# jopohl/urh

Hardware: NVIDIA H100
Metric: MSamples/s IQ demod+digitize (complex64) (higher is better)
Workload: dtype f32

## Files before the change

### urh_b200/csrc/center.cu

```cuda
#include "dense.cuh"
#include "scan.cuh"

#include <math.h>
#include <stdlib.h>

int urh_window_var_bitwise(urh_ctx* ctx, const float* d_x, int64_t n, const int64_t* d_prefix, int64_t t0, int64_t t1, int64_t r0,
                           int64_t r1, float* h_out2);

struct CenStats {
    double sum, sumsq;
    float mn, mx;
    long long cnt;
};

__global__ void __launch_bounds__(URH_WARPS_PER_BLOCK * 32)
k_tile_stats_f32(const float* __restrict__ x, int64_t n, int64_t ntiles, UrhTileStats* __restrict__ ts) {
    const int lane = threadIdx.x & 31;
    const int64_t tile = (int64_t)blockIdx.x * URH_WARPS_PER_BLOCK + (threadIdx.x >> 5);
    if (tile >= ntiles) return;
    const int64_t base = tile * URH_TILE;
    UrhStatAcc acc;
    acc.init();
    acc.all_noise = false;
    if (base + URH_TILE <= n && (((uintptr_t)x) & 15) == 0) {
        const float4* p = (const float4*)(x + base) + lane;
        constexpr int ITERS = URH_TILE / 128;
        float4 cur[4], nxt[4];
#pragma unroll
        for (int j = 0; j < 4; j++) cur[j] = __ldg(p + j * 32);
        for (int it = 0; it < ITERS; it += 4) {
            if (it + 4 < ITERS) {
#pragma unroll
                for (int j = 0; j < 4; j++) nxt[j] = __ldg(p + (it + 4 + j) * 32);
            }
#pragma unroll
            for (int j = 0; j < 4; j++) {
                acc.add(cur[j].x); acc.add(cur[j].y); acc.add(cur[j].z); acc.add(cur[j].w);
            }
#pragma unroll
            for (int j = 0; j < 4; j++) cur[j] = nxt[j];
        }
    } else {
        for (int j = lane; j < URH_TILE; j += 32)
            if (base + j < n) acc.add(x[base + j]);
    }
    acc.store(ts + tile, lane);
}

__global__ void k_tile_counts(const UrhTileStats* __restrict__ ts, int64_t ntiles, int64_t* __restrict__ prefix) {
    const int64_t t = (int64_t)blockIdx.x * blockDim.x + threadIdx.x;
    if (t < ntiles) prefix[t] = ts[t].cnt;
}

__global__ void k_find_window_tiles(const int64_t* __restrict__ prefix, int64_t ntiles, int64_t r0, int64_t r1, int64_t* __restrict__ win) {
    const int64_t t = (int64_t)blockIdx.x * blockDim.x + threadIdx.x;
    if (t >= ntiles) return;
    const int64_t a = prefix[t], b = prefix[t + 1];
    if (b <= a) return;
    const bool covered = a >= r0 && b <= r1;
    const bool has_r0 = a <= r0 && r0 < b, has_r1 = a <= r1 - 1 && r1 - 1 < b;
    if (has_r0) { win[0] = t; win[2] = covered ? -1 : t; }
    if (has_r1) { win[1] = t; win[3] = (covered || has_r0) ? -1 : t; }
}

#define CEN_PER (URH_TILE / 256)
__device__ __forceinline__ int64_t cen_tile_ranks(const float* __restrict__ x, int64_t n, int64_t t, int64_t tile_rank0, float (&v)[CEN_PER],
                                                  int* s_pre) {
    const int64_t base = t * URH_TILE + (int64_t)threadIdx.x * CEN_PER;
    int mine = 0;
#pragma unroll
    for (int j = 0; j < CEN_PER; j++) {
        v[j] = (base + j < n) ? x[base + j] : -5.0f;
        mine += (v[j] > -4.0f) ? 1 : 0;
    }
    s_pre[threadIdx.x] = mine;
    __syncthreads();
    for (int off = 1; off < 256; off <<= 1) {
        int add = 0;
        if (threadIdx.x >= off) add = s_pre[threadIdx.x - off];
        __syncthreads();
        s_pre[threadIdx.x] += add;
        __syncthreads();
    }
    return tile_rank0 + s_pre[threadIdx.x] - mine;
}

__device__ __forceinline__ void cen_block_fold(double sum, double sq, float mn, float mx, long long cnt, CenStats* out) {
    __shared__ double s_sum[256], s_sq[256];
    __shared__ float s_mn[256], s_mx[256];
    __shared__ long long s_cnt[256];
    __syncthreads();
    s_sum[threadIdx.x] = sum; s_sq[threadIdx.x] = sq; s_mn[threadIdx.x] = mn; s_mx[threadIdx.x] = mx; s_cnt[threadIdx.x] = cnt;
    __syncthreads();
    for (int off = 128; off > 0; off >>= 1) {
        if (threadIdx.x < off) {
            s_sum[threadIdx.x] += s_sum[threadIdx.x + off];
            s_sq[threadIdx.x] += s_sq[threadIdx.x + off];
            s_mn[threadIdx.x] = fminf(s_mn[threadIdx.x], s_mn[threadIdx.x + off]);
            s_mx[threadIdx.x] = fmaxf(s_mx[threadIdx.x], s_mx[threadIdx.x + off]);
            s_cnt[threadIdx.x] += s_cnt[threadIdx.x + off];
        }
        __syncthreads();
    }
    if (threadIdx.x == 0) {
        CenStats r;
        r.sum = s_sum[0]; r.sumsq = s_sq[0]; r.mn = s_mn[0]; r.mx = s_mx[0]; r.cnt = s_cnt[0];
        *out = r;
    }
}

__global__ void __launch_bounds__(256) k_cut_tile_stats(const float* __restrict__ x, int64_t n, const int64_t* __restrict__ prefix,
                                                       const int64_t* __restrict__ win, int64_t r0, int64_t r1, CenStats* __restrict__ out) {
    __shared__ int s_pre[256];
    const int64_t t = win[2 + blockIdx.x];
    double sum = 0.0, sq = 0.0;
    float mn = INFINITY, mx = -INFINITY;
    long long cnt = 0;
    if (t >= 0) {
        float v[CEN_PER];
        int64_t rank = cen_tile_ranks(x, n, t, prefix[t], v, s_pre);
#pragma unroll
        for (int j = 0; j < CEN_PER; j++) {
            if (v[j] > -4.0f) {
                if (rank >= r0 && rank < r1) {
                    sum += (double)v[j];
                    sq += (double)v[j] * (double)v[j];
                    mn = fminf(mn, v[j]);
                    mx = fmaxf(mx, v[j]);
                    cnt++;
                }
                rank++;
            }
        }
    }
    cen_block_fold(sum, sq, mn, mx, cnt, out + blockIdx.x);
}

__global__ void __launch_bounds__(256) k_interior_tile_stats(const UrhTileStats* __restrict__ ts, const int64_t* __restrict__ prefix,
                                                            int64_t ntiles, int64_t r0, int64_t r1, CenStats* __restrict__ partial) {
    double sum = 0.0, sq = 0.0;
    float mn = INFINITY, mx = -INFINITY;
    long long cnt = 0;
    for (int64_t t = (int64_t)blockIdx.x * 256 + threadIdx.x; t < ntiles; t += (int64_t)gridDim.x * 256) {
        const int64_t a = prefix[t], b = prefix[t + 1];
        if (b > a && a >= r0 && b <= r1) {
            const UrhTileStats v = ts[t];
            sum += v.sum; sq += v.sumsq; mn = fminf(mn, v.mn); mx = fmaxf(mx, v.mx); cnt += v.cnt;
        }
    }
    cen_block_fold(sum, sq, mn, mx, cnt, partial + blockIdx.x);
}

__global__ void __launch_bounds__(256) k_center_fold(const CenStats* __restrict__ partial, int64_t count, CenStats* __restrict__ out) {
    double sum = 0.0, sq = 0.0;
    float mn = INFINITY, mx = -INFINITY;
    long long cnt = 0;
    for (int64_t t = threadIdx.x; t < count; t += 256) {
        const CenStats p = partial[t];
        sum += p.sum; sq += p.sumsq; mn = fminf(mn, p.mn); mx = fmaxf(mx, p.mx); cnt += p.cnt;
    }
    cen_block_fold(sum, sq, mn, mx, cnt, out);
}

int urh_center_tiles_begin(urh_ctx* ctx, const float* d_x, const UrhTileStats* ts, int64_t n, int64_t* h_total) {
    const int64_t ntiles = urh_div_up(n, URH_TILE);
    int64_t *prefix, *d_total;
    URH_CHECK(urh_arena(ctx, (size_t)ntiles + 1, &prefix));
    URH_CHECK(urh_arena(ctx, 4, &d_total));
    URH_LAUNCH(ctx, k_tile_counts, (unsigned)urh_div_up(ntiles, 256), 256, 0, ts, ntiles, prefix);
    URH_CHECK((urhscan::device_scan<int64_t, urhscan::AddI64>(ctx, prefix, ntiles, urhscan::AddI64(), (int64_t)0, true, d_total)));
    URH_CUDA(ctx, cudaMemcpyAsync(prefix + ntiles, d_total, sizeof(int64_t), cudaMemcpyDeviceToDevice, ctx->stream));
    URH_CHECK(urh_read_i64(ctx, d_total, 1, h_total));
    ctx->center_prefix = prefix;
    ctx->center_ts = ts;
    ctx->center_n = n;
    ctx->center_x = d_x;
    return URH_OK;
}

static int tiles_from_array(urh_ctx* ctx, const float* d_x, int64_t n, int64_t* h_total) {
    urh_arena_reset(ctx);
    ctx->center_prefix = nullptr;
    const int64_t ntiles = urh_div_up(n, URH_TILE);
    UrhTileStats* ts;
    URH_CHECK(urh_arena(ctx, (size_t)ntiles, &ts));
    URH_LAUNCH(ctx, k_tile_stats_f32, (unsigned)urh_div_up(ntiles, URH_WARPS_PER_BLOCK), URH_WARPS_PER_BLOCK * 32, 0, d_x, n, ntiles, ts);
    return urh_center_tiles_begin(ctx, d_x, ts, n, h_total);
}

static bool tiles_match(const urh_ctx* ctx, const float* d_x, int64_t n) {
    return ctx->center_prefix && ctx->center_n == n && ctx->center_x == (const void*)d_x;
}

extern "C" int urh_center_window_stats(urh_ctx* ctx, const float* d_qad, int64_t n, int64_t r0, int64_t r1, double* h_out5) {
    h_out5[0] = 0.0; h_out5[1] = INFINITY; h_out5[2] = -INFINITY; h_out5[3] = 0.0; h_out5[4] = 0.0;
    if (!tiles_match(ctx, d_qad, n)) URH_FAIL(ctx, URH_ERR_INVALID, "urh_afp_demod_tiles (same qad, same n) must precede urh_center_window_stats");
    if (r1 <= r0) return URH_OK;
    const int64_t ntiles = urh_div_up(n, URH_TILE);
    const int64_t* prefix = (const int64_t*)ctx->center_prefix;
    const UrhTileStats* ts = (const UrhTileStats*)ctx->center_ts;
    int64_t* d_win;
    CenStats* partial;
    CenStats* folded;
    const int nb = ctx->sm_count * 2;
    URH_CHECK(urh_arena(ctx, 4, &d_win));
    URH_CHECK(urh_arena(ctx, (size_t)nb + 4, &partial));
    URH_CHECK(urh_arena(ctx, 2, &folded));
    URH_CUDA(ctx, cudaMemsetAsync(d_win, 0xff, 4 * sizeof(int64_t), ctx->stream));
    URH_LAUNCH(ctx, k_find_window_tiles, (unsigned)urh_div_up(ntiles, 256), 256, 0, prefix, ntiles, r0, r1, d_win);
    URH_LAUNCH(ctx, k_interior_tile_stats, nb, 256, 0, ts, prefix, ntiles, r0, r1, partial);
    URH_LAUNCH(ctx, k_cut_tile_stats, 2, 256, 0, d_qad, n, prefix, d_win, r0, r1, partial + nb);
    URH_LAUNCH(ctx, k_center_fold, 1, 256, 0, partial, (int64_t)nb + 2, folded);
    CenStats st;
    URH_CUDA(ctx, cudaMemcpyAsync(ctx->h_mail, folded, sizeof(CenStats), cudaMemcpyDeviceToHost, ctx->stream));
    URH_CUDA(ctx, cudaStreamSynchronize(ctx->stream));
    memcpy(&st, ctx->h_mail, sizeof(st));
    h_out5[0] = (double)st.cnt; h_out5[1] = (double)st.mn; h_out5[2] = (double)st.mx; h_out5[3] = st.sum; h_out5[4] = st.sumsq;
    return URH_OK;
}

extern "C" int urh_center_window_var(urh_ctx* ctx, const float* d_qad, int64_t n, int64_t r0, int64_t r1, double* h_out2) {
    h_out2[0] = h_out2[1] = 0.0;
    if (!tiles_match(ctx, d_qad, n)) URH_FAIL(ctx, URH_ERR_INVALID, "the tile table of this array must precede urh_center_window_var");
    if (r1 <= r0) return URH_OK;
    float mv[2];
    URH_CHECK(urh_window_var_bitwise(ctx, d_qad, n, (const int64_t*)ctx->center_prefix, 0, urh_div_up(n, URH_TILE) - 1, r0, r1, mv));
    h_out2[0] = (double)mv[0];
    h_out2[1] = (double)mv[1];
    return URH_OK;
}

extern "C" int urh_center_stats(urh_ctx* ctx, const float* d_x, int64_t n, int64_t max_size, double* h_out) {
    for (int i = 0; i < 7; i++) h_out[i] = 0.0;
    if (n <= 0) return URH_OK;
    int64_t total = 0;
    URH_CHECK(tiles_from_array(ctx, d_x, n, &total));
    int64_t r0 = (int64_t)(0.05 * (double)total), r1 = (int64_t)(0.95 * (double)total);
    if (max_size >= 0 && r1 - r0 > max_size) r1 = r0 + max_size;
    h_out[0] = (double)total; h_out[1] = (double)r0; h_out[2] = (double)r1;
    if (r1 <= r0) return URH_OK;
    double w[5];
    URH_CHECK(urh_center_window_stats(ctx, d_x, n, r0, r1, w));
    if (w[0] <= 0.0) return URH_OK;
    h_out[3] = w[1]; h_out[4] = w[2];
    float mv[2];
    URH_CHECK(urh_window_var_bitwise(ctx, d_x, n, (const int64_t*)ctx->center_prefix, 0, urh_div_up(n, URH_TILE) - 1, r0, r1, mv));
    h_out[5] = (double)mv[0];
    h_out[6] = (double)mv[1];
    return URH_OK;
}

__global__ void k_hist_edges(double hmin, double hstep, int64_t nbins, float* __restrict__ fe) {
    const int64_t k = (int64_t)blockIdx.x * blockDim.x + threadIdx.x;
    if (k <= nbins) fe[k] = __double2float_ru(__dadd_rn(hmin, __dmul_rn((double)k, hstep)));
    if (k == nbins) {
        fe[nbins + 1] = __double2float_rd(__dadd_rn(hmin, __dmul_rn((double)nbins, hstep)));
        fe[nbins + 2] = fmaxf(__double2float_ru(hmin), nextafterf(-4.0f, 0.0f));
    }
}

struct HistBins {
    const float* fe;
    float f_min, f_hi, scale, off;
    int nbins;
    __device__ __forceinline__ void load(const float* fe_, float scale_, int nbins_) {
        fe = fe_; nbins = nbins_; scale = scale_;
        f_hi = fe[nbins + 1];
        f_min = fe[nbins + 2];
        off = -fe[0] * scale;
    }
    template <bool FAST>
    __device__ __forceinline__ int bin_of(float f) const {
        const bool valid = f >= f_min && f <= f_hi;
        if (FAST) {
            const float t = fmaf(f, scale, off);
            int r = __float_as_int(t + 12582912.0f) - 0x4B400000;
            r = max(0, min(r, nbins));
            int k = r - ((f < fe[r]) ? 1 : 0);
            k = min(k, nbins - 1);
            return valid ? k : -1;
        }
        if (!valid) return -1;
        int k = (int)((f - fe[0]) * scale);
        k = max(0, min(k, nbins - 1));
        while (k > 0 && f < fe[k]) k--;
        while (k < nbins - 1 && f >= fe[k + 1]) k++;
        return k;
    }
};

struct HistCache {
    float lo0, hi0, lo1, hi1, lo2, hi2, lo3, hi3;
    int h0, h1, h2, h3;
    unsigned c0, c1, c2, c3;
    __device__ __forceinline__ void init() {
        lo0 = lo1 = lo2 = lo3 = INFINITY;
        hi0 = hi1 = hi2 = hi3 = -INFINITY;
        h0 = h1 = h2 = h3 = 0;
        c0 = c1 = c2 = c3 = 0u;
    }
};

template <bool SMEM>
__device__ __forceinline__ void hist_bump(unsigned int* s_hist, unsigned long long* hist, int k, unsigned c) {
    if (SMEM) atomicAdd(&s_hist[k], c);
    else atomicAdd(&hist[k], (unsigned long long)c);
}

template <bool SMEM, bool FAST>
__device__ __forceinline__ void hist_miss(HistCache& hc, const HistBins& hb, unsigned int* s_hist, unsigned long long* hist, float f) {
    const int k = hb.bin_of<FAST>(f);
    if (k < 0) return;
    const float lo = fmaxf(hb.fe[k], hb.f_min);
    const float hi = (k == hb.nbins - 1) ? nextafterf(hb.f_hi, INFINITY) : hb.fe[k + 1];
    unsigned cm = hc.c0; int which = 0;
    if (hc.c1 < cm) { cm = hc.c1; which = 1; }
    if (hc.c2 < cm) { cm = hc.c2; which = 2; }
    if (hc.c3 < cm) { cm = hc.c3; which = 3; }
    const int old = which == 0 ? hc.h0 : which == 1 ? hc.h1 : which == 2 ? hc.h2 : hc.h3;
    if (cm) hist_bump<SMEM>(s_hist, hist, old, cm);
    if (which == 0) { hc.h0 = k; hc.c0 = 1u; hc.lo0 = lo; hc.hi0 = hi; }
    else if (which == 1) { hc.h1 = k; hc.c1 = 1u; hc.lo1 = lo; hc.hi1 = hi; }
    else if (which == 2) { hc.h2 = k; hc.c2 = 1u; hc.lo2 = lo; hc.hi2 = hi; }
    else { hc.h3 = k; hc.c3 = 1u; hc.lo3 = lo; hc.hi3 = hi; }
}

template <bool SMEM, bool FAST>
__device__ __forceinline__ void hist_put(HistCache& hc, const HistBins& hb, unsigned int* s_hist, unsigned long long* hist, float f,
                                         unsigned one) {
    unsigned miss;
    asm("{\n\t.reg .pred p0, p1, p2, p3, pv;\n\t"
        "setp.ge.f32 p0, %5, %6;\n\tsetp.lt.and.f32 p0, %5, %7, p0;\n\t@p0 mad.lo.u32 %0, %0, %15, %15;\n\t"
        "setp.ge.f32 p1, %5, %8;\n\tsetp.lt.and.f32 p1, %5, %9, p1;\n\t@p1 mad.lo.u32 %1, %1, %15, %15;\n\t"
        "setp.ge.f32 p2, %5, %10;\n\tsetp.lt.and.f32 p2, %5, %11, p2;\n\t@p2 mad.lo.u32 %2, %2, %15, %15;\n\t"
        "setp.ge.f32 p3, %5, %12;\n\tsetp.lt.and.f32 p3, %5, %13, p3;\n\t@p3 mad.lo.u32 %3, %3, %15, %15;\n\t"
        "or.pred p0, p0, p1;\n\tor.pred p2, p2, p3;\n\tor.pred p0, p0, p2;\n\t"
        "setp.ge.f32 pv, %5, %14;\n\t"
        "and.pred pv, pv, !p0;\n\t"
        "selp.u32 %4, 1, 0, pv;\n\t}"
        : "+r"(hc.c0), "+r"(hc.c1), "+r"(hc.c2), "+r"(hc.c3), "=r"(miss)
        : "f"(f), "f"(hc.lo0), "f"(hc.hi0), "f"(hc.lo1), "f"(hc.hi1), "f"(hc.lo2), "f"(hc.hi2), "f"(hc.lo3), "f"(hc.hi3),
          "f"(hb.f_min), "r"(one));
    if (miss) hist_miss<SMEM, FAST>(hc, hb, s_hist, hist, f);
}

template <bool SMEM>
__device__ __forceinline__ void hist_flush(HistCache& hc, unsigned int* s_hist, unsigned long long* hist) {
    if (hc.c0) hist_bump<SMEM>(s_hist, hist, hc.h0, hc.c0);
    if (hc.c1) hist_bump<SMEM>(s_hist, hist, hc.h1, hc.c1);
    if (hc.c2) hist_bump<SMEM>(s_hist, hist, hc.h2, hc.c2);
    if (hc.c3) hist_bump<SMEM>(s_hist, hist, hc.h3, hc.c3);
}

template <bool SMEM, bool FAST>
__device__ __forceinline__ void hist_interior_body(const float* __restrict__ x, int64_t n, int64_t t_first, int64_t t_end, int blk, int nblk,
                                                   const float* __restrict__ g_fe, float scale, int nbins,
                                                   unsigned long long* __restrict__ hist, int edges_in_smem,
                                                   const int64_t* __restrict__ prefix) {
    extern __shared__ unsigned int s_dyn[];
    unsigned int* s_hist = s_dyn;
    float* s_fe = (float*)(s_dyn + (SMEM ? nbins : 0));
    const int lane = threadIdx.x & 31;
    if (SMEM)
        for (int b = threadIdx.x; b < nbins; b += 256) s_hist[b] = 0u;
    if (edges_in_smem)
        for (int b = threadIdx.x; b < nbins + 3; b += 256) s_fe[b] = g_fe[b];
    __syncthreads();
    HistBins hb;
    if (FAST) hb.load(s_fe, scale, nbins);
    else hb.load(edges_in_smem ? s_fe : g_fe, scale, nbins);
    HistCache hc;
    hc.init();
    const int64_t gw = (int64_t)blk * 8 + (threadIdx.x >> 5), nw = (int64_t)nblk * 8;
    const bool vec = (((uintptr_t)x) & 15) == 0;
    const unsigned one = blockDim.x >> 8;
    {
        for (int64_t t = t_first + gw; t < t_end; t += nw) {
            if (prefix[t + 1] == prefix[t]) continue;
            const int64_t base = t * URH_TILE;
            if (vec) {
                const float4* p = (const float4*)(x + base) + lane;
                constexpr int ITERS = URH_TILE / 128, DEPTH = 4;
                float4 buf[DEPTH];
#pragma unroll
                for (int j = 0; j < DEPTH; j++) buf[j] = __ldg(p + j * 32);
#pragma unroll 1
                for (int it = 0; it < ITERS; it += DEPTH) {
                    const bool more = it + DEPTH < ITERS;
#pragma unroll
                    for (int j = 0; j < DEPTH; j++) {
                        const float4 v = buf[j];
                        if (more) buf[j] = __ldg(p + (it + DEPTH + j) * 32);
                        hist_put<SMEM, FAST>(hc, hb, s_hist, hist, v.x, one);
                        hist_put<SMEM, FAST>(hc, hb, s_hist, hist, v.y, one);
                        hist_put<SMEM, FAST>(hc, hb, s_hist, hist, v.z, one);
                        hist_put<SMEM, FAST>(hc, hb, s_hist, hist, v.w, one);
                    }
                }
            } else {
                for (int j = lane; j < URH_TILE; j += 32) hist_put<SMEM, FAST>(hc, hb, s_hist, hist, x[base + j], one);
            }
        }
    }
    hist_flush<SMEM>(hc, s_hist, hist);
    if (SMEM) {
        __syncthreads();
        for (int b = threadIdx.x; b < nbins; b += 256)
            if (s_hist[b]) atomicAdd(&hist[b], (unsigned long long)s_hist[b]);
    }
}

template <bool SMEM, bool FAST>
__global__ void __launch_bounds__(256, 4) k_hist_interior(const float* __restrict__ x, int64_t n, const int64_t* __restrict__ win,
                                                      const float* __restrict__ g_fe, float scale, int nbins,
                                                      unsigned long long* __restrict__ hist, int edges_in_smem,
                                                      const int64_t* __restrict__ prefix) {
    const int64_t w0 = win[0];
    hist_interior_body<SMEM, FAST>(x, n, w0 + 1, w0 >= 0 ? win[1] : 0, blockIdx.x, gridDim.x, g_fe, scale, nbins, hist, edges_in_smem, prefix);
}

__device__ __forceinline__ void hist_window_ends_body(const float* __restrict__ x, int64_t n, const int64_t* __restrict__ prefix,
                                                      const int64_t* __restrict__ win, int64_t r0, int64_t r1,
                                                      const float* __restrict__ g_fe, float scale, int nbins,
                                                      unsigned long long* __restrict__ hist, unsigned long long* __restrict__ hist2 = nullptr) {
    __shared__ int s_pre[256];
    const int64_t t = win[blockIdx.x];
    if (t < 0 || (blockIdx.x == 1 && t == win[0])) return;
    HistBins hb;
    hb.load(g_fe, scale, nbins);
    float v[CEN_PER];
    int64_t rank = cen_tile_ranks(x, n, t, prefix[t], v, s_pre);
#pragma unroll
    for (int j = 0; j < CEN_PER; j++) {
        const bool kept = v[j] > -4.0f;
        const int k = hb.bin_of<false>(v[j]);
        if (k >= 0 && rank >= r0 && rank < r1) {
            atomicAdd(&hist[k], 1ull);
            if (hist2) atomicAdd(&hist2[k], 1ull);
        }
        rank += kept ? 1 : 0;
    }
}

__global__ void __launch_bounds__(256) k_hist_window_ends(const float* __restrict__ x, int64_t n, const int64_t* __restrict__ prefix,
                                                         const int64_t* __restrict__ win, int64_t r0, int64_t r1,
                                                         const float* __restrict__ g_fe, float scale, int nbins,
                                                         unsigned long long* __restrict__ hist) {
    hist_window_ends_body(x, n, prefix, win, r0, r1, g_fe, scale, nbins, hist);
}

extern "C" int urh_center_histogram_tiles(urh_ctx* ctx, const float* d_qad, int64_t n, int64_t r0, int64_t r1, double hmin,
                                          double hstep, int64_t nbins, int64_t* h_hist) {
    if (nbins <= 0) return URH_OK;
    if (!tiles_match(ctx, d_qad, n)) URH_FAIL(ctx, URH_ERR_INVALID, "urh_afp_demod_tiles (same qad, same n) must precede urh_center_histogram_tiles");
    if (nbins > (int64_t)1 << 30) URH_FAIL(ctx, URH_ERR_INVALID, "too many histogram bins");
    const int64_t ntiles = urh_div_up(n, URH_TILE);
    const int64_t* prefix = (const int64_t*)ctx->center_prefix;
    unsigned long long* hist;
    float* fe;
    int64_t* d_win;
    URH_CHECK(urh_arena(ctx, (size_t)nbins, &hist));
    URH_CHECK(urh_arena(ctx, (size_t)nbins + 3, &fe));
    URH_CHECK(urh_arena(ctx, 4, &d_win));
    URH_CUDA(ctx, cudaMemsetAsync(hist, 0, (size_t)nbins * sizeof(unsigned long long), ctx->stream));
    URH_CUDA(ctx, cudaMemsetAsync(d_win, 0xff, 4 * sizeof(int64_t), ctx->stream));
    if (r1 > r0) {
        URH_LAUNCH(ctx, k_hist_edges, (unsigned)urh_div_up(nbins + 1, 256), 256, 0, hmin, hstep, nbins, fe);
        URH_LAUNCH(ctx, k_find_window_tiles, (unsigned)urh_div_up(ntiles, 256), 256, 0, prefix, ntiles, r0, r1, d_win);
        const bool in_smem = nbins <= 12000;
        const int edges_smem = (in_smem && nbins <= 6000) ? 1 : 0;
        const size_t dyn = (in_smem ? (size_t)nbins * 4 : 0) + (edges_smem ? (size_t)(nbins + 3) * 4 : 0);
        const float scale = (float)(1.0 / hstep);
        const double edge_abs = fmax(fabs(hmin), fabs(hmin + (double)nbins * hstep));
        const bool fast = edges_smem && hstep > 0.0 && edge_abs / hstep < 1048576.0;
        const unsigned gs = (unsigned)min(urh_div_up(ntiles, 8), (int64_t)ctx->sm_count * 8);
        const int64_t* cw = d_win;
        const float* cfe = fe;
        if (in_smem && fast) URH_LAUNCH(ctx, (k_hist_interior<true, true>), gs, 256, dyn, d_qad, n, cw, cfe, scale, (int)nbins, hist, edges_smem, prefix);
        else if (in_smem) URH_LAUNCH(ctx, (k_hist_interior<true, false>), gs, 256, dyn, d_qad, n, cw, cfe, scale, (int)nbins, hist, edges_smem, prefix);
        else URH_LAUNCH(ctx, (k_hist_interior<false, false>), gs, 256, dyn, d_qad, n, cw, cfe, scale, (int)nbins, hist, edges_smem, prefix);
        URH_LAUNCH(ctx, k_hist_window_ends, 2, 256, 0, d_qad, n, prefix, (const int64_t*)d_win, r0, r1, (const float*)fe, scale, (int)nbins, hist);
    }
    URH_CUDA(ctx, cudaMemcpyAsync(h_hist, hist, (size_t)nbins * sizeof(int64_t), cudaMemcpyDeviceToHost, ctx->stream));
    URH_CUDA(ctx, cudaStreamSynchronize(ctx->stream));
    return URH_OK;
}

extern "C" int urh_center_histogram(urh_ctx* ctx, const float* d_x, int64_t n, int64_t r0, int64_t r1, double hmin,
                                    double hstep, int64_t nbins, int64_t* h_hist) {
    if (nbins <= 0 || n <= 0) return URH_OK;
    if (!tiles_match(ctx, d_x, n)) {
        int64_t total = 0;
        URH_CHECK(tiles_from_array(ctx, d_x, n, &total));
    }
    return urh_center_histogram_tiles(ctx, d_x, n, r0, r1, hmin, hstep, nbins, h_hist);
}

#include "tilescan.cuh"

#define CEN_MAX_BINS 6000
#define CEN_VAR_MIN_RATIO 0x1p-14

struct __align__(16) CenterPlan {
    long long total, offset;
    long long r0, r1;
    long long lr0, lr1;
    long long win[4];
    CenStats local;
    double hmin, edge1, delta;
    long long nbins;
    double center;
    float centerf;
    float scale;
    int fast;
    int state;
    unsigned int ticket;
    int certified;
    long long straddle;
    long long pad;
};

struct ScanKept {
    const UrhTileStats* ts;
    int64_t* prefix;
    __device__ __forceinline__ int64_t load(int64_t t) const { return ts[t].cnt; }
    __device__ __forceinline__ void post(int64_t t, const int64_t& excl, const int64_t&) const { prefix[t] = excl; }
};
struct CenAddI64 {
    __device__ __forceinline__ int64_t operator()(int64_t a, int64_t b) const { return a + b; }
};

__global__ void k_center_ranks(const int64_t* __restrict__ counts, int rank, int world, int64_t max_size, CenterPlan* __restrict__ plan) {
    long long total = 0, offset = 0;
    for (int q = 0; q < world; q++) {
        if (q < rank) offset += counts[q];
        total += counts[q];
    }
    const long long kept = counts[rank];
    long long r0 = (long long)(0.05 * (double)total), r1 = (long long)(0.95 * (double)total);
    if (max_size >= 0 && r1 - r0 > max_size) r1 = r0 + max_size;
    plan->total = total; plan->offset = offset; plan->r0 = r0; plan->r1 = r1;
    long long a = r0 - offset, b = r1 - offset;
    a = a < 0 ? 0 : (a > kept ? kept : a);
    b = b < 0 ? 0 : (b > kept ? kept : b);
    plan->lr0 = a; plan->lr1 = b;
    plan->ticket = 0u;
    plan->state = 1;
    plan->certified = 0;
    plan->straddle = 0;
}

__device__ __forceinline__ int64_t cen_tile_of_rank(const int64_t* __restrict__ prefix, int64_t ntiles, int64_t r) {
    int64_t lo = 0, hi = ntiles;
    while (hi - lo > 1) {
        const int64_t mid = (lo + hi) >> 1;
        if (prefix[mid] <= r) lo = mid; else hi = mid;
    }
    return lo;
}

__global__ void __launch_bounds__(256) k_center_window(const float* __restrict__ x, int64_t n, const UrhTileStats* __restrict__ ts,
                                                      const int64_t* __restrict__ prefix, int64_t ntiles, CenterPlan* __restrict__ plan,
                                                      CenStats* __restrict__ partial) {
    __shared__ long long s_win[4];
    __shared__ int s_pre[256];
    __shared__ bool s_last;
    const long long r0 = plan->lr0, r1 = plan->lr1;
    if (threadIdx.x == 0) {
        long long w0 = -1, w1 = -1, w2 = -1, w3 = -1;
        if (r1 > r0) {
            w0 = cen_tile_of_rank(prefix, ntiles, r0);
            w1 = cen_tile_of_rank(prefix, ntiles, r1 - 1);
            const bool cov0 = prefix[w0] >= r0 && prefix[w0 + 1] <= r1;
            const bool cov1 = prefix[w1] >= r0 && prefix[w1 + 1] <= r1;
            w2 = cov0 ? -1 : w0;
            w3 = (cov1 || w1 == w0) ? -1 : w1;
        }
        s_win[0] = w0; s_win[1] = w1; s_win[2] = w2; s_win[3] = w3;
        if (blockIdx.x == 0) { plan->win[0] = w0; plan->win[1] = w1; plan->win[2] = w2; plan->win[3] = w3; }
    }
    __syncthreads();
    double sum = 0.0, sq = 0.0;
    float mn = INFINITY, mx = -INFINITY;
    long long cnt = 0;
    if (s_win[0] >= 0) {
        for (int64_t t = s_win[0] + (int64_t)blockIdx.x * 256 + threadIdx.x; t <= s_win[1]; t += (int64_t)gridDim.x * 256) {
            const int64_t a = prefix[t], b = prefix[t + 1];
            if (b > a && a >= r0 && b <= r1) {
                const UrhTileStats v = ts[t];
                sum += v.sum; sq += v.sumsq; mn = fminf(mn, v.mn); mx = fmaxf(mx, v.mx); cnt += v.cnt;
            }
        }
    }
    cen_block_fold(sum, sq, mn, mx, cnt, partial + blockIdx.x);
    if (blockIdx.x < 2) {
        const int64_t t = s_win[2 + blockIdx.x];
        sum = 0.0; sq = 0.0; mn = INFINITY; mx = -INFINITY; cnt = 0;
        if (t >= 0) {
            float v[CEN_PER];
            int64_t rank = cen_tile_ranks(x, n, t, prefix[t], v, s_pre);
#pragma unroll
            for (int j = 0; j < CEN_PER; j++) {
                if (v[j] > -4.0f) {
                    if (rank >= r0 && rank < r1) {
                        sum += (double)v[j];
                        sq += (double)v[j] * (double)v[j];
                        mn = fminf(mn, v[j]);
                        mx = fmaxf(mx, v[j]);
                        cnt++;
                    }
                    rank++;
                }
            }
        }
        cen_block_fold(sum, sq, mn, mx, cnt, partial + gridDim.x + blockIdx.x);
    }
    __threadfence();
    __syncthreads();
    if (threadIdx.x == 0) s_last = atomicAdd(&plan->ticket, 1u) == gridDim.x - 1;
    __syncthreads();
    if (!s_last) return;
    __threadfence();
    sum = 0.0; sq = 0.0; mn = INFINITY; mx = -INFINITY; cnt = 0;
    for (int64_t t = threadIdx.x; t < (int64_t)gridDim.x + 2; t += 256) {
        CenStats p;
        {
            const int4* src = (const int4*)(partial + t);
            int4 w0 = __ldcg(src), w1 = __ldcg(src + 1);
            memcpy(&p, &w0, 16);
            memcpy((char*)&p + 16, &w1, 16);
        }
        sum += p.sum; sq += p.sumsq; mn = fminf(mn, p.mn); mx = fmaxf(mx, p.mx); cnt += p.cnt;
    }
    cen_block_fold(sum, sq, mn, mx, cnt, &plan->local);
}

__global__ void __launch_bounds__(256) k_center_plan(const CenStats* __restrict__ parts, int world, CenterPlan* __restrict__ plan,
                                                    float* __restrict__ fe, unsigned long long* __restrict__ hist,
                                                    unsigned long long* __restrict__ xhist) {
    __shared__ int s_state;
    __shared__ long long s_nbins;
    __shared__ double s_hmin, s_edge1, s_delta;
    if (threadIdx.x == 0) {
        double cnt = 0.0, sum = 0.0, sq = 0.0;
        float mn = INFINITY, mx = -INFINITY;
        for (int q = 0; q < world; q++) {
            cnt += (double)parts[q].cnt;
            mn = fminf(mn, parts[q].mn);
            mx = fmaxf(mx, parts[q].mx);
            sum = __dadd_rn(sum, parts[q].sum);
            sq = __dadd_rn(sq, parts[q].sumsq);
        }
        int state = 0;
        long long nbins = 0;
        double hmin = 0.0, edge1 = 0.0, delta = 0.0;
        if (plan->r1 > plan->r0 && cnt > 0.0) {
            const double mean = __ddiv_rn(sum, cnt);
            double ss = __dsub_rn(sq, __dmul_rn(__dmul_rn(cnt, mean), mean));
            if (ss < 0.0) ss = 0.0;
            const double var = __ddiv_rn(ss, cnt);
            const double hstep = (double)__double2float_rn(var);
            hmin = (double)mn;
            const double stop = __dadd_rn((double)mx, hstep);
            if (!(var >= __dmul_rn(__dmul_rn(mean, mean), CEN_VAR_MIN_RATIO))) state = 2;
            else if (hstep != 0.0) {
                const double val = __ddiv_rn(__dsub_rn(stop, hmin), hstep);
                if (val == val && fabs(val) < 9.0e18) {
                    const long long len = (long long)ceil(val);
                    if (len >= 2) {
                        nbins = len - 1;
                        edge1 = __dadd_rn(hmin, hstep);
                        delta = __dsub_rn(edge1, hmin);
                        state = (nbins <= CEN_MAX_BINS && delta > 0.0) ? 1 : 2;
                    }
                }
            }
        }
        plan->hmin = hmin; plan->edge1 = edge1; plan->delta = delta; plan->nbins = nbins;
        plan->state = state;
        plan->center = 0.0; plan->centerf = 0.0f;
        if (state == 1) {
            plan->scale = (float)(1.0 / delta);
            const double edge_abs = fmax(fabs(hmin), fabs(hmin + (double)nbins * delta));
            plan->fast = (edge_abs / delta < 1048576.0) ? 1 : 0;
        }
        s_state = state; s_nbins = nbins; s_hmin = hmin; s_edge1 = edge1; s_delta = delta;
    }
    __syncthreads();
    if (s_state != 1) return;
    const long long nbins = s_nbins;
    for (long long k = threadIdx.x; k <= nbins; k += 256) {
        const double e = (k == 0) ? s_hmin : (k == 1 ? s_edge1 : __dadd_rn(s_hmin, __dmul_rn((double)k, s_delta)));
        fe[k] = __double2float_ru(e);
        if (k == nbins) {
            fe[nbins + 1] = __double2float_rd(e);
            fe[nbins + 2] = fmaxf(__double2float_ru(s_hmin), nextafterf(-4.0f, 0.0f));
        }
        if (k < nbins) {
            hist[k] = 0ull;
            if (xhist) xhist[k] = 0ull;
        }
    }
}

template <bool FAST>
__global__ void __launch_bounds__(256, 3) k_hist_interior_dev(const float* __restrict__ x, int64_t n, const CenterPlan* __restrict__ plan,
                                                          const float* __restrict__ g_fe, unsigned long long* __restrict__ hist,
                                                          const int64_t* __restrict__ prefix) {
    if (plan->state != 1 || plan->certified || (plan->fast != 0) != FAST) return;
    hist_interior_body<true, FAST>(x, n, plan->win[0] + 1, plan->win[1], blockIdx.x, gridDim.x, g_fe, plan->scale, (int)plan->nbins, hist, 1,
                                   prefix);
}

__device__ __forceinline__ void cen_full_slabs(int64_t win0, int64_t win1, int64_t slab_tiles, int64_t* sf, int64_t* se) {
    *sf = (win0 + slab_tiles) / slab_tiles;
    *se = win1 / slab_tiles;
}

__global__ void __launch_bounds__(256) k_hist_window_ends_dev(const float* __restrict__ x, int64_t n, const int64_t* __restrict__ prefix,
                                                             const CenterPlan* __restrict__ plan, const float* __restrict__ g_fe,
                                                             unsigned long long* __restrict__ hist, unsigned long long* __restrict__ xhist,
                                                             int64_t slab_tiles) {
    if (plan->state != 1) return;
    if (blockIdx.x < 2) {
        hist_window_ends_body(x, n, prefix, (const int64_t*)plan->win, plan->lr0, plan->lr1, g_fe, plan->scale, (int)plan->nbins, hist, xhist);
        return;
    }
    const int64_t w0 = plan->win[0], w1 = plan->win[1];
    int64_t sf, se;
    cen_full_slabs(w0, w1, slab_tiles, &sf, &se);
    int64_t a_end = w1, b_begin = w1;
    if (sf < se) { a_end = sf * slab_tiles; b_begin = se * slab_tiles; }
    const int blk = blockIdx.x - 2, nblk = gridDim.x - 2, nbins = (int)plan->nbins;
    const float scale = plan->scale;
    if (plan->fast) {
        hist_interior_body<true, true>(x, n, w0 + 1, a_end, blk, nblk, g_fe, scale, nbins, xhist, 1, prefix);
        hist_interior_body<true, true>(x, n, b_begin, w1, blk, nblk, g_fe, scale, nbins, xhist, 1, prefix);
    } else {
        hist_interior_body<true, false>(x, n, w0 + 1, a_end, blk, nblk, g_fe, scale, nbins, xhist, 1, prefix);
        hist_interior_body<true, false>(x, n, b_begin, w1, blk, nblk, g_fe, scale, nbins, xhist, 1, prefix);
    }
}

__device__ __forceinline__ double cen_left_edge(const CenterPlan* plan, int k) {
    return (k == 0) ? plan->hmin : (k == 1 ? plan->edge1 : __dadd_rn(plan->hmin, __dmul_rn((double)k, plan->delta)));
}

#define CERT_THREADS 512
__global__ void __launch_bounds__(CERT_THREADS) k_center_certify(const UrhFine fine, CenterPlan* __restrict__ plan, const float* __restrict__ fe,
                                                                 const unsigned long long* __restrict__ xhist, unsigned long long* __restrict__ lo,
                                                                 unsigned long long* __restrict__ hi) {
    __shared__ unsigned long long s_ge[URH_FINE_NB + 1];
    __shared__ unsigned long long s_part[CERT_THREADS];
    __shared__ unsigned char s_flag[CEN_MAX_BINS];
    __shared__ unsigned long long s_key[3];
    __shared__ unsigned int s_certain;
    if (plan->state != 1) return;
    const int tid = threadIdx.x;
    constexpr int PER = URH_FINE_NB / CERT_THREADS;
    int64_t sf, se;
    cen_full_slabs(plan->win[0], plan->win[1], fine.slab_tiles, &sf, &se);
    unsigned long long b[PER], tot = 0;
#pragma unroll
    for (int j = 0; j < PER; j++) {
        unsigned long long v = 0;
        for (int64_t sl = sf; sl < se; sl++) v += fine.gh[sl * URH_FINE_NB + tid * PER + j];
        b[j] = v;
        tot += v;
    }
    s_part[tid] = tot;
    if (tid < 3) s_key[tid] = 0ull;
    if (tid == 0) s_certain = 0u;
    __syncthreads();
    for (int off = 1; off < CERT_THREADS; off <<= 1) {
        const unsigned long long add = (tid + off < CERT_THREADS) ? s_part[tid + off] : 0ull;
        __syncthreads();
        s_part[tid] += add;
        __syncthreads();
    }
    unsigned long long run = (tid + 1 < CERT_THREADS) ? s_part[tid + 1] : 0ull;
#pragma unroll
    for (int j = PER - 1; j >= 0; j--) {
        run += b[j];
        s_ge[tid * PER + j] = run;
    }
    if (tid == 0) s_ge[URH_FINE_NB] = 0ull;
    __syncthreads();
    const int nbins = (int)plan->nbins;
    const float f_hi = fe[nbins + 1], f_min = fe[nbins + 2], top = nextafterf(f_hi, INFINITY);
    auto ge = [&](float t, unsigned long long& glo, unsigned long long& ghi) {
        const int bt = urh_fine_bucket(t, fine.scale, fine.off);
        const bool straddles = urh_fine_bucket(nextafterf(t, -INFINITY), fine.scale, fine.off) == bt;
        ghi = s_ge[bt];
        glo = straddles ? s_ge[bt + 1] : s_ge[bt];
    };
    for (int k = tid; k < nbins; k += CERT_THREADS) {
        const float a = fmaxf(fe[k], f_min), e = (k == nbins - 1) ? top : fminf(fe[k + 1], top);
        unsigned long long l = 0, u = 0;
        if (a < e) {
            unsigned long long alo, ahi, elo, ehi;
            ge(a, alo, ahi);
            ge(e, elo, ehi);
            l = alo > ehi ? alo - ehi : 0ull;
            u = ahi - elo;
        }
        lo[k] = xhist[k] + l;
        hi[k] = xhist[k] + u;
    }
    __syncthreads();
    int window = (int)(0.05 * (double)nbins) + 1;
    if (window < 2) window = 2;
    for (int k = tid; k < nbins; k += CERT_THREADS) {
        const unsigned long long l = lo[k], u = hi[k];
        bool certain = l > 0ull, possible = u > 0ull;
        for (int d = -(window - 1); d < window && (certain || possible); d++) {
            const int j = k + d;
            if (d == 0 || j < 0 || j >= nbins) continue;
            certain = certain && l > hi[j];
            possible = possible && u > lo[j];
        }
        s_flag[k] = certain ? 1 : (possible ? 2 : 0);
        if (certain) atomicAdd(&s_certain, 1u);
    }
    __syncthreads();
    for (int pass = 0; pass < 3; pass++) {
        const long long p0 = pass > 0 ? (long long)(8191 - (s_key[0] & 8191)) : -1, p1 = pass > 1 ? (long long)(8191 - (s_key[1] & 8191)) : -1;
        for (int k = tid; k < nbins; k += CERT_THREADS) {
            if (k == p0 || k == p1) continue;
            if (pass < 2 && s_flag[k] == 1) atomicMax(&s_key[pass], (lo[k] << 13) | (unsigned long long)(8191 - k));
            if (pass == 2 && s_flag[k] != 0) atomicMax(&s_key[2], hi[k]);
        }
        __syncthreads();
    }
    if (tid != 0 || s_certain < 2u) return;
    const int k1 = 8191 - (int)(s_key[0] & 8191), k2 = 8191 - (int)(s_key[1] & 8191);
    plan->straddle = (long long)((hi[k1] - lo[k1]) + (hi[k2] - lo[k2]));
    if (!(lo[k2] > s_key[2])) return;
    const double c = __ddiv_rn(__dadd_rn(cen_left_edge(plan, k1), cen_left_edge(plan, k2)), 2.0);
    plan->center = c;
    plan->centerf = __double2float_rn(c);
    plan->certified = 1;
}

__global__ void __launch_bounds__(256) k_center_pick(const unsigned long long* __restrict__ y, CenterPlan* __restrict__ plan) {
    __shared__ unsigned long long s_best[256];
    __shared__ int s_idx[256];
    __shared__ int s_cnt[256];
    if (plan->state != 1 || plan->certified) return;
    const int nbins = (int)plan->nbins;
    int window = (int)(0.05 * (double)nbins) + 1;
    if (window < 2) window = 2;
    unsigned long long top_val[2] = {0ull, 0ull};
    int top_idx[2] = {-1, -1};
    int found = 0;
    bool undecided = false;
    for (int pass = 0; pass < 2 && !undecided; pass++) {
        unsigned long long best = 0ull;
        int bi = -1, ties = 0;
        for (int i = threadIdx.x; i < nbins; i += 256) {
            if (pass == 1 && i == top_idx[0]) continue;
            const unsigned long long v = y[i];
            if (v == 0ull || v < best) continue;
            bool peak = true;
            for (int d = 1; d < window && peak; d++) {
                const unsigned long long a = (i + d < nbins) ? y[i + d] : 0ull;
                const unsigned long long b = (i - d >= 0) ? y[i - d] : 0ull;
                peak = v > a && v > b;
            }
            if (!peak) continue;
            if (v > best) { best = v; bi = i; ties = 1; }
            else ties++;
        }
        s_best[threadIdx.x] = best; s_idx[threadIdx.x] = bi; s_cnt[threadIdx.x] = ties;
        __syncthreads();
        if (threadIdx.x == 0) {
            unsigned long long b = 0ull;
            int idx = -1, t = 0;
            for (int j = 0; j < 256; j++) {
                if (s_idx[j] < 0) continue;
                if (s_best[j] > b) { b = s_best[j]; idx = s_idx[j]; t = s_cnt[j]; }
                else if (s_best[j] == b) t += s_cnt[j];
            }
            s_best[0] = b; s_idx[0] = idx; s_cnt[0] = t;
        }
        __syncthreads();
        const unsigned long long b = s_best[0];
        const int idx = s_idx[0], t = s_cnt[0];
        __syncthreads();
        if (idx < 0) break;
        if (pass == 0) {
            top_val[0] = b; top_idx[0] = idx; found = 1;
            if (t == 2) {
                int other = -1;
                for (int i = threadIdx.x; i < nbins; i += 256) {
                    if (i == idx || y[i] != b) continue;
                    bool peak = true;
                    for (int d = 1; d < window && peak; d++) {
                        const unsigned long long a = (i + d < nbins) ? y[i + d] : 0ull;
                        const unsigned long long c = (i - d >= 0) ? y[i - d] : 0ull;
                        peak = b > a && b > c;
                    }
                    if (peak) other = i;
                }
                s_idx[threadIdx.x] = other;
                __syncthreads();
                if (threadIdx.x == 0) {
                    int o = -1;
                    for (int j = 0; j < 256; j++) if (s_idx[j] >= 0) o = s_idx[j];
                    s_idx[0] = o;
                }
                __syncthreads();
                top_idx[1] = s_idx[0]; top_val[1] = b; found = 2;
                __syncthreads();
                break;
            }
            if (t > 2) undecided = true;
        } else {
            if (t > 1) undecided = true;
            else { top_val[1] = b; top_idx[1] = idx; found = 2; }
        }
    }
    if (threadIdx.x != 0) return;
    if (undecided) { plan->state = 2; return; }
    if (found == 0) { plan->state = 0; return; }
    double c;
    if (found == 1) c = cen_left_edge(plan, top_idx[0]);
    else c = __ddiv_rn(__dadd_rn(cen_left_edge(plan, top_idx[0]), cen_left_edge(plan, top_idx[1])), 2.0);
    plan->center = c;
    plan->centerf = __double2float_rn(c);
    plan->state = 1;
    (void)top_val;
}

int urh_center_chain(urh_ctx* ctx, const float* d_qad, int64_t n, const UrhTileStats* ts, int64_t max_size, int rank, int world,
                     const UrhFine* fine, CenterPlan** d_plan_out) {
    const int64_t ntiles = urh_div_up(n, URH_TILE);
    int64_t* prefix;
    CenterPlan* plan;
    CenStats* partial;
    float* fe;
    unsigned long long* hist;
    int64_t* d_counts;
    CenStats* d_parts;
    unsigned long long *xhist = nullptr, *cert_lo = nullptr, *cert_hi = nullptr;
    const int nb = ctx->sm_count * 2;
    URH_CHECK(urh_arena(ctx, (size_t)ntiles + 1, &prefix));
    URH_CHECK(urh_arena(ctx, 1, &plan));
    URH_CHECK(urh_arena(ctx, (size_t)nb + 2, &partial));
    URH_CHECK(urh_arena(ctx, (size_t)CEN_MAX_BINS + 3, &fe));
    URH_CHECK(urh_arena(ctx, (size_t)CEN_MAX_BINS, &hist));
    URH_CHECK(urh_arena(ctx, (size_t)world, &d_counts));
    URH_CHECK(urh_arena(ctx, (size_t)world, &d_parts));
    if (fine) {
        URH_CHECK(urh_arena(ctx, (size_t)CEN_MAX_BINS, &xhist));
        URH_CHECK(urh_arena(ctx, (size_t)CEN_MAX_BINS, &cert_lo));
        URH_CHECK(urh_arena(ctx, (size_t)CEN_MAX_BINS, &cert_hi));
    }
    ScanKept fk;
    fk.ts = ts; fk.prefix = prefix;
    URH_CHECK((urhts::scan<int64_t, CenAddI64, ScanKept>(ctx, ntiles, (int64_t)0, CenAddI64(), fk, prefix + ntiles)));
    const int64_t* counts = prefix + ntiles;
    if (world > 1) {
        URH_TL_MARK(ctx, "x1 kept counts: enter");
        URH_CHECK(urh_nccl_allgather(ctx, prefix + ntiles, d_counts, sizeof(int64_t)));
        URH_TL_MARK(ctx, "x1 kept counts: done");
        counts = d_counts;
    }
    URH_LAUNCH(ctx, k_center_ranks, 1, 1, 0, counts, rank, world, max_size, plan);
    URH_LAUNCH(ctx, k_center_window, nb, 256, 0, d_qad, n, ts, (const int64_t*)prefix, ntiles, plan, partial);
    const CenStats* parts = &plan->local;
    if (world > 1) {
        URH_TL_MARK(ctx, "x2 window partials: enter");
        URH_CHECK(urh_nccl_allgather(ctx, &plan->local, d_parts, sizeof(CenStats)));
        URH_TL_MARK(ctx, "x2 window partials: done");
        parts = d_parts;
    }
    URH_LAUNCH(ctx, k_center_plan, 1, 256, 0, parts, world, plan, fe, hist, xhist);
    const size_t dyn = (size_t)CEN_MAX_BINS * 4 + (size_t)(CEN_MAX_BINS + 3) * 4;
    const unsigned gs = (unsigned)min(urh_div_up(ntiles, 8), (int64_t)ctx->sm_count * 8);
    URH_LAUNCH(ctx, k_hist_window_ends_dev, fine ? 2 + ctx->sm_count * 4 : 2, 256, fine ? dyn : 0, d_qad, n, (const int64_t*)prefix,
               (const CenterPlan*)plan, (const float*)fe, hist, xhist, fine ? fine->slab_tiles : (int64_t)1);
    if (fine) URH_LAUNCH(ctx, k_center_certify, 1, CERT_THREADS, 0, *fine, plan, (const float*)fe, (const unsigned long long*)xhist, cert_lo, cert_hi);
    URH_LAUNCH(ctx, (k_hist_interior_dev<true>), gs, 256, dyn, d_qad, n, (const CenterPlan*)plan, (const float*)fe, hist, (const int64_t*)prefix);
    URH_LAUNCH(ctx, (k_hist_interior_dev<false>), gs, 256, dyn, d_qad, n, (const CenterPlan*)plan, (const float*)fe, hist, (const int64_t*)prefix);
    if (world > 1) {
        URH_TL_MARK(ctx, "x3 histogram sum: enter");
        URH_CHECK(urh_nccl_allreduce_i64(ctx, (int64_t*)hist, CEN_MAX_BINS, 0));
        URH_TL_MARK(ctx, "x3 histogram sum: done");
    }
    URH_LAUNCH(ctx, k_center_pick, 1, 256, 0, (const unsigned long long*)hist, plan);
    ctx->center_prefix = prefix;
    ctx->center_ts = ts;
    ctx->center_n = n;
    ctx->center_x = d_qad;
    *d_plan_out = plan;
    return URH_OK;
}

int urh_center_plan_certify_stats(urh_ctx* ctx, const CenterPlan* plan, int64_t* h_dst3) {
    h_dst3[0] = h_dst3[1] = h_dst3[2] = 0;
    URH_CUDA(ctx, cudaMemcpyAsync(h_dst3, &plan->certified, sizeof(int), cudaMemcpyDeviceToHost, ctx->stream));
    URH_CUDA(ctx, cudaMemcpyAsync(h_dst3 + 2, &plan->straddle, sizeof(long long), cudaMemcpyDeviceToHost, ctx->stream));
    return URH_OK;
}

extern "C" int urh_center_certify_stats(urh_ctx* ctx, int64_t* h_out3) {
    for (int i = 0; i < 3; i++) h_out3[i] = ctx->center_cert[i];
    return URH_OK;
}

int urh_center_plan_result(urh_ctx* ctx, const CenterPlan* plan, const float** d_centerf, const double** d_center, const int** d_state) {
    if (d_centerf) *d_centerf = &plan->centerf;
    if (d_center) *d_center = &plan->center;
    if (d_state) *d_state = &plan->state;
    return URH_OK;
}
```

### urh_b200/csrc/common.cuh

```cuda
#pragma once
#include <cuda_runtime.h>
#include <stdint.h>
#include <stdio.h>
#include <stdlib.h>
#include <string.h>
#include <vector>

#include "../../include/urh_b200.h"

#define URH_FULL_MASK 0xffffffffu

struct urh_block {
    void* ptr;
    size_t bytes;
};

struct urh_ctx {
    int device;
    int sm_count;
    cudaStream_t stream;
    cudaStream_t copy_stream[2];
    cudaEvent_t ev_start, ev_stop;
    cudaEvent_t ev_copy[2], ev_comp[2];
    cudaEvent_t ev_k0, ev_k1;
    int profiling;
    int dense_timed;
    cudaEvent_t tl_ev[32];
    const char* tl_name[32];
    int tl_count, tl_ready;
    char err[512];
    int64_t launches;
    std::vector<urh_block> arena;
    size_t arena_block;
    size_t arena_used;
    size_t arena_need;
    int64_t* pulses;
    size_t pulses_cap_rows;
    int64_t pulses_k;
    int64_t* h_mail;
    void* h_stage[2];
    size_t h_stage_bytes;
    int fft_plan;
    int fft_nfft;
    int64_t fft_batch;
    bool fft_valid;
    void* img_tw;
    int img_tw_n;
    void* shard_tiles;
    void* shard_staging;
    int shard_cap, shard_tol;
    int64_t shard_n;
    void* shard_state;
    int64_t costas_stats[3];
    int64_t costas_redone;
    int64_t costas_stitch[4];
    int mod_plan[2];
    int mod_plan_valid[2];
    int64_t mod_plan_n[2];
    int bits_valid;
    int64_t bits_nmsg, bits_total, bits_npos;
    void *bits_ptr, *bits_msg_off, *bits_pauses, *bits_pos;
    const void* center_ts;
    const void* center_x;
    int64_t center_n;
    void* center_prefix;
    int64_t center_cert[3];
    int64_t spec_stats[3];
    void* nccl_comm;
    void* nccl_stage;
    void* nccl_hstage;
    int nccl_rank, nccl_world;
    void* ts_mem;
    int64_t ts_cap_blocks;
    unsigned long long ts_issued;
    uint32_t ts_epoch;
    void* step_dev;
    void* shard_fin;
    int64_t stream_free_low, stream_chunks;
    size_t arena_live;
    size_t arena_peak;
    std::vector<int64_t> segments;
};

#define URH_CUDA(ctx, call)                                                                         \
    do {                                                                                            \
        cudaError_t e__ = (call);                                                                   \
        if (e__ != cudaSuccess) {                                                                   \
            snprintf((ctx)->err, sizeof((ctx)->err), "%s:%d: %s -> %s", __FILE__, __LINE__, #call,  \
                     cudaGetErrorString(e__));                                                      \
            return (e__ == cudaErrorMemoryAllocation) ? URH_ERR_NOMEM : URH_ERR_CUDA;               \
        }                                                                                           \
    } while (0)

#define URH_CHECK(call)                 \
    do {                                \
        int rc__ = (call);              \
        if (rc__ != URH_OK) return rc__; \
    } while (0)

#define URH_FAIL(ctx, code, ...)                                  \
    do {                                                          \
        snprintf((ctx)->err, sizeof((ctx)->err), __VA_ARGS__);    \
        return (code);                                            \
    } while (0)

#define URH_LAUNCH(ctx, kernel, grid, block, smem, ...)                                   \
    do {                                                                                  \
        kernel<<<(grid), (block), (smem), (ctx)->stream>>>(__VA_ARGS__);                  \
        (ctx)->launches++;                                                                \
        URH_CUDA(ctx, cudaGetLastError());                                                \
    } while (0)

#define URH_TL_MARK(ctx, label) do { if ((ctx)->profiling >= 2 && (ctx)->tl_ready && (ctx)->tl_count < 32) { \
        (ctx)->tl_name[(ctx)->tl_count] = (label); cudaEventRecord((ctx)->tl_ev[(ctx)->tl_count++], (ctx)->stream); } } while (0)
#define URH_TL_RESET(ctx) do { (ctx)->tl_count = 0; } while (0)
#define URH_PROF_BEGIN(ctx) do { if ((ctx)->profiling) cudaEventRecord((ctx)->ev_k0, (ctx)->stream); } while (0)
#define URH_PROF_END(ctx) do { if ((ctx)->profiling) { cudaEventRecord((ctx)->ev_k1, (ctx)->stream); (ctx)->dense_timed = 1; } } while (0)

void urh_arena_reset(urh_ctx* ctx);
int urh_arena_alloc(urh_ctx* ctx, size_t bytes, void** out);
template <typename T>
static inline int urh_arena(urh_ctx* ctx, size_t count, T** out) {
    void* p = nullptr;
    int rc = urh_arena_alloc(ctx, count * sizeof(T), &p);
    *out = (T*)p;
    return rc;
}
struct UrhArenaMark {
    size_t block, used, live;
};
static inline UrhArenaMark urh_arena_mark(const urh_ctx* ctx) { return UrhArenaMark{ctx->arena_block, ctx->arena_used, ctx->arena_live}; }
static inline void urh_arena_release(urh_ctx* ctx, const UrhArenaMark& m) {
    ctx->arena_block = m.block;
    ctx->arena_used = m.used;
    ctx->arena_live = m.live;
}
int urh_ensure_pulses(urh_ctx* ctx, size_t rows);
int urh_ensure_pulses_keep(urh_ctx* ctx, size_t rows, size_t keep);
void urh_stream_sample_free(urh_ctx* ctx);
void urh_release_mod_plans(urh_ctx* ctx);
int urh_ensure_stage(urh_ctx* ctx, size_t bytes);

struct UrhCostasStream {
    float* state;
    int64_t* acc;
    int segs;
};
int urh_costas_stream_begin(urh_ctx* ctx, UrhCostasStream* S);
int urh_costas_stream_chunk(urh_ctx* ctx, UrhCostasStream* S, int64_t c, const void* d_iq, int dtype, int64_t n, float noise_sqrd,
                            int loop_order, float bandwidth, float* d_out);
int urh_costas_stream_end(urh_ctx* ctx, const UrhCostasStream* S);
int64_t urh_costas_arena_bytes(int64_t n, int loop_order);

int urh_read_i64(urh_ctx* ctx, const int64_t* d_src, int count, int64_t* h_out);

__host__ __device__ static inline int64_t urh_div_up(int64_t a, int64_t b) { return (a + b - 1) / b; }

static inline int urh_iq_bytes(int dtype) {
    switch (dtype) {
        case URH_DT_I8:
        case URH_DT_U8: return 2;
        case URH_DT_I16:
        case URH_DT_U16: return 4;
        case URH_DT_F32: return 8;
        default: return 0;
    }
}

static inline float urh_noise_value(int mod_type) {
    switch (mod_type) {
        case URH_MOD_ASK: return 0.0f;
        case URH_MOD_FSK:
        case URH_MOD_PSK:
        case URH_MOD_OQPSK: return -4.0f;
        case URH_MOD_QAM: return 0.0f * -4.0f;
        default: return 0.0f;
    }
}
```

### urh_b200/csrc/digitize.cu

```cuda
#include "dense.cuh"
#include "scan.cuh"
#include "sparse.cuh"
#include "fsk_fast.cuh"
#include "dense_f32.cuh"
#include "stream_ring.cuh"

#include <math.h>
#include <stdlib.h>


template <int DT, int MOD, bool DIGITIZE>
__device__ __forceinline__ void dense_iq_tile(const void* __restrict__ iq, int64_t n, const UrhDemodParams& dp, float* __restrict__ qad_out,
                                              int vec_in, int vec_out, const UrhClassify& cls, int tol, UrhTileSummary* __restrict__ tiles,
                                              uint32_t* __restrict__ staging, int stage_cap, int16_t* __restrict__ init_cls, int cls_of_zero,
                                              int64_t tile, int has_halo, UrhTileStats* __restrict__ tile_stats, const UrhFine& fine,
                                              unsigned int* s_fine, unsigned int* g_fine) {
    const int lane = threadIdx.x & 31;
    const int64_t tile_start = tile * URH_TILE;
    const int tile_len = (int)((n - tile_start) < URH_TILE ? (n - tile_start) : URH_TILE);
    const int iters = (tile_len + 63) >> 6;

    UrhRunTracker rt;
    if (DIGITIZE) rt.init(tol, staging + tile * (int64_t)stage_cap);
    UrhStatAcc acc;
    acc.init();

    float cA = 0.0f, cB = 0.0f;
    if (MOD == URH_MOD_FSK && (tile_start > 0 || has_halo) && lane == 0) {
        typedef typename UrhElem<DT>::type E;
        const E* pp = (const E*)iq + 2 * (tile_start - 1);
        const UrhFskTerms t = urh_fsk_terms((float)pp[0], (float)pp[1]);
        cA = t.A; cB = t.B;
    }

    UrhPair cur = urh_load_pair<DT>(iq, tile_start + 2 * lane, n, vec_in != 0);
    for (int it = 0; it < iters; it++) {
        const int64_t pos0 = tile_start + (int64_t)it * 64 + 2 * lane;
        UrhPair nxt;
        if (it + 1 < iters) nxt = urh_load_pair<DT>(iq, pos0 + 64, n, vec_in != 0);

        const float m0 = __fadd_rn(__fmul_rn(cur.r0, cur.r0), __fmul_rn(cur.i0, cur.i0));
        const float m1 = __fadd_rn(__fmul_rn(cur.r1, cur.r1), __fmul_rn(cur.i1, cur.i1));
        float s0 = dp.noise_value, s1 = dp.noise_value;
        if (MOD == URH_MOD_FSK) {
            const UrhFskTerms t0 = urh_fsk_terms(cur.r0, cur.i0);
            const UrhFskTerms t1 = urh_fsk_terms(cur.r1, cur.i1);
            float pA = __shfl_up_sync(URH_FULL_MASK, t1.A, 1);
            float pB = __shfl_up_sync(URH_FULL_MASK, t1.B, 1);
            if (lane == 0) { pA = cA; pB = cB; }
            cA = __shfl_sync(URH_FULL_MASK, t1.A, 31);
            cB = __shfl_sync(URH_FULL_MASK, t1.B, 31);
            if (!(m0 <= dp.noise_sqrd)) s0 = urh_fsk_angle(pA, pB, t0.C, t0.D);
            if (!(m1 <= dp.noise_sqrd)) s1 = urh_fsk_angle(t0.A, t0.B, t1.C, t1.D);
        } else if (MOD == URH_MOD_ASK) {
            if (!(m0 <= dp.noise_sqrd)) s0 = __fdiv_rn(__fsqrt_rn(m0), dp.max_mag);
            if (!(m1 <= dp.noise_sqrd)) s1 = __fdiv_rn(__fsqrt_rn(m1), dp.max_mag);
        }
        if (pos0 == 0 && !has_halo) s0 = dp.noise_value;

        const bool v0 = pos0 < n, v1 = pos0 + 1 < n;
        if (tile_stats) {
            if (v0) { acc.add(s0); acc.all_noise = acc.all_noise && (s0 == dp.noise_value); }
            if (v1) { acc.add(s1); acc.all_noise = acc.all_noise && (s1 == dp.noise_value); }
            if (s_fine) {
                if (v0) urh_fine_add(s0, fine, s_fine, g_fine);
                if (v1) urh_fine_add(s1, fine, s_fine, g_fine);
            }
        }
        if (qad_out) {
            if (v1 && vec_out) urh_stg_f2(qad_out + pos0, s0, s1);
            else {
                if (v0) qad_out[pos0] = s0;
                if (v1) qad_out[pos0 + 1] = s1;
            }
        }
        if (DIGITIZE) {
            const int c0 = urh_classify(s0, cls), c1 = urh_classify(s1, cls);
            if (pos0 == 0) *init_cls = (int16_t)((s0 == cls.noise_value) ? -1 : cls_of_zero);
            rt.feed(it, c0, c1, v0, v1, lane);
        }
        cur = nxt;
    }
    if (tile_stats) acc.store(tile_stats + tile, lane);
    if (DIGITIZE) rt.finish(tile_len, tiles + tile, lane);
}

template <int DT, int MOD, bool DIGITIZE>
__global__ void __launch_bounds__(URH_WARPS_PER_BLOCK * 32)
k_dense_iq(const void* __restrict__ iq, int64_t n, UrhDemodParams dp, float* __restrict__ qad_out, int vec_in,
           int vec_out, const __grid_constant__ UrhClassify cls, int tol, UrhTileSummary* __restrict__ tiles,
           uint32_t* __restrict__ staging, int stage_cap, int16_t* __restrict__ init_cls, int cls_of_zero,
           int64_t tile_begin, int64_t tile_count, int has_halo, UrhTileStats* __restrict__ tile_stats, const UrhFine fine) {
    extern __shared__ unsigned int s_fine[];
    const int64_t tile_rel = (int64_t)blockIdx.x * URH_WARPS_PER_BLOCK + (threadIdx.x >> 5);
    const int64_t block_tile0 = tile_begin + (int64_t)blockIdx.x * URH_WARPS_PER_BLOCK;
    if (fine.gh) urh_fine_zero(s_fine);
    if (tile_rel < tile_count && (tile_begin + tile_rel) * URH_TILE < n)
        dense_iq_tile<DT, MOD, DIGITIZE>(iq, n, dp, qad_out, vec_in, vec_out, cls, tol, tiles, staging, stage_cap, init_cls, cls_of_zero,
                                    tile_begin + tile_rel, has_halo, tile_stats, fine,
                                    fine.gh ? s_fine : nullptr, fine.gh ? urh_fine_row(fine, tile_begin + tile_rel, block_tile0) : nullptr);
    if (fine.gh) urh_fine_flush(fine, s_fine, block_tile0);
}

template <int DT, bool DIGITIZE, bool WRITE, bool STATS>
__global__ void __launch_bounds__(URH_WARPS_PER_BLOCK * 32, (DT == URH_DT_F32) ? 5 : 4)
k_fsk_fifo(const void* __restrict__ iq, int64_t n, UrhDemodParams dp, float* __restrict__ qad_out, float thr0,
           float cls_noise, int tol, UrhTileSummary* __restrict__ tiles, uint32_t* __restrict__ staging, int stage_cap,
           int64_t tile_begin, int64_t tile_count, UrhTileStats* __restrict__ tile_stats, const UrhFine fine,
           const float* __restrict__ d_thr0 = nullptr, float* __restrict__ margin = nullptr) {
    __shared__ __align__(16) unsigned char s_fifo[URH_WARPS_PER_BLOCK][URH_FSK_FIFO + 1][64 * 2 * sizeof(typename UrhElem<DT>::type)];
    extern __shared__ unsigned int s_fine[];
    const bool fine_on = STATS && fine.gh;
    if (DIGITIZE && STATS) thr0 = *d_thr0;
    const int lane = threadIdx.x & 31;
    const int64_t tile_rel = (int64_t)blockIdx.x * URH_WARPS_PER_BLOCK + (threadIdx.x >> 5);
    const int64_t block_tile0 = tile_begin + (int64_t)blockIdx.x * URH_WARPS_PER_BLOCK;
    if (fine_on) urh_fine_zero(s_fine);
    if (tile_rel < tile_count) {
        const int64_t tile = tile_begin + tile_rel;
        UrhRunTracker rt;
        if (DIGITIZE) rt.init(tol, staging + tile * (int64_t)stage_cap);
        UrhOne one;
        one.p = dp.one;
        one.m = dp.mone;
        const uint32_t fifo = (uint32_t)__cvta_generic_to_shared(&s_fifo[threadIdx.x >> 5][0][0]);
        urh_fsk_full_tile<DT, DIGITIZE, WRITE, STATS>(iq, n, tile * URH_TILE, dp, qad_out, thr0, cls_noise, rt, lane, one,
                                                      STATS ? tile_stats + tile : nullptr, fifo, DIGITIZE ? tiles + tile : nullptr, fine,
                                                      fine_on ? s_fine : nullptr, fine_on ? urh_fine_row(fine, tile, block_tile0) : nullptr,
                                                      (DIGITIZE && STATS) ? margin + tile : nullptr);
    }
    if (fine_on) urh_fine_flush(fine, s_fine, block_tile0);
}

#define URH_GUESS_SAMPLES 16384
#define URH_GUESS_BINS 128
#define URH_GUESS_THREADS 1024
__global__ void __launch_bounds__(URH_GUESS_THREADS) k_speculate_guess(const float2* __restrict__ iq, int64_t n, float noise_sqrd, int forced,
                                                                      float forced_tg, float* __restrict__ d_tg, unsigned int* __restrict__ redone) {
    constexpr int PER = URH_GUESS_SAMPLES / URH_GUESS_THREADS;
    __shared__ unsigned int s_hist[URH_GUESS_BINS];
    __shared__ float s_mn[32], s_mx[32];
    if (forced) {
        if (threadIdx.x == 0) { *d_tg = forced_tg; *redone = 0u; }
        return;
    }
    for (int b = threadIdx.x; b < URH_GUESS_BINS; b += blockDim.x) s_hist[b] = 0u;
    float v[PER];
    float mn = INFINITY, mx = -INFINITY;
#pragma unroll
    for (int k = 0; k < PER; k++) {
        const int64_t i = 1 + (int64_t)(k * URH_GUESS_THREADS + threadIdx.x) * (n - 1) / URH_GUESS_SAMPLES;
        const float2 p = iq[i - 1], c = iq[i];
        v[k] = NAN;
        if (!(c.x * c.x + c.y * c.y <= noise_sqrd)) {
            v[k] = atan2f(p.x * c.y - p.y * c.x, p.x * c.x + p.y * c.y);
            mn = fminf(mn, v[k]);
            mx = fmaxf(mx, v[k]);
        }
    }
    for (int off = 16; off > 0; off >>= 1) {
        mn = fminf(mn, __shfl_xor_sync(URH_FULL_MASK, mn, off));
        mx = fmaxf(mx, __shfl_xor_sync(URH_FULL_MASK, mx, off));
    }
    if ((threadIdx.x & 31) == 0) { s_mn[threadIdx.x >> 5] = mn; s_mx[threadIdx.x >> 5] = mx; }
    __syncthreads();
    mn = INFINITY; mx = -INFINITY;
    for (int w = 0; w < URH_GUESS_THREADS / 32; w++) { mn = fminf(mn, s_mn[w]); mx = fmaxf(mx, s_mx[w]); }
    const float width = (mx - mn) / URH_GUESS_BINS;
    if (width > 0.0f) {
#pragma unroll
        for (int k = 0; k < PER; k++)
            if (!isnan(v[k])) atomicAdd(&s_hist[min((int)((v[k] - mn) / width), URH_GUESS_BINS - 1)], 1u);
    }
    __syncthreads();
    if (threadIdx.x != 0) return;
    *redone = 0u;
    if (!(mn <= mx)) { *d_tg = 0.0f; return; }
    if (!(width > 0.0f)) { *d_tg = mn; return; }
    constexpr int WINDOW = (int)(0.05 * URH_GUESS_BINS) + 1;
    int top[2] = {-1, -1};
    for (int b = 0; b < URH_GUESS_BINS; b++) {
        const unsigned int y = s_hist[b];
        bool peak = y > 0u;
        for (int d = 1; d < WINDOW && peak; d++)
            peak = y > (b + d < URH_GUESS_BINS ? s_hist[b + d] : 0u) && y > (b - d >= 0 ? s_hist[b - d] : 0u);
        if (!peak) continue;
        if (top[0] < 0 || y > s_hist[top[0]]) { top[1] = top[0]; top[0] = b; }
        else if (top[1] < 0 || y > s_hist[top[1]]) top[1] = b;
    }
    if (top[0] < 0) *d_tg = 0.5f * (mn + mx);
    else if (top[1] < 0) *d_tg = mn + ((float)top[0] + 0.5f) * width;
    else *d_tg = mn + (0.5f * (float)(top[0] + top[1]) + 0.5f) * width;
}


extern "C" int urh_get_center_thresholds(float center, float spacing, int modulation_order, float* h_out) {
    const int n = modulation_order / 2;
    for (int i = 0; i < n; i++) {
        volatile float t = (float)(n - (i + 1)) * spacing;
        h_out[i] = center - t;
    }
    for (int i = n; i < modulation_order - 1; i++) {
        volatile float t = (float)(i + 1 - n) * spacing;
        h_out[i] = center + t;
    }
    return URH_OK;
}

static int fill_classify(urh_ctx* ctx, UrhClassify* C, int mod_type, float center, uint8_t bits_per_symbol,
                         float spacing) {
    if (bits_per_symbol > 8) URH_FAIL(ctx, URH_ERR_INVALID, "bits_per_symbol %d > 8 not supported", (int)bits_per_symbol);
    memset(C, 0, sizeof(*C));
    C->noise_value = urh_noise_value(mod_type);
    C->order = 1 << bits_per_symbol;
    if (C->order > 1) urh_get_center_thresholds(center, spacing, C->order, C->thr);
    return URH_OK;
}

static int host_classify(float s, const UrhClassify& C) {
    int c = C.order - 1;
    for (int k = 0; k < C.order - 1; k++)
        if (s <= C.thr[k]) { c = k; break; }
    return c;
}

static float max_magnitude_for(int dtype) {
    switch (dtype) {
        case URH_DT_I8: return (float)sqrt(127.0 * 127.0 + 128.0 * 128.0);
        case URH_DT_U8: return (float)sqrt(255.0 * 255.0);
        case URH_DT_I16: return (float)sqrt(32768.0 * 32768.0 + 32767.0 * 32767.0);
        case URH_DT_U16: return (float)sqrt(65535.0 * 65535.0);
        default: return (float)sqrt(2.0);
    }
}

static bool iq_vec_aligned(const void* p, int dtype) { return ((uintptr_t)p % (2 * (size_t)urh_iq_bytes(dtype))) == 0; }

template <int DT, int MOD, bool DIG>
static int launch_dense_iq_t(urh_ctx* ctx, const void* d_iq, int64_t n, const UrhDemodParams& dp, float* d_qad,
                             const UrhClassify& cls, int tol, UrhTileSummary* tiles, uint32_t* staging,
                             int stage_cap, int16_t* init_cls, int cls_of_zero, int has_halo = 0,
                             UrhTileStats* tile_stats = nullptr, int64_t tile_lo = 0, int64_t tile_hi = -1,
                             const UrhFine& fine = UrhFine{}, UrhSpec* spec = nullptr) {
    const int64_t ntiles = urh_div_up(n, URH_TILE);
    const size_t fine_smem = fine.gh ? (size_t)URH_FINE_NB * sizeof(unsigned int) : 0;
    if (tile_hi < 0 || tile_hi > ntiles) tile_hi = ntiles;
    const int vec_in = iq_vec_aligned(d_iq, DT) ? 1 : 0;
    const int vec_out = (d_qad && ((uintptr_t)d_qad % 8) == 0) ? 1 : 0;
    const int threads = URH_WARPS_PER_BLOCK * 32;
    auto generic = [&](int64_t begin, int64_t end) -> int {
        begin = begin < tile_lo ? tile_lo : begin;
        end = end > tile_hi ? tile_hi : end;
        const int64_t count = end - begin;
        if (count <= 0) return URH_OK;
        URH_LAUNCH(ctx, (k_dense_iq<DT, MOD, DIG>), (unsigned)urh_div_up(count, URH_WARPS_PER_BLOCK), threads, fine_smem, d_iq, n, dp,
                   d_qad, vec_in, vec_out, cls, tol, tiles, staging, stage_cap, init_cls, cls_of_zero, begin, count, has_halo,
                   tile_stats, fine);
        return URH_OK;
    };
    const int64_t nfull = n / URH_TILE;
    const bool fast = MOD == URH_MOD_FSK && vec_in && (!d_qad || vec_out) && (!DIG || cls.order == 2) && nfull > 1;
    URH_PROF_BEGIN(ctx);
    if (fast) {
        const int64_t fb = tile_lo > 1 ? tile_lo : 1, fe = tile_hi < nfull ? tile_hi : nfull;
        if (fe > fb) {
            const unsigned grid = (unsigned)urh_div_up(fe - fb, URH_WARPS_PER_BLOCK);
            bool speculated = false;
            if constexpr (DT == URH_DT_F32 && MOD == URH_MOD_FSK && !DIG) {
                if (spec && tile_stats && d_qad) {
                    URH_LAUNCH(ctx, (k_fsk_fifo<DT, true, true, true>), grid, threads, fine_smem, d_iq, n, dp, d_qad, 0.0f, dp.noise_value,
                               tol, tiles, staging, stage_cap, fb, fe - fb, tile_stats, fine, (const float*)spec->tg, spec->margin);
                    spec->lo = fb;
                    spec->hi = fe;
                    speculated = true;
                }
            }
            if (speculated) {
            } else if (tile_stats && d_qad && !DIG) {
                URH_LAUNCH(ctx, (k_fsk_fifo<DT, false, true, true>), grid, threads, fine_smem, d_iq, n, dp, d_qad, cls.thr[0], cls.noise_value,
                           tol, tiles, staging, stage_cap, fb, fe - fb, tile_stats, fine);
            } else if (d_qad) {
                URH_LAUNCH(ctx, (k_fsk_fifo<DT, DIG, true, false>), grid, threads, 0, d_iq, n, dp, d_qad, cls.thr[0], cls.noise_value, tol,
                           tiles, staging, stage_cap, fb, fe - fb, nullptr, UrhFine{});
            } else {
                URH_LAUNCH(ctx, (k_fsk_fifo<DT, DIG, false, false>), grid, threads, 0, d_iq, n, dp, d_qad, cls.thr[0], cls.noise_value, tol,
                           tiles, staging, stage_cap, fb, fe - fb, nullptr, UrhFine{});
            }
        }
        URH_CHECK(generic(0, 1));
        URH_CHECK(generic(nfull, ntiles));
    } else {
        URH_CHECK(generic(0, ntiles));
    }
    URH_PROF_END(ctx);
    return URH_OK;
}

template <int MOD, bool DIG>
static int launch_dense_iq_m(urh_ctx* ctx, int dtype, const void* d_iq, int64_t n, const UrhDemodParams& dp,
                             float* d_qad, const UrhClassify& cls, int tol, UrhTileSummary* tiles,
                             uint32_t* staging, int stage_cap, int16_t* init_cls, int cls_of_zero, int has_halo = 0,
                             UrhTileStats* tile_stats = nullptr, int64_t tile_lo = 0, int64_t tile_hi = -1,
                             const UrhFine& fine = UrhFine{}, UrhSpec* spec = nullptr) {
    switch (dtype) {
        case URH_DT_I8: return launch_dense_iq_t<URH_DT_I8, MOD, DIG>(ctx, d_iq, n, dp, d_qad, cls, tol, tiles, staging, stage_cap, init_cls, cls_of_zero, has_halo, tile_stats, tile_lo, tile_hi, fine);
        case URH_DT_U8: return launch_dense_iq_t<URH_DT_U8, MOD, DIG>(ctx, d_iq, n, dp, d_qad, cls, tol, tiles, staging, stage_cap, init_cls, cls_of_zero, has_halo, tile_stats, tile_lo, tile_hi, fine);
        case URH_DT_I16: return launch_dense_iq_t<URH_DT_I16, MOD, DIG>(ctx, d_iq, n, dp, d_qad, cls, tol, tiles, staging, stage_cap, init_cls, cls_of_zero, has_halo, tile_stats, tile_lo, tile_hi, fine);
        case URH_DT_U16: return launch_dense_iq_t<URH_DT_U16, MOD, DIG>(ctx, d_iq, n, dp, d_qad, cls, tol, tiles, staging, stage_cap, init_cls, cls_of_zero, has_halo, tile_stats, tile_lo, tile_hi, fine);
        case URH_DT_F32: return launch_dense_iq_t<URH_DT_F32, MOD, DIG>(ctx, d_iq, n, dp, d_qad, cls, tol, tiles, staging, stage_cap, init_cls, cls_of_zero, has_halo, tile_stats, tile_lo, tile_hi, fine, spec);
        default: URH_FAIL(ctx, URH_ERR_DTYPE, "Unsupported dtype");
    }
}

int urh_costas_demod(urh_ctx* ctx, const void* d_iq, int dtype, int64_t n, float noise_sqrd, int loop_order,
                     float bandwidth, float* d_out);

static UrhDemodParams make_demod_params(float noise_mag, int mod_type, int dtype) {
    UrhDemodParams dp;
    volatile float nm = noise_mag;
    volatile float sq = nm * nm;
    dp.noise_sqrd = sq;
    dp.noise_value = urh_noise_value(mod_type);
    dp.max_mag = max_magnitude_for(dtype);
    dp.one = 1.0f;
    dp.mone = -1.0f;
    return dp;
}

extern "C" int urh_afp_demod(urh_ctx* ctx, const void* d_iq, int dtype, int64_t n, float noise_mag, int mod_type,
                             int mod_order, float costas_loop_bandwidth, float* d_out) {
    if (n < 0) URH_FAIL(ctx, URH_ERR_INVALID, "negative length");
    if (urh_iq_bytes(dtype) == 0) URH_FAIL(ctx, URH_ERR_DTYPE, "Unsupported dtype");
    if (n == 0) return URH_OK;
    if (n <= 2 || (mod_type != URH_MOD_ASK && mod_type != URH_MOD_FSK && mod_type != URH_MOD_PSK)) {
        URH_CUDA(ctx, cudaMemsetAsync(d_out, 0, (size_t)n * sizeof(float), ctx->stream));
        if (n > 2) {
            const float nv = urh_noise_value(mod_type);
            URH_CUDA(ctx, cudaMemcpyAsync(d_out, &nv, sizeof(float), cudaMemcpyHostToDevice, ctx->stream));
            URH_CUDA(ctx, cudaStreamSynchronize(ctx->stream));
        }
        return URH_OK;
    }
    const UrhDemodParams dp = make_demod_params(noise_mag, mod_type, dtype);
    if (mod_type == URH_MOD_PSK) return urh_costas_demod(ctx, d_iq, dtype, n, dp.noise_sqrd, mod_order, costas_loop_bandwidth, d_out);
    UrhClassify cls;
    memset(&cls, 0, sizeof(cls));
    if (mod_type == URH_MOD_ASK)
        return launch_dense_iq_m<URH_MOD_ASK, false>(ctx, dtype, d_iq, n, dp, d_out, cls, 0, nullptr, nullptr, 0, nullptr, 0);
    return launch_dense_iq_m<URH_MOD_FSK, false>(ctx, dtype, d_iq, n, dp, d_out, cls, 0, nullptr, nullptr, 0, nullptr, 0);
}

int urh_center_tiles_begin(urh_ctx* ctx, const float* d_x, const UrhTileStats* ts, int64_t n, int64_t* h_total);

extern "C" int urh_afp_demod_tiles(urh_ctx* ctx, const void* d_iq, int dtype, int64_t n, float noise_mag, int mod_type,
                                   float* d_qad_out, int halo, int64_t* h_kept) {
    if (n <= 2 || (mod_type != URH_MOD_ASK && mod_type != URH_MOD_FSK) || !d_qad_out)
        URH_FAIL(ctx, URH_ERR_INVALID, "urh_afp_demod_tiles: ASK/FSK, n > 2 and a qad buffer are required");
    if (urh_iq_bytes(dtype) == 0) URH_FAIL(ctx, URH_ERR_DTYPE, "Unsupported dtype");
    urh_arena_reset(ctx);
    const UrhDemodParams dp = make_demod_params(noise_mag, mod_type, dtype);
    UrhClassify cls;
    memset(&cls, 0, sizeof(cls));
    const int64_t ntiles = urh_div_up(n, URH_TILE);
    UrhTileStats* ts;
    URH_CHECK(urh_arena(ctx, (size_t)ntiles, &ts));
    if (mod_type == URH_MOD_ASK)
        URH_CHECK((launch_dense_iq_m<URH_MOD_ASK, false>(ctx, dtype, d_iq, n, dp, d_qad_out, cls, 0, nullptr, nullptr, 0, nullptr, 0, halo, ts)));
    else
        URH_CHECK((launch_dense_iq_m<URH_MOD_FSK, false>(ctx, dtype, d_iq, n, dp, d_qad_out, cls, 0, nullptr, nullptr, 0, nullptr, 0, halo, ts)));
    return urh_center_tiles_begin(ctx, d_qad_out, ts, n, h_kept);
}

int urh_finish_local(urh_ctx* ctx, int64_t n, int tol, bool is_ask, uint32_t sps, const UrhTileSummary* tiles, const uint32_t* staging,
                     int stage_cap, const int16_t* d_init, int64_t* k);
int urh_finish_shard(urh_ctx* ctx, int64_t n, int tol, bool is_ask, uint32_t sps, const UrhTileSummary* tiles, const uint32_t* staging,
                     int stage_cap, const int16_t* d_init, int64_t global_offset, int64_t n_total, int64_t* k);

static int stage_cap_for(int tol) { return URH_TILE / (tol + 1) + 2; }

static int digitizer_tables(urh_ctx* ctx, int64_t ntiles, int cap, UrhTileSummary** tiles, uint32_t** staging, int16_t** d_init) {
    URH_CHECK(urh_arena(ctx, (size_t)ntiles, tiles));
    URH_CHECK(urh_arena(ctx, (size_t)ntiles * cap, staging));
    return urh_arena(ctx, 8, d_init);
}

static int launch_dense_qad(urh_ctx* ctx, const float* x, int64_t n, const UrhClassify& cls, int tol, UrhTileSummary* tiles,
                            uint32_t* staging, int cap, int16_t* init, int c0, const float* d_thr0 = nullptr,
                            const UrhTileStats* ts = nullptr) {
    const unsigned grid = (unsigned)urh_div_up(urh_div_up(n, URH_TILE), URH_WARPS_PER_BLOCK);
    const int vec_in = (((uintptr_t)x % 8) == 0) ? 1 : 0;
    if (cls.order == 2)
        URH_LAUNCH(ctx, (k_dense_f32<SrcQad2, float>), grid, URH_WARPS_PER_BLOCK * 32, 0, x, n, vec_in, cls, tol, tiles, staging, cap, init,
                   c0, d_thr0, ts);
    else
        URH_LAUNCH(ctx, (k_dense_f32<SrcQad, float>), grid, URH_WARPS_PER_BLOCK * 32, 0, x, n, vec_in, cls, tol, tiles, staging, cap, init,
                   c0, d_thr0, ts);
    return URH_OK;
}

extern "C" int urh_grab_pulse_lens(urh_ctx* ctx, const float* d_qad, int64_t n, float center, uint16_t tolerance,
                                   int mod_type, uint32_t samples_per_symbol, uint8_t bits_per_symbol,
                                   float center_spacing, int64_t* k) {
    if (!k) return URH_ERR_INVALID;
    *k = 0;
    ctx->pulses_k = 0;
    if (n < 0) URH_FAIL(ctx, URH_ERR_INVALID, "negative length");
    if (n == 0) return URH_OK;
    urh_arena_reset(ctx);
    UrhClassify cls;
    URH_CHECK(fill_classify(ctx, &cls, mod_type, center, bits_per_symbol, center_spacing));
    const int tol = tolerance;
    const int64_t ntiles = urh_div_up(n, URH_TILE);
    const int cap = stage_cap_for(tol);
    UrhTileSummary* tiles;
    uint32_t* staging;
    int16_t* d_init;
    URH_CHECK(digitizer_tables(ctx, ntiles, cap, &tiles, &staging, &d_init));
    URH_PROF_BEGIN(ctx);
    URH_CHECK(launch_dense_qad(ctx, d_qad, n, cls, tol, tiles, staging, cap, d_init, host_classify(0.0f, cls)));
    URH_PROF_END(ctx);
    return urh_finish_local(ctx, n, tol, mod_type == URH_MOD_ASK, samples_per_symbol, tiles, staging, cap, d_init, k);
}

extern "C" int urh_demod_digitize(urh_ctx* ctx, const void* d_iq, int dtype, int64_t n, float noise_mag,
                                  int mod_type, float center, uint16_t tolerance, uint32_t samples_per_symbol,
                                  uint8_t bits_per_symbol, float center_spacing, float* d_qad_out, int64_t* k) {
    if (!k) return URH_ERR_INVALID;
    *k = 0;
    ctx->pulses_k = 0;
    if (n < 0) URH_FAIL(ctx, URH_ERR_INVALID, "negative length");
    if (urh_iq_bytes(dtype) == 0) URH_FAIL(ctx, URH_ERR_DTYPE, "Unsupported dtype");
    if (n == 0) return URH_OK;
    if (n <= 2 || (mod_type != URH_MOD_ASK && mod_type != URH_MOD_FSK)) {
        float* q = d_qad_out;
        if (!q) URH_CUDA(ctx, cudaMalloc((void**)&q, (size_t)n * sizeof(float)));
        int rc = urh_afp_demod(ctx, d_iq, dtype, n, noise_mag, mod_type, 1 << bits_per_symbol, 0.1f, q);
        if (rc == URH_OK)
            rc = urh_grab_pulse_lens(ctx, q, n, center, tolerance, mod_type, samples_per_symbol, bits_per_symbol,
                                     center_spacing, k);
        if (!d_qad_out) {
            cudaStreamSynchronize(ctx->stream);
            cudaFree(q);
        }
        return rc;
    }
    urh_arena_reset(ctx);
    UrhClassify cls;
    URH_CHECK(fill_classify(ctx, &cls, mod_type, center, bits_per_symbol, center_spacing));
    const UrhDemodParams dp = make_demod_params(noise_mag, mod_type, dtype);
    const int tol = tolerance;
    const int64_t ntiles = urh_div_up(n, URH_TILE);
    const int cap = stage_cap_for(tol);
    UrhTileSummary* tiles;
    uint32_t* staging;
    int16_t* d_init;
    URH_CHECK(digitizer_tables(ctx, ntiles, cap, &tiles, &staging, &d_init));
    const int c0 = host_classify(0.0f, cls);
    if (mod_type == URH_MOD_ASK)
        URH_CHECK((launch_dense_iq_m<URH_MOD_ASK, true>(ctx, dtype, d_iq, n, dp, d_qad_out, cls, tol, tiles, staging, cap, d_init, c0)));
    else
        URH_CHECK((launch_dense_iq_m<URH_MOD_FSK, true>(ctx, dtype, d_iq, n, dp, d_qad_out, cls, tol, tiles, staging, cap, d_init, c0)));
    return urh_finish_local(ctx, n, tol, mod_type == URH_MOD_ASK, samples_per_symbol, tiles, staging, cap, d_init, k);
}

int urh_finish_chunk(urh_ctx* ctx, int64_t n, int tol, bool is_ask, uint32_t sps, const UrhTileSummary* tiles, const uint32_t* staging,
                     int stage_cap, const int16_t* d_init, UrhChain* chain, int64_t global_offset, int64_t n_total, int64_t row_base,
                     int64_t rows_cap, int64_t* k);

static int64_t rows_bound(int64_t n, int tol) { return n / (tol + 1) + 3; }

struct StreamSizes {
    int64_t cs;
    int64_t src_slot;
    int64_t qad_slot;
    int64_t ring_bytes;
    int64_t arena;
    int64_t scan_items;
    int64_t rows_chunk;
};
static int64_t finish_arena_bytes(int64_t tiles, int64_t rows_cap, bool ask) {
    return r256(tiles * (int64_t)sizeof(RunCarry)) + 2 * r256(tiles * 4) + 2 * r256(tiles * 8) + r256((32 + 8) * 8) +
           (ask ? r256(rows_cap * 16) : 0);
}
static int psk_order_of(int entry) { return (entry & URH_STREAM_PSK) ? ((entry & URH_STREAM_PSK4) ? 4 : 2) : 0; }
static int psk_entry_flags(int mod_order) { return URH_STREAM_PSK | (mod_order >= 4 ? URH_STREAM_PSK4 : 0); }

static StreamSizes stream_sizes(int64_t n, int dtype, int tol, int64_t chunk_samples, int ring, int entry) {
    StreamSizes z;
    const int kind = entry & 0xf;
    const int psk = psk_order_of(entry);
    const bool resident = entry & URH_STREAM_RESIDENT;
    const int64_t ntiles = urh_div_up(n, URH_TILE);
    z.cs = resident ? ntiles * URH_TILE : stream_chunk_samples(n, chunk_samples);
    const int64_t ct = z.cs / URH_TILE;
    const int64_t cap = stage_cap_for(tol);
    const bool iq = kind != URH_STREAM_ENTRY_GRAB_PULSE_LENS;
    const bool digitize = kind != URH_STREAM_ENTRY_AFP_DEMOD;
    z.rows_chunk = rows_bound(z.cs, tol);
    if (resident) {
        z.src_slot = iq ? n * urh_iq_bytes(dtype) : n * 4;
        z.qad_slot = (kind == URH_STREAM_ENTRY_GRAB_PULSE_LENS) ? 0 : n * 4;
        z.ring_bytes = r256(z.src_slot) + r256(z.qad_slot);
    } else {
        z.src_slot = (kind == URH_STREAM_ENTRY_GRAB_PULSE_LENS && (entry & URH_STREAM_QAD_ON_DEVICE)) ? 0
                     : URH_STREAM_PAD + z.cs * (iq ? urh_iq_bytes(dtype) : 4);
        const bool qad_ring = kind == URH_STREAM_ENTRY_AFP_DEMOD ||
                              (kind == URH_STREAM_ENTRY_DEMOD_DIGITIZE && ((entry & URH_STREAM_QAD_OUT) || psk));
        z.qad_slot = qad_ring ? z.cs * 4 : 0;
        z.ring_bytes = ring * (r256(z.src_slot) + r256(z.qad_slot));
        if (kind == URH_STREAM_ENTRY_DEMOD_CENTER_DIGITIZE) z.ring_bytes += r256(n * 4);
    }
    z.arena = 0;
    z.scan_items = ct > z.rows_chunk ? ct : z.rows_chunk;
    if (digitize) z.arena += r256(ct * (int64_t)sizeof(UrhTileSummary)) + r256(ct * cap * 4) + r256(16) + r256(sizeof(UrhChain)) +
                             finish_arena_bytes(ct, z.rows_chunk, true);
    if (psk && !resident) z.arena += urh_costas_arena_bytes(z.cs, psk) + r256(16) + r256(6 * 8);
    if (kind == URH_STREAM_ENTRY_DEMOD_CENTER_DIGITIZE) {
        z.arena += r256(ntiles * (int64_t)sizeof(UrhTileStats)) + r256((int64_t)URH_FINE_SLABS * URH_FINE_NB * 4) + r256((ntiles + 1) * 8) +
                   ((int64_t)2 << 20);
        if (ntiles > z.scan_items) z.scan_items = ntiles;
    }
    return z;
}

static int64_t segment_arena_bytes(int64_t tiles) {
    const int64_t cap = URH_TILE / 10 + 2, cand = tiles * URH_TILE / 10 + 3;
    return r256(tiles * (int64_t)sizeof(UrhTileSummary)) + r256(tiles * cap * 4) + 2 * r256(tiles * (int64_t)sizeof(RunCarry)) +
           2 * r256(2 * (int64_t)sizeof(RunCarry)) + r256(tiles * 4) + r256(tiles * 8) + r256(32) + r256(cand * 8) + r256(cand * 2) +
           3 * r256((tiles + 2) * 16);
}
SegmentStreamSizes urh_segment_stream_sizes(int64_t n, int dtype, int64_t chunk_samples) {
    SegmentStreamSizes z;
    z.cs = stream_chunk_samples(n, chunk_samples);
    z.src_slot = r256(URH_STREAM_PAD + z.cs * urh_iq_bytes(dtype));
    z.mag_bytes = r256(z.cs * 8);
    z.arena = segment_arena_bytes(z.cs / URH_TILE);
    return z;
}

extern "C" int urh_stream_footprint(int64_t n, int dtype, int tolerance, int64_t chunk_samples, int ring, int entry, int64_t rows,
                                    int64_t* bytes) {
    if (!bytes || n < 0 || tolerance < 0 || tolerance > 0xffff || (entry & 0xf) > URH_STREAM_ENTRY_ESTIMATE) return URH_ERR_INVALID;
    if ((entry & 0xf) == URH_STREAM_ENTRY_SEGMENT_MESSAGES) {
        if (urh_iq_bytes(dtype) == 0) return URH_ERR_DTYPE;
        if (entry & URH_STREAM_RESIDENT) {
            *bytes = r256(n * urh_iq_bytes(dtype)) + r256(n * 8) + segment_arena_bytes(urh_div_up(n, URH_TILE)) + URH_ARENA_BLOCK;
            return URH_OK;
        }
        if (ring < 2 || ring > URH_STREAM_MAX_RING) return URH_ERR_INVALID;
        const SegmentStreamSizes z = urh_segment_stream_sizes(n, dtype, chunk_samples);
        *bytes = ring * z.src_slot + z.mag_bytes + stream_arena_bytes(z.arena);
        return URH_OK;
    }
    if ((entry & 0xf) == URH_STREAM_ENTRY_ESTIMATE) {
        if (!(entry & URH_STREAM_RESIDENT)) return URH_ERR_INVALID;
        if (urh_iq_bytes(dtype) == 0) return URH_ERR_DTYPE;
        int64_t demod = 0;
        URH_CHECK(urh_stream_footprint(n, dtype, 0, chunk_samples, ring, URH_STREAM_ENTRY_AFP_DEMOD | URH_STREAM_PSK | URH_STREAM_RESIDENT,
                                       -1, &demod));
        *bytes = r256(n * 8) + demod;
        return URH_OK;
    }
    if (!(entry & URH_STREAM_RESIDENT) && (ring < 2 || ring > URH_STREAM_MAX_RING)) return URH_ERR_INVALID;
    if ((entry & 0xf) != URH_STREAM_ENTRY_GRAB_PULSE_LENS && urh_iq_bytes(dtype) == 0) return URH_ERR_DTYPE;
    if ((entry & URH_STREAM_PSK) && (entry & 0xf) != URH_STREAM_ENTRY_AFP_DEMOD && (entry & 0xf) != URH_STREAM_ENTRY_DEMOD_DIGITIZE)
        return URH_ERR_INVALID;
    const StreamSizes z = stream_sizes(n, dtype, tolerance, chunk_samples, ring, entry);
    const bool digitize = (entry & 0xf) != URH_STREAM_ENTRY_AFP_DEMOD;
    const int64_t r = rows == -2 ? n / 64 + 1024 : (rows < 0 ? rows_bound(n, tolerance) : rows);
    if (entry & URH_STREAM_RESIDENT) {
        const int64_t ntiles = urh_div_up(n, URH_TILE);
        int64_t b = z.ring_bytes + URH_ARENA_BLOCK;
        if (digitize)
            b += r256(ntiles * (int64_t)sizeof(UrhTileSummary)) + r256(ntiles * (int64_t)stage_cap_for(tolerance) * 4) +
                 finish_arena_bytes(ntiles, r + r / 4, true) + 16 * (r + r / 4);
        if ((entry & 0xf) == URH_STREAM_ENTRY_DEMOD_CENTER_DIGITIZE)
            b += r256(ntiles * (int64_t)sizeof(UrhTileStats)) + r256((int64_t)URH_FINE_SLABS * URH_FINE_NB * 4) + r256((ntiles + 1) * 8);
        if (psk_order_of(entry)) b += urh_costas_arena_bytes(n, psk_order_of(entry));
        *bytes = b;
        return URH_OK;
    }
    int64_t b = z.ring_bytes + stream_arena_bytes(z.arena);
    const int64_t nb = 2 * (z.scan_items / 256 + 1);
    b += 256 + (nb > 8192 ? nb : 8192) * (4 + 2 * 32);
    if (digitize) b += 3 * 16 * (r + z.rows_chunk);
    *bytes = b;
    return URH_OK;
}

extern "C" int urh_stream_stats(urh_ctx* ctx, int64_t* h_out3) {
    h_out3[0] = ctx->stream_free_low;
    h_out3[1] = ctx->stream_chunks;
    h_out3[2] = (int64_t)ctx->arena_peak;
    return URH_OK;
}

struct StreamDigitizer {
    UrhTileSummary* tiles;
    uint32_t* staging;
    int16_t* d_init;
    UrhChain* chain;
    int cap, tol;
    bool is_ask;
    uint32_t sps;
    int64_t n, rows, rows_all;
    UrhArenaMark mark;
    int init(urh_ctx* ctx, int64_t n_total, int64_t cs, int tolerance, bool ask, uint32_t samples_per_symbol) {
        n = n_total; tol = tolerance; is_ask = ask; sps = samples_per_symbol; rows = 0;
        cap = stage_cap_for(tol);
        rows_all = rows_bound(n, tol);
        URH_CHECK(digitizer_tables(ctx, cs / URH_TILE, cap, &tiles, &staging, &d_init));
        URH_CHECK(urh_arena(ctx, 1, &chain));
        URH_CUDA(ctx, cudaMemsetAsync(d_init, 0, 16, ctx->stream));
        mark = urh_arena_mark(ctx);
        return URH_OK;
    }
    int finish(urh_ctx* ctx, int64_t s0, int64_t s1) {
        const int64_t rc = rows_bound(s1 - s0, tol);
        const int64_t need = rows + rc;
        if (need > (int64_t)ctx->pulses_cap_rows) {
            int64_t grow = 2 * (int64_t)ctx->pulses_cap_rows;
            if (grow > rows_all + rc) grow = rows_all + rc;
            URH_CHECK(urh_ensure_pulses_keep(ctx, (size_t)(grow > need ? grow : need), (size_t)rows));
        }
        urh_arena_release(ctx, mark);
        int64_t kc = 0;
        URH_CHECK(urh_finish_chunk(ctx, s1 - s0, tol, is_ask, sps, tiles, staging, cap, d_init, chain, s0, n, rows, rc, &kc));
        urh_stream_sample_free(ctx);
        rows += kc;
        return URH_OK;
    }
};

static int stream_check(urh_ctx* ctx, int64_t n, int ring, int mod_type, int dtype, bool iq);
static int psk_stream_check(urh_ctx* ctx, int64_t n, int ring, int dtype) {
    URH_CHECK(stream_check(ctx, n, ring, URH_MOD_PSK, dtype, false));
    if (n <= 2) URH_FAIL(ctx, URH_ERR_INVALID, "streamed PSK demodulation: n > 2");
    if (urh_iq_bytes(dtype) == 0) URH_FAIL(ctx, URH_ERR_DTYPE, "Unsupported dtype");
    return URH_OK;
}

static int stream_check(urh_ctx* ctx, int64_t n, int ring, int mod_type, int dtype, bool iq) {
    if (n <= 0) URH_FAIL(ctx, URH_ERR_INVALID, "streamed call: empty capture");
    if (ring < 2 || ring > URH_STREAM_MAX_RING) URH_FAIL(ctx, URH_ERR_INVALID, "streamed call: ring of %d slots (2..%d)", ring, URH_STREAM_MAX_RING);
    if (iq && (n <= 2 || (mod_type != URH_MOD_ASK && mod_type != URH_MOD_FSK)))
        URH_FAIL(ctx, URH_ERR_INVALID, "streamed demodulation: ASK/FSK and n > 2 (PSK is a serial recurrence)");
    if (iq && urh_iq_bytes(dtype) == 0) URH_FAIL(ctx, URH_ERR_DTYPE, "Unsupported dtype");
    return URH_OK;
}

template <bool DIG>
static int stream_dense_iq(urh_ctx* ctx, int dtype, int mod_type, const char* d_src, int64_t src_slot, int64_t n, const UrhDemodParams& dp,
                           float* qad_global, const UrhClassify& cls, int tol, StreamDigitizer* dz, int64_t s0, int64_t s1, int s,
                           UrhTileStats* ts = nullptr, const UrhFine& fine = UrhFine{}) {
    const int b = urh_iq_bytes(dtype);
    const void* iq = d_src + s * src_slot + URH_STREAM_PAD - s0 * b;
    const int64_t t0 = s0 / URH_TILE, t1 = urh_div_up(s1, URH_TILE);
    UrhTileSummary* tiles = dz ? dz->tiles - t0 : nullptr;
    uint32_t* staging = dz ? dz->staging - t0 * dz->cap : nullptr;
    const int cap = dz ? dz->cap : 0;
    int16_t* init = dz ? dz->d_init : nullptr;
    const int c0 = DIG ? host_classify(0.0f, cls) : 0;
    if (mod_type == URH_MOD_ASK)
        return launch_dense_iq_m<URH_MOD_ASK, DIG>(ctx, dtype, iq, n, dp, qad_global, cls, tol, tiles, staging, cap, init, c0, 0, ts, t0, t1, fine);
    return launch_dense_iq_m<URH_MOD_FSK, DIG>(ctx, dtype, iq, n, dp, qad_global, cls, tol, tiles, staging, cap, init, c0, 0, ts, t0, t1, fine);
}

static int stream_dense_qad(urh_ctx* ctx, const float* x, int64_t s0, int64_t s1, const UrhClassify& cls, StreamDigitizer& dz,
                            const float* d_thr0 = nullptr, const UrhTileStats* ts = nullptr) {
    return launch_dense_qad(ctx, x, s1 - s0, cls, dz.tol, dz.tiles, dz.staging, dz.cap, s0 == 0 ? dz.d_init : nullptr,
                            d_thr0 ? 0 : host_classify(0.0f, cls), d_thr0, ts ? ts + s0 / URH_TILE : nullptr);
}

struct CenterPlan;
int urh_center_chain(urh_ctx* ctx, const float* d_qad, int64_t n, const UrhTileStats* ts, int64_t max_size, int rank, int world,
                     const UrhFine* fine, CenterPlan** d_plan_out);
int urh_center_plan_result(urh_ctx* ctx, const CenterPlan* plan, const float** d_centerf, const double** d_center, const int** d_state);
int urh_center_plan_certify_stats(urh_ctx* ctx, const CenterPlan* plan, int64_t* h_dst3);

extern "C" int urh_shard_digitize(urh_ctx* ctx, const void* d_iq, int dtype, const float* d_qad_in, int64_t n, int has_halo,
                                  float noise_mag, int mod_type, float center, uint16_t tolerance, uint32_t samples_per_symbol,
                                  uint8_t bits_per_symbol, float center_spacing, float* d_qad_out, int64_t global_offset,
                                  int64_t n_total, int64_t* k) {
    if (!k) return URH_ERR_INVALID;
    *k = 0;
    ctx->pulses_k = 0;
    if (n <= 0) URH_FAIL(ctx, URH_ERR_INVALID, "empty shard");
    if (mod_type != URH_MOD_ASK && mod_type != URH_MOD_FSK) URH_FAIL(ctx, URH_ERR_INVALID, "sharded path: ASK / FSK only");
    if (!d_qad_in && urh_iq_bytes(dtype) == 0) URH_FAIL(ctx, URH_ERR_DTYPE, "Unsupported dtype");
    if (!ctx->nccl_comm) URH_FAIL(ctx, URH_ERR_INVALID, "NCCL communicator not initialised (urh_nccl_init)");
    urh_arena_reset(ctx);
    UrhClassify cls;
    URH_CHECK(fill_classify(ctx, &cls, mod_type, center, bits_per_symbol, center_spacing));
    const int tol = tolerance;
    const int64_t ntiles = urh_div_up(n, URH_TILE);
    const int cap = stage_cap_for(tol);
    UrhTileSummary* tiles;
    uint32_t* staging;
    int16_t* d_init;
    URH_CHECK(digitizer_tables(ctx, ntiles, cap, &tiles, &staging, &d_init));
    URH_CUDA(ctx, cudaMemsetAsync(d_init, 0, 16, ctx->stream));
    const int c0 = host_classify(0.0f, cls);
    if (d_qad_in) {
        URH_PROF_BEGIN(ctx);
        URH_CHECK(launch_dense_qad(ctx, d_qad_in, n, cls, tol, tiles, staging, cap, d_init, c0));
        URH_PROF_END(ctx);
    } else {
        const UrhDemodParams dp = make_demod_params(noise_mag, mod_type, dtype);
        if (mod_type == URH_MOD_ASK)
            URH_CHECK((launch_dense_iq_m<URH_MOD_ASK, true>(ctx, dtype, d_iq, n, dp, d_qad_out, cls, tol, tiles, staging, cap, d_init, c0, has_halo)));
        else
            URH_CHECK((launch_dense_iq_m<URH_MOD_FSK, true>(ctx, dtype, d_iq, n, dp, d_qad_out, cls, tol, tiles, staging, cap, d_init, c0, has_halo)));
    }
    return urh_finish_shard(ctx, n, tol, mod_type == URH_MOD_ASK, samples_per_symbol, tiles, staging, cap, d_init, global_offset, n_total, k);
}

struct StreamCenter {
    int ring;
    int64_t chunk_samples;
    const void* h_iq;
    float* h_qad;
    int64_t* kept;
};
static int demod_center_digitize_impl(urh_ctx* ctx, const void* d_iq, int dtype, int64_t n, int has_halo, float noise_mag, int mod_type,
                                      uint16_t tolerance, uint32_t samples_per_symbol, int64_t max_size, float* d_qad_out, bool sharded,
                                      int64_t global_offset, int64_t n_total, double* center, int* center_state, int64_t* k,
                                      const void* h_iq = nullptr, int64_t chunk_samples = 0, const StreamCenter* sc = nullptr) {
    if (!k || !center || !center_state) return URH_ERR_INVALID;
    *k = 0;
    *center = 0.0;
    *center_state = 0;
    ctx->pulses_k = 0;
    if (n <= 2 || (mod_type != URH_MOD_ASK && mod_type != URH_MOD_FSK) || !d_qad_out)
        URH_FAIL(ctx, URH_ERR_INVALID, "demod_center_digitize: ASK/FSK, n > 2 and a qad buffer are required");
    if (urh_iq_bytes(dtype) == 0) URH_FAIL(ctx, URH_ERR_DTYPE, "Unsupported dtype");
    if (sharded && !ctx->nccl_comm) URH_FAIL(ctx, URH_ERR_INVALID, "NCCL communicator not initialised (urh_nccl_init)");
    urh_arena_reset(ctx);
    URH_TL_RESET(ctx);
    URH_TL_MARK(ctx, "step start");
    const UrhDemodParams dp = make_demod_params(noise_mag, mod_type, dtype);
    UrhClassify cls;
    memset(&cls, 0, sizeof(cls));
    const int64_t ntiles = urh_div_up(n, URH_TILE);
    UrhTileStats* ts;
    URH_CHECK(urh_arena(ctx, (size_t)ntiles, &ts));
    const bool no_certify = getenv("URH_B200_CENTER_NO_CERTIFY") != nullptr;
    UrhFine fine = {};
    if (!sharded && !no_certify) {
        fine.slab_tiles = urh_div_up(ntiles, URH_FINE_SLABS);
        if (fine.slab_tiles < URH_WARPS_PER_BLOCK) fine.slab_tiles = URH_WARPS_PER_BLOCK;
        const int64_t nslabs = urh_div_up(ntiles, fine.slab_tiles);
        URH_CHECK(urh_arena(ctx, (size_t)(nslabs * URH_FINE_NB), &fine.gh));
        URH_CUDA(ctx, cudaMemsetAsync(fine.gh, 0, (size_t)(nslabs * URH_FINE_NB) * sizeof(unsigned int), ctx->stream));
        fine.scale = (mod_type == URH_MOD_FSK) ? 512.0f : 4096.0f;
        fine.off = (mod_type == URH_MOD_FSK) ? 2048.0f : 0.0f;
    }
    const int64_t chunk_tiles = (h_iq && chunk_samples > 0) ? (chunk_samples >= URH_TILE ? chunk_samples / URH_TILE : 1) : ntiles;
    const size_t sample_bytes = (size_t)urh_iq_bytes(dtype);
    StreamRing ring;
    int64_t scs = 0;
    if (sc) {
        const StreamSizes z = stream_sizes(n, dtype, tolerance, sc->chunk_samples, sc->ring, URH_STREAM_ENTRY_DEMOD_CENTER_DIGITIZE);
        scs = z.cs;
        URH_CHECK(ring.init(ctx, sc->ring, sc->ring * r256(z.src_slot)));
        const int64_t slot = r256(z.src_slot);
        std::vector<UrhWindow> win;
        URH_CHECK(urh_filter_windows(URH_FILTER_TILES, n, n, 1, 0, sc->chunk_samples, nullptr, nullptr, 0, win));
        URH_CHECK(stream_run(ctx, win, ring, (const char*)sc->h_iq, urh_iq_bytes(dtype), ring.mem, slot, sc->h_qad != nullptr,
                             [&](int64_t, const UrhWindow& w, int s) {
                                 return stream_dense_iq<false>(ctx, dtype, mod_type, ring.mem, slot, n, dp, d_qad_out, cls, 0, nullptr, w.k0, w.k1,
                                                               s, ts, fine);
                             },
                             [&](int64_t, const UrhWindow& w, int, cudaStream_t cp) {
                                 URH_CUDA(ctx, cudaMemcpyAsync(sc->h_qad + w.k0, d_qad_out + w.k0, (size_t)(w.k1 - w.k0) * sizeof(float),
                                                               cudaMemcpyDeviceToHost, cp));
                                 return URH_OK;
                             },
                             place_after_pad, true));
    }
    cls.noise_value = urh_noise_value(mod_type);
    cls.order = 2;
    const int tol = tolerance;
    const int cap = stage_cap_for(tol);
    UrhTileSummary* tiles = nullptr;
    uint32_t* staging = nullptr;
    int16_t* d_init = nullptr;
    if (!sc) URH_CHECK(digitizer_tables(ctx, ntiles, cap, &tiles, &staging, &d_init));
    const bool speculate = !sharded && !h_iq && !sc && mod_type == URH_MOD_FSK && dtype == URH_DT_F32 &&
                           getenv("URH_B200_NO_SPECULATE") == nullptr;
    UrhSpec spec = {};
    if (speculate) {
        float* tg;
        URH_CHECK(urh_arena(ctx, 1, &tg));
        URH_CHECK(urh_arena(ctx, 1, &spec.redone));
        URH_CHECK(urh_arena(ctx, (size_t)ntiles, &spec.margin));
        spec.tg = tg;
        const char* forced = getenv("URH_B200_SPECULATE_GUESS");
        URH_LAUNCH(ctx, k_speculate_guess, 1, URH_GUESS_THREADS, 0, (const float2*)d_iq, n, dp.noise_sqrd, forced ? 1 : 0,
                   forced ? strtof(forced, nullptr) : 0.0f, tg, spec.redone);
    }
    int chunk_no = 0;
    for (int64_t t0 = 0; t0 < (sc ? 0 : ntiles); t0 += chunk_tiles, chunk_no++) {
        const int64_t t1 = (t0 + chunk_tiles < ntiles) ? t0 + chunk_tiles : ntiles;
        if (h_iq) {
            const int64_t s0 = t0 * URH_TILE, s1 = (t1 * URH_TILE < n) ? t1 * URH_TILE : n;
            cudaEvent_t ev = ctx->ev_copy[chunk_no & 1];
            URH_CUDA(ctx, cudaMemcpyAsync((char*)d_iq + (size_t)s0 * sample_bytes, (const char*)h_iq + (size_t)s0 * sample_bytes,
                                          (size_t)(s1 - s0) * sample_bytes, cudaMemcpyHostToDevice, ctx->copy_stream[0]));
            URH_CUDA(ctx, cudaEventRecord(ev, ctx->copy_stream[0]));
            URH_CUDA(ctx, cudaStreamWaitEvent(ctx->stream, ev, 0));
        }
        if (mod_type == URH_MOD_ASK)
            URH_CHECK((launch_dense_iq_m<URH_MOD_ASK, false>(ctx, dtype, d_iq, n, dp, d_qad_out, cls, 0, nullptr, nullptr, 0, nullptr, 0, has_halo, ts, t0, t1, fine)));
        else
            URH_CHECK((launch_dense_iq_m<URH_MOD_FSK, false>(ctx, dtype, d_iq, n, dp, d_qad_out, cls, tol, tiles, staging, cap, nullptr, 0, has_halo,
                                                             ts, t0, t1, fine, speculate ? &spec : nullptr)));
    }
    CenterPlan* plan = nullptr;
    URH_CHECK(urh_center_chain(ctx, d_qad_out, n, ts, max_size, sharded ? ctx->nccl_rank : 0, sharded ? ctx->nccl_world : 1,
                               fine.gh ? &fine : nullptr, &plan));
    const float* d_centerf;
    const double* d_center;
    const int* d_state;
    urh_center_plan_result(ctx, plan, &d_centerf, &d_center, &d_state);
    int64_t rows = 0;
    if (sc) {
        URH_CUDA(ctx, cudaMemcpyAsync(ctx->h_mail + 40, d_center, sizeof(double), cudaMemcpyDeviceToHost, ctx->stream));
        URH_CUDA(ctx, cudaMemcpyAsync(ctx->h_mail + 41, d_state, sizeof(int), cudaMemcpyDeviceToHost, ctx->stream));
        URH_CHECK(urh_center_plan_certify_stats(ctx, plan, ctx->h_mail + 42));
        URH_CUDA(ctx, cudaMemcpyAsync(ctx->h_mail + 45, (const int64_t*)ctx->center_prefix + ntiles, sizeof(int64_t), cudaMemcpyDeviceToHost,
                                      ctx->stream));
        URH_CUDA(ctx, cudaStreamSynchronize(ctx->stream));
        int st0 = 0;
        memcpy(&st0, ctx->h_mail + 41, sizeof(int));
        if (st0 == 1) {
            StreamDigitizer dz;
            URH_CHECK(dz.init(ctx, n, scs, tol, mod_type == URH_MOD_ASK, samples_per_symbol));
            for (int64_t s0 = 0; s0 < n; s0 += scs) {
                const int64_t s1 = s0 + scs < n ? s0 + scs : n;
                URH_CHECK(stream_dense_qad(ctx, d_qad_out + s0, s0, s1, cls, dz, d_centerf, ts));
                URH_CHECK(dz.finish(ctx, s0, s1));
            }
            rows = dz.rows;
        }
        *sc->kept = ctx->h_mail[45];
    } else {
        URH_CUDA(ctx, cudaMemsetAsync(d_init, 0, 16, ctx->stream));
        const int vec_in = (((uintptr_t)d_qad_out % 8) == 0) ? 1 : 0;
        int64_t grid = urh_div_up(ntiles, URH_WARPS_PER_BLOCK);
        if (speculate) {
            int per_sm = 0;
            URH_CUDA(ctx, cudaOccupancyMaxActiveBlocksPerMultiprocessor(&per_sm, k_dense_f32<SrcQad2, float>, URH_WARPS_PER_BLOCK * 32, 0));
            const int64_t resident = (int64_t)ctx->sm_count * (per_sm > 0 ? per_sm : 1);
            if (grid > resident) grid = resident;
        }
        URH_LAUNCH(ctx, (k_dense_f32<SrcQad2, float>), (unsigned)grid, URH_WARPS_PER_BLOCK * 32, 0,
                   (const float*)d_qad_out, n, vec_in, cls, tol, tiles, staging, cap, d_init, 0, d_centerf, (const UrhTileStats*)ts, spec);
        URH_CUDA(ctx, cudaMemcpyAsync(ctx->h_mail + 40, d_center, sizeof(double), cudaMemcpyDeviceToHost, ctx->stream));
        URH_CUDA(ctx, cudaMemcpyAsync(ctx->h_mail + 41, d_state, sizeof(int), cudaMemcpyDeviceToHost, ctx->stream));
        URH_CHECK(urh_center_plan_certify_stats(ctx, plan, ctx->h_mail + 42));
        ctx->h_mail[46] = 0;
        if (speculate) URH_CUDA(ctx, cudaMemcpyAsync(ctx->h_mail + 46, spec.redone, sizeof(unsigned int), cudaMemcpyDeviceToHost, ctx->stream));
        if (sharded)
            URH_CHECK(urh_finish_shard(ctx, n, tol, mod_type == URH_MOD_ASK, samples_per_symbol, tiles, staging, cap, d_init, global_offset, n_total, &rows));
        else
            URH_CHECK(urh_finish_local(ctx, n, tol, mod_type == URH_MOD_ASK, samples_per_symbol, tiles, staging, cap, d_init, &rows));
    }
    memcpy(center, ctx->h_mail + 40, sizeof(double));
    int st = 0;
    memcpy(&st, ctx->h_mail + 41, sizeof(int));
    *center_state = st;
    ctx->center_cert[0] = ctx->h_mail[42];
    ctx->center_cert[1] = fine.gh ? URH_FINE_NB : 0;
    ctx->center_cert[2] = ctx->h_mail[44];
    const int64_t redone = (spec.hi > spec.lo) ? ctx->h_mail[46] : 0;
    ctx->spec_stats[0] = spec.hi - spec.lo;
    ctx->spec_stats[1] = spec.hi - spec.lo - redone;
    ctx->spec_stats[2] = redone;
    if (st != 1) {
        ctx->pulses_k = 0;
        rows = 0;
    }
    *k = rows;
    return URH_OK;
}

extern "C" int urh_speculate_stats(urh_ctx* ctx, int64_t* h_out3) {
    for (int i = 0; i < 3; i++) h_out3[i] = ctx->spec_stats[i];
    return URH_OK;
}

extern "C" int urh_demod_center_digitize(urh_ctx* ctx, const void* d_iq, int dtype, int64_t n, float noise_mag, int mod_type,
                                         uint16_t tolerance, uint32_t samples_per_symbol, int64_t max_size, float* d_qad_out,
                                         double* center, int* center_state, int64_t* k) {
    return demod_center_digitize_impl(ctx, d_iq, dtype, n, 0, noise_mag, mod_type, tolerance, samples_per_symbol, max_size, d_qad_out, false,
                                      0, n, center, center_state, k);
}

extern "C" int urh_demod_center_digitize_host(urh_ctx* ctx, const void* h_iq, int dtype, int64_t n, float noise_mag, int mod_type,
                                              uint16_t tolerance, uint32_t samples_per_symbol, int64_t max_size, int64_t chunk_samples,
                                              void* d_iq_scratch, float* d_qad_out, double* center, int* center_state, int64_t* k) {
    if (!h_iq || !d_iq_scratch) return URH_ERR_INVALID;
    URH_CUDA(ctx, cudaEventRecord(ctx->ev_comp[0], ctx->stream));
    URH_CUDA(ctx, cudaStreamWaitEvent(ctx->copy_stream[0], ctx->ev_comp[0], 0));
    return demod_center_digitize_impl(ctx, d_iq_scratch, dtype, n, 0, noise_mag, mod_type, tolerance, samples_per_symbol, max_size, d_qad_out,
                                      false, 0, n, center, center_state, k, h_iq, chunk_samples > 0 ? chunk_samples : ((int64_t)1 << 24));
}

extern "C" int urh_shard_demod_center_digitize_host(urh_ctx* ctx, const void* h_iq, int dtype, int64_t n, int has_halo, float noise_mag,
                                                    int mod_type, uint16_t tolerance, uint32_t samples_per_symbol, int64_t max_size,
                                                    int64_t chunk_samples, void* d_iq_scratch, float* d_qad_out, int64_t global_offset,
                                                    int64_t n_total, double* center, int* center_state, int64_t* k) {
    if (!h_iq || !d_iq_scratch) return URH_ERR_INVALID;
    URH_CUDA(ctx, cudaEventRecord(ctx->ev_comp[0], ctx->stream));
    URH_CUDA(ctx, cudaStreamWaitEvent(ctx->copy_stream[0], ctx->ev_comp[0], 0));
    return demod_center_digitize_impl(ctx, d_iq_scratch, dtype, n, has_halo, noise_mag, mod_type, tolerance, samples_per_symbol, max_size,
                                      d_qad_out, true, global_offset, n_total, center, center_state, k, h_iq,
                                      chunk_samples > 0 ? chunk_samples : ((int64_t)1 << 24));
}

extern "C" int urh_shard_demod_center_digitize(urh_ctx* ctx, const void* d_iq, int dtype, int64_t n, int has_halo, float noise_mag,
                                               int mod_type, uint16_t tolerance, uint32_t samples_per_symbol, int64_t max_size,
                                               float* d_qad_out, int64_t global_offset, int64_t n_total, double* center,
                                               int* center_state, int64_t* k) {
    return demod_center_digitize_impl(ctx, d_iq, dtype, n, has_halo, noise_mag, mod_type, tolerance, samples_per_symbol, max_size, d_qad_out,
                                      true, global_offset, n_total, center, center_state, k);
}

extern "C" int urh_afp_demod_stream(urh_ctx* ctx, const void* h_iq, int dtype, int64_t n, float noise_mag, int mod_type, int64_t chunk_samples,
                                    int ring, float* h_qad) {
    if (!h_iq || !h_qad) return URH_ERR_INVALID;
    URH_CHECK(stream_check(ctx, n, ring, mod_type, dtype, true));
    urh_arena_reset(ctx);
    const StreamSizes z = stream_sizes(n, dtype, 0, chunk_samples, ring, URH_STREAM_ENTRY_AFP_DEMOD);
    StreamRing R;
    URH_CHECK(R.init(ctx, ring, z.ring_bytes));
    char* d_src = R.mem;
    float* d_qad = (float*)(R.mem + ring * r256(z.src_slot));
    const UrhDemodParams dp = make_demod_params(noise_mag, mod_type, dtype);
    UrhClassify cls;
    memset(&cls, 0, sizeof(cls));
    std::vector<UrhWindow> win;
    URH_CHECK(urh_filter_windows(URH_FILTER_TILES, n, n, 1, 0, chunk_samples, nullptr, nullptr, 0, win));
    return stream_run(ctx, win, R, (const char*)h_iq, urh_iq_bytes(dtype), d_src, r256(z.src_slot), true,
                      [&](int64_t, const UrhWindow& w, int s) {
                          return stream_dense_iq<false>(ctx, dtype, mod_type, d_src, r256(z.src_slot), n, dp, d_qad + s * z.cs - w.k0, cls, 0,
                                                        nullptr, w.k0, w.k1, s);
                      },
                      contiguous_download(ctx, (const char*)d_qad, z.cs * 4, (char*)h_qad, 4), place_after_pad);
}

extern "C" int urh_grab_pulse_lens_stream(urh_ctx* ctx, const float* qad, int qad_on_device, int64_t n, float center, uint16_t tolerance,
                                          int mod_type, uint32_t samples_per_symbol, uint8_t bits_per_symbol, float center_spacing,
                                          int64_t chunk_samples, int ring, int64_t* k) {
    if (!k || !qad) return URH_ERR_INVALID;
    *k = 0;
    ctx->pulses_k = 0;
    URH_CHECK(stream_check(ctx, n, ring, mod_type, 0, false));
    urh_arena_reset(ctx);
    UrhClassify cls;
    URH_CHECK(fill_classify(ctx, &cls, mod_type, center, bits_per_symbol, center_spacing));
    const StreamSizes z = stream_sizes(n, 0, tolerance, chunk_samples, ring,
                                       URH_STREAM_ENTRY_GRAB_PULSE_LENS | (qad_on_device ? URH_STREAM_QAD_ON_DEVICE : 0));
    StreamRing R;
    URH_CHECK(R.init(ctx, ring, z.ring_bytes));
    StreamDigitizer dz;
    URH_CHECK(dz.init(ctx, n, z.cs, tolerance, mod_type == URH_MOD_ASK, samples_per_symbol));
    char* d_src = R.mem;
    std::vector<UrhWindow> win;
    URH_CHECK(urh_filter_windows(URH_FILTER_TILES, n, n, 0, 0, chunk_samples, nullptr, nullptr, 0, win));
    URH_CHECK(stream_run(ctx, win, R, qad_on_device ? nullptr : (const char*)qad, 4, d_src, r256(z.src_slot), false,
                         [&](int64_t, const UrhWindow& w, int s) {
                             const float* x = qad_on_device ? qad + w.k0 : (const float*)(d_src + s * r256(z.src_slot) + URH_STREAM_PAD);
                             URH_CHECK(stream_dense_qad(ctx, x, w.k0, w.k1, cls, dz));
                             return dz.finish(ctx, w.k0, w.k1);
                         },
                         no_download, place_after_pad));
    *k = dz.rows;
    return URH_OK;
}

extern "C" int urh_demod_digitize_stream(urh_ctx* ctx, const void* h_iq, int dtype, int64_t n, float noise_mag, int mod_type, float center,
                                         uint16_t tolerance, uint32_t samples_per_symbol, uint8_t bits_per_symbol, float center_spacing,
                                         int64_t chunk_samples, int ring, float* h_qad_out, int64_t* k) {
    if (!k || !h_iq) return URH_ERR_INVALID;
    *k = 0;
    ctx->pulses_k = 0;
    URH_CHECK(stream_check(ctx, n, ring, mod_type, dtype, true));
    urh_arena_reset(ctx);
    UrhClassify cls;
    URH_CHECK(fill_classify(ctx, &cls, mod_type, center, bits_per_symbol, center_spacing));
    const UrhDemodParams dp = make_demod_params(noise_mag, mod_type, dtype);
    const StreamSizes z = stream_sizes(n, dtype, tolerance, chunk_samples, ring,
                                       URH_STREAM_ENTRY_DEMOD_DIGITIZE | (h_qad_out ? URH_STREAM_QAD_OUT : 0));
    StreamRing R;
    URH_CHECK(R.init(ctx, ring, z.ring_bytes));
    StreamDigitizer dz;
    URH_CHECK(dz.init(ctx, n, z.cs, tolerance, mod_type == URH_MOD_ASK, samples_per_symbol));
    char* d_src = R.mem;
    float* d_qad = h_qad_out ? (float*)(R.mem + ring * r256(z.src_slot)) : nullptr;
    std::vector<UrhWindow> win;
    URH_CHECK(urh_filter_windows(URH_FILTER_TILES, n, n, 1, 0, chunk_samples, nullptr, nullptr, 0, win));
    URH_CHECK(stream_run(ctx, win, R, (const char*)h_iq, urh_iq_bytes(dtype), d_src, r256(z.src_slot), h_qad_out != nullptr,
                         [&](int64_t, const UrhWindow& w, int s) {
                             URH_CHECK(stream_dense_iq<true>(ctx, dtype, mod_type, d_src, r256(z.src_slot), n, dp,
                                                             d_qad ? d_qad + s * z.cs - w.k0 : nullptr, cls, tolerance, &dz, w.k0, w.k1, s));
                             return dz.finish(ctx, w.k0, w.k1);
                         },
                         contiguous_download(ctx, (const char*)d_qad, z.cs * 4, (char*)h_qad_out, 4), place_after_pad));
    *k = dz.rows;
    return URH_OK;
}

extern "C" int urh_demod_center_digitize_stream(urh_ctx* ctx, const void* h_iq, int dtype, int64_t n, float noise_mag, int mod_type,
                                                uint16_t tolerance, uint32_t samples_per_symbol, int64_t max_size, int64_t chunk_samples,
                                                int ring, float* d_qad_out, float* h_qad_out, double* center, int* center_state,
                                                int64_t* kept, int64_t* k) {
    if (!h_iq || !d_qad_out || !kept) return URH_ERR_INVALID;
    URH_CHECK(stream_check(ctx, n, ring, mod_type, dtype, true));
    StreamCenter sc;
    sc.ring = ring; sc.chunk_samples = chunk_samples; sc.h_iq = h_iq; sc.h_qad = h_qad_out; sc.kept = kept;
    return demod_center_digitize_impl(ctx, nullptr, dtype, n, 0, noise_mag, mod_type, tolerance, samples_per_symbol, max_size, d_qad_out,
                                      false, 0, n, center, center_state, k, nullptr, 0, &sc);
}

extern "C" int urh_afp_demod_psk_stream(urh_ctx* ctx, const void* h_iq, int dtype, int64_t n, float noise_mag, int mod_order,
                                        float costas_loop_bandwidth, int64_t chunk_samples, int ring, float* h_qad) {
    if (!h_iq || !h_qad) return URH_ERR_INVALID;
    URH_CHECK(psk_stream_check(ctx, n, ring, dtype));
    urh_arena_reset(ctx);
    const StreamSizes z = stream_sizes(n, dtype, 0, chunk_samples, ring, URH_STREAM_ENTRY_AFP_DEMOD | psk_entry_flags(mod_order));
    StreamRing R;
    URH_CHECK(R.init(ctx, ring, z.ring_bytes));
    const int64_t slot = r256(z.src_slot);
    char* d_src = R.mem;
    float* d_qad = (float*)(R.mem + ring * slot);
    const UrhDemodParams dp = make_demod_params(noise_mag, URH_MOD_PSK, dtype);
    UrhCostasStream cs;
    URH_CHECK(urh_costas_stream_begin(ctx, &cs));
    const UrhArenaMark mark = urh_arena_mark(ctx);
    std::vector<UrhWindow> win;
    URH_CHECK(urh_filter_windows(URH_FILTER_TILES, n, n, 0, 0, chunk_samples, nullptr, nullptr, 0, win));
    URH_CHECK(stream_run(ctx, win, R, (const char*)h_iq, urh_iq_bytes(dtype), d_src, slot, true,
                         [&](int64_t c, const UrhWindow& w, int s) {
                             urh_arena_release(ctx, mark);
                             return urh_costas_stream_chunk(ctx, &cs, c, d_src + s * slot + URH_STREAM_PAD, dtype, w.k1 - w.k0, dp.noise_sqrd,
                                                            mod_order, costas_loop_bandwidth, d_qad + s * z.cs);
                         },
                         contiguous_download(ctx, (const char*)d_qad, z.cs * 4, (char*)h_qad, 4), place_after_pad));
    return urh_costas_stream_end(ctx, &cs);
}

extern "C" int urh_demod_digitize_psk_stream(urh_ctx* ctx, const void* h_iq, int dtype, int64_t n, float noise_mag, float center,
                                             uint16_t tolerance, uint32_t samples_per_symbol, uint8_t bits_per_symbol, float center_spacing,
                                             int64_t chunk_samples, int ring, float* h_qad_out, int64_t* k) {
    if (!k || !h_iq) return URH_ERR_INVALID;
    *k = 0;
    ctx->pulses_k = 0;
    URH_CHECK(psk_stream_check(ctx, n, ring, dtype));
    urh_arena_reset(ctx);
    UrhClassify cls;
    URH_CHECK(fill_classify(ctx, &cls, URH_MOD_PSK, center, bits_per_symbol, center_spacing));
    const int mod_order = 1 << bits_per_symbol;
    const UrhDemodParams dp = make_demod_params(noise_mag, URH_MOD_PSK, dtype);
    const StreamSizes z = stream_sizes(n, dtype, tolerance, chunk_samples, ring,
                                       URH_STREAM_ENTRY_DEMOD_DIGITIZE | (h_qad_out ? URH_STREAM_QAD_OUT : 0) | psk_entry_flags(mod_order));
    StreamRing R;
    URH_CHECK(R.init(ctx, ring, z.ring_bytes));
    const int64_t slot = r256(z.src_slot);
    char* d_src = R.mem;
    float* d_qad = (float*)(R.mem + ring * slot);
    UrhCostasStream cs;
    URH_CHECK(urh_costas_stream_begin(ctx, &cs));
    StreamDigitizer dz;
    URH_CHECK(dz.init(ctx, n, z.cs, tolerance, false, samples_per_symbol));
    std::vector<UrhWindow> win;
    URH_CHECK(urh_filter_windows(URH_FILTER_TILES, n, n, 0, 0, chunk_samples, nullptr, nullptr, 0, win));
    URH_CHECK(stream_run(ctx, win, R, (const char*)h_iq, urh_iq_bytes(dtype), d_src, slot, h_qad_out != nullptr,
                         [&](int64_t c, const UrhWindow& w, int s) {
                             urh_arena_release(ctx, dz.mark);
                             float* q = d_qad + s * z.cs;
                             URH_CHECK(urh_costas_stream_chunk(ctx, &cs, c, d_src + s * slot + URH_STREAM_PAD, dtype, w.k1 - w.k0, dp.noise_sqrd,
                                                               mod_order, 0.1f, q));
                             URH_CHECK(stream_dense_qad(ctx, q, w.k0, w.k1, cls, dz));
                             return dz.finish(ctx, w.k0, w.k1);
                         },
                         contiguous_download(ctx, (const char*)d_qad, z.cs * 4, (char*)h_qad_out, 4), place_after_pad));
    *k = dz.rows;
    return urh_costas_stream_end(ctx, &cs);
}

struct UrhShardState {
    UrhCandidates cand;
};
static UrhShardState* shard_state(urh_ctx* ctx) {
    if (!ctx->shard_state) ctx->shard_state = calloc(1, sizeof(UrhShardState));
    return (UrhShardState*)ctx->shard_state;
}

extern "C" int urh_shard_candidates(urh_ctx* ctx, int carry_valid, int carry_cls, int64_t carry_len, int64_t global_offset,
                                    int64_t* count, const int64_t** d_pos, const int16_t** d_cls, int* last_cand_cls) {
    if (!ctx->shard_tiles) URH_FAIL(ctx, URH_ERR_INVALID, "urh_segment_shard_pass must precede urh_shard_candidates");
    UrhShardCarry in;
    in.valid = carry_valid; in.cls = carry_cls; in.len = carry_len;
    UrhShardState* S = shard_state(ctx);
    URH_CHECK(urh_collect_candidates_shard(ctx, ctx->shard_n, ctx->shard_tol, (const UrhTileSummary*)ctx->shard_tiles,
                                           (const uint32_t*)ctx->shard_staging, ctx->shard_cap, in, global_offset, &S->cand));
    *count = S->cand.count;
    if (d_pos) *d_pos = S->cand.pos;
    if (d_cls) *d_cls = S->cand.cls;
    if (last_cand_cls) {
        *last_cand_cls = 0;
        if (S->cand.count > 0) {
            int16_t v = 0;
            URH_CUDA(ctx, cudaMemcpyAsync(&v, S->cand.cls + S->cand.count - 1, sizeof(v), cudaMemcpyDeviceToHost, ctx->stream));
            URH_CUDA(ctx, cudaStreamSynchronize(ctx->stream));
            *last_cand_cls = v;
        }
    }
    ctx->shard_tiles = nullptr;
    return URH_OK;
}

extern "C" int urh_fetch_candidates(urh_ctx* ctx, int64_t* h_pos, int16_t* h_cls, int64_t count) {
    UrhShardState* S = shard_state(ctx);
    if (count < 0 || count > S->cand.count) URH_FAIL(ctx, URH_ERR_INVALID, "fetch_candidates: count exceeds the table");
    if (count == 0) return URH_OK;
    URH_CUDA(ctx, cudaMemcpyAsync(h_pos, S->cand.pos, (size_t)count * sizeof(int64_t), cudaMemcpyDeviceToHost, ctx->stream));
    URH_CUDA(ctx, cudaMemcpyAsync(h_cls, S->cand.cls, (size_t)count * sizeof(int16_t), cudaMemcpyDeviceToHost, ctx->stream));
    URH_CUDA(ctx, cudaStreamSynchronize(ctx->stream));
    return URH_OK;
}

extern "C" int urh_fetch_pulses(urh_ctx* ctx, int64_t* h_rows, int64_t k) {
    if (k < 0 || k > ctx->pulses_k) URH_FAIL(ctx, URH_ERR_INVALID, "fetch_pulses: k=%lld exceeds last result %lld", (long long)k, (long long)ctx->pulses_k);
    if (k == 0) return URH_OK;
    URH_CUDA(ctx, cudaMemcpyAsync(h_rows, ctx->pulses, (size_t)k * 2 * sizeof(int64_t), cudaMemcpyDeviceToHost, ctx->stream));
    URH_CUDA(ctx, cudaStreamSynchronize(ctx->stream));
    return URH_OK;
}

extern "C" int urh_pulses_device_ptr(urh_ctx* ctx, const int64_t** d_rows, int64_t* k) {
    if (d_rows) *d_rows = ctx->pulses;
    if (k) *k = ctx->pulses_k;
    return URH_OK;
}


__global__ void k_selftest_div(uint64_t seed, int64_t count, unsigned long long* mismatches, unsigned long long* tested) {
    const int64_t stride = (int64_t)gridDim.x * blockDim.x;
    unsigned long long bad = 0, ok = 0;
    for (int64_t i = (int64_t)blockIdx.x * blockDim.x + threadIdx.x; i < count; i += stride) {
        uint64_t h = seed + (uint64_t)i * 0x9E3779B97F4A7C15ull;
        h = (h ^ (h >> 30)) * 0xBF58476D1CE4E5B9ull;
        h = (h ^ (h >> 27)) * 0x94D049BB133111EBull;
        h ^= h >> 31;
        uint64_t g = h * 0xD6E8FEB86659FD93ull + 0x632BE59BD9B4E019ull;
        g ^= g >> 29;
        const uint32_t span = URH_DIVWIN_HI - URH_DIVWIN_LO;
        uint32_t ea = URH_DIVWIN_LO + (uint32_t)((h >> 40) % span), eb = URH_DIVWIN_LO + (uint32_t)((g >> 40) % span);
        uint32_t ma = (uint32_t)h & 0x7fffff, mb = (uint32_t)g & 0x7fffff;
        if ((i & 15) == 1) ma = 0;
        if ((i & 15) == 2) mb = 0;
        if ((i & 15) == 3) { ma = 0x7fffff; }
        if ((i & 15) == 4) { mb = 0x7fffff; }
        if ((i & 15) == 5) { eb = ea; }
        float a0 = __uint_as_float((ea << 23) | ma), b0 = __uint_as_float((eb << 23) | mb);
        float a1 = __uint_as_float(((URH_DIVWIN_LO + (uint32_t)((g >> 12) % span)) << 23) | ((uint32_t)(h >> 9) & 0x7fffff));
        float b1 = __uint_as_float(((URH_DIVWIN_LO + (uint32_t)((h >> 12) % span)) << 23) | ((uint32_t)(g >> 9) & 0x7fffff));
        if ((i & 15) == 6) { a1 = __uint_as_float((URH_DIVWIN_LO << 23)); b1 = __uint_as_float(((URH_DIVWIN_HI - 1) << 23) | 0x7fffff); }
        if ((i & 15) == 8) { b1 = __uint_as_float((URH_DIVWIN_LO << 23)); a1 = __uint_as_float(((URH_DIVWIN_HI - 1) << 23) | 0x7fffff); }
        if ((i & 63) == 7) a1 = 0.0f;
        const float2 q = urh_div2_window(make_float2(a0, a1), make_float2(b0, b1));
        const float r0 = __fdiv_rn(a0, b0), r1 = __fdiv_rn(a1, b1);
        bad += (__float_as_uint(q.x) != __float_as_uint(r0)) + (__float_as_uint(q.y) != __float_as_uint(r1));
        ok += 2;
    }
    atomicAdd(mismatches, bad);
    atomicAdd(tested, ok);
}

extern "C" int urh_selftest_packed_div(urh_ctx* ctx, uint64_t seed, int64_t count, int64_t* mismatches, int64_t* tested) {
    urh_arena_reset(ctx);
    unsigned long long* d;
    URH_CHECK(urh_arena(ctx, 2, &d));
    URH_CUDA(ctx, cudaMemsetAsync(d, 0, 16, ctx->stream));
    URH_LAUNCH(ctx, k_selftest_div, (unsigned)(ctx->sm_count * 8), 256, 0, seed, count, d, d + 1);
    int64_t h[2];
    URH_CHECK(urh_read_i64(ctx, (const int64_t*)d, 2, h));
    *mismatches = h[0];
    *tested = h[1];
    return URH_OK;
}
```

### urh_b200/csrc/finish.cu

```cuda
#include "sparse.cuh"
#include "tilescan.cuh"

#include <limits.h>

#define CLS_NONE INT_MIN

struct __align__(16) CandAgg {
    int64_t cnt;
    int32_t last_cls;
    int32_t pad;
};
struct CandOp {
    __device__ __forceinline__ CandAgg operator()(const CandAgg& a, const CandAgg& b) const {
        CandAgg r;
        r.cnt = a.cnt + b.cnt;
        r.last_cls = (b.last_cls != CLS_NONE) ? b.last_cls : a.last_cls;
        r.pad = 0;
        return r;
    }
};
struct __align__(16) FireAgg {
    int64_t fired;
    int64_t last_pos;
};
struct FireOp {
    __device__ __forceinline__ FireAgg operator()(const FireAgg& a, const FireAgg& b) const {
        FireAgg r;
        r.fired = a.fired + b.fired;
        r.last_pos = (b.last_pos >= 0) ? b.last_pos : a.last_pos;
        return r;
    }
};

struct ScanRunCarry {
    const UrhTileSummary* tiles;
    int64_t n;
    RunCarry* carry;
    __device__ __forceinline__ RunCarry load(int64_t t) const {
        const int64_t rem = n - t * URH_TILE;
        const int tile_len = rem < URH_TILE ? (int)rem : URH_TILE;
        const UrhTileSummary s = tiles[t];
        RunCarry r;
        r.len = s.tail_len;
        r.cls = s.last_cls;
        r.flags = (s.head_len == tile_len) ? 1 : 0;
        return r;
    }
    __device__ __forceinline__ void post(int64_t t, const RunCarry& excl, const RunCarry&) const { carry[t] = excl; }
};

struct __align__(16) TileFire {
    int32_t first_cls;
    int32_t first_rel;
    int32_t fired;
    int32_t last_rel;
};
struct ScanCandidates {
    const UrhTileSummary* tiles;
    const uint32_t* staging;
    int stage_cap;
    const RunCarry* carry;
    const RunCarry* xcarry;
    int tol;
    int32_t* head_rel;
    int32_t* prev_cls;
    TileFire* fire;
    __device__ __forceinline__ CandAgg load(int64_t t) const {
        const UrhTileSummary s = tiles[t];
        RunCarry c = carry[t];
        if (xcarry) c = RunCarryOp()(*xcarry, c);
        int64_t start_len = 0;
        if (!(c.flags & 2) && c.cls == s.first_cls) start_len = c.len;
        int32_t rel = -1;
        if (start_len <= tol && (int64_t)tol < start_len + s.head_len) rel = (int32_t)(tol - start_len);
        head_rel[t] = rel;
        TileFire f;
        f.first_cls = CLS_NONE; f.first_rel = -1; f.fired = 0; f.last_rel = -1;
        int prev = CLS_NONE;
        if (rel >= 0) {
            prev = s.first_cls;
            f.first_cls = prev;
            f.first_rel = rel;
        }
        const uint32_t* st = staging + t * (int64_t)stage_cap;
        for (int j = 0; j < s.ncand; j += 4) {
            uint32_t w[4];
#pragma unroll
            for (int u = 0; u < 4; u++) w[u] = (j + u < s.ncand) ? st[j + u] : 0u;
#pragma unroll
            for (int u = 0; u < 4; u++) {
                if (j + u < s.ncand) {
                    const int cl = (int)(w[u] & 0xffffu) - 1;
                    const int p = (int)(w[u] >> 16);
                    if (prev == CLS_NONE) {
                        f.first_cls = cl;
                        f.first_rel = p;
                    } else if (cl != prev) {
                        f.fired++;
                        f.last_rel = p;
                    }
                    prev = cl;
                }
            }
        }
        fire[t] = f;
        CandAgg r;
        r.cnt = (int64_t)s.ncand + (rel >= 0 ? 1 : 0);
        r.last_cls = prev;
        r.pad = 0;
        return r;
    }
    __device__ __forceinline__ void post(int64_t t, const CandAgg& excl, const CandAgg&) const { prev_cls[t] = excl.last_cls; }
};

struct ScanFirings {
    const TileFire* fire;
    const int32_t* prev_cls;
    const int16_t* d_prev0;
    int64_t global_offset;
    int64_t* row_off;
    int64_t* prev_fired;
    __device__ __forceinline__ FireAgg load(int64_t t) const {
        const TileFire f = fire[t];
        int prev = prev_cls[t];
        if (prev == CLS_NONE) prev = *d_prev0;
        FireAgg r;
        r.fired = f.fired;
        int32_t last = f.last_rel;
        if (f.first_cls != CLS_NONE && f.first_cls != prev) {
            r.fired++;
            if (last < 0) last = f.first_rel;
        }
        r.last_pos = (last >= 0) ? t * URH_TILE + global_offset + last : -1;
        return r;
    }
    __device__ __forceinline__ void post(int64_t t, const FireAgg& excl, const FireAgg&) const {
        row_off[t] = excl.fired;
        prev_fired[t] = excl.last_pos;
    }
};

constexpr int FIN_TILES = 32;
constexpr int FIN_BATCH = 8;

struct FinRows {
    int64_t* out;
    int64_t cap_rows;
    int tol;
    int is_ask;
    int64_t sps;
};

struct FinWalk {
    int prev;
    int64_t pp;
    int64_t idx;
};

__device__ __forceinline__ void fin_row(const FinRows& R, int64_t idx, int64_t p, int64_t pp, int prev) {
    const int64_t rec = (pp >= 0) ? (p - pp) : (p + 1 - R.tol);
    int64_t st = prev;
    if (R.is_ask && st == -1 && rec < R.sps) st = 0;
    if (idx < R.cap_rows) *((longlong2*)R.out + idx) = make_longlong2(st, rec);
}

__device__ __forceinline__ void fin_chunk(FinWalk& W, uint32_t w, int cnt, int lane, int64_t base, const FinRows& R) {
    const int c = (int)(w & 0xffffu) - 1;
    const int rel = (int)(w >> 16);
    int pc = __shfl_up_sync(URH_FULL_MASK, c, 1);
    if (lane == 0) pc = W.prev;
    const bool fire = lane < cnt && c != pc;
    const unsigned fm = __ballot_sync(URH_FULL_MASK, fire);
    const unsigned lower = fm & ((1u << lane) - 1u);
    const int before = __shfl_sync(URH_FULL_MASK, rel, lower ? 31 - __clz(lower) : 0);
    if (fire) fin_row(R, W.idx + __popc(lower), base + rel, lower ? base + before : W.pp, pc);
    if (fm) W.pp = base + __shfl_sync(URH_FULL_MASK, rel, 31 - __clz(fm));
    W.idx += __popc(fm);
    if (cnt > 0) W.prev = __shfl_sync(URH_FULL_MASK, c, cnt - 1);
}

__global__ void __launch_bounds__(256) k_finish_rows(const UrhTileSummary* __restrict__ tiles, const uint32_t* __restrict__ staging,
                                                    int stage_cap, const int32_t* __restrict__ head_rel, const int32_t* __restrict__ prev_cls,
                                                    const int16_t* __restrict__ d_prev0, const int64_t* __restrict__ row_off,
                                                    const int64_t* __restrict__ prev_fired, const int64_t* __restrict__ d_xprev_fired,
                                                    int64_t ntiles, int64_t global_offset, int64_t n_total, int tol, int is_ask, int64_t sps,
                                                    int emit_tail, int64_t row_base, int64_t* __restrict__ out, int64_t cap_rows,
                                                    int64_t* __restrict__ d_out) {
    const int64_t t0 = ((int64_t)blockIdx.x * blockDim.x + threadIdx.x) / 32 * FIN_TILES;
    if (t0 >= ntiles) return;
    const int lane = threadIdx.x & 31;
    FinRows R;
    R.out = out; R.cap_rows = cap_rows; R.tol = tol; R.is_ask = is_ask; R.sps = sps;
    const int64_t tl = t0 + lane;
    int l_first = 0, l_ncand = 0, l_rel = -1, l_prev = 0;
    int64_t l_idx = 0, l_pp = -1;
    if (tl < ntiles) {
        const UrhTileSummary s = tiles[tl];
        l_first = s.first_cls;
        l_ncand = s.ncand;
        l_rel = head_rel[tl];
        l_prev = prev_cls[tl];
        if (l_prev == CLS_NONE) l_prev = *d_prev0;
        l_idx = row_off[tl];
        l_pp = prev_fired[tl];
        if (l_pp < 0) l_pp = *d_xprev_fired;
    }
    for (int j0 = 0; j0 < FIN_TILES && t0 + j0 < ntiles; j0 += FIN_BATCH) {
        uint32_t w0[FIN_BATCH];
#pragma unroll
        for (int u = 0; u < FIN_BATCH; u++) {
            const int nc = __shfl_sync(URH_FULL_MASK, l_ncand, j0 + u);
            w0[u] = (lane < nc) ? __ldg(staging + (t0 + j0 + u) * (int64_t)stage_cap + lane) : 0u;
        }
#pragma unroll
        for (int u = 0; u < FIN_BATCH; u++) {
            const int j = j0 + u;
            const int64_t t = t0 + j;
            if (t >= ntiles) break;
            const int64_t base = t * URH_TILE + global_offset;
            const int ncand = __shfl_sync(URH_FULL_MASK, l_ncand, j);
            const int rel = __shfl_sync(URH_FULL_MASK, l_rel, j);
            FinWalk W;
            W.prev = __shfl_sync(URH_FULL_MASK, l_prev, j);
            W.pp = __shfl_sync(URH_FULL_MASK, l_pp, j);
            W.idx = __shfl_sync(URH_FULL_MASK, l_idx, j);
            if (rel >= 0) {
                const int c = __shfl_sync(URH_FULL_MASK, l_first, j);
                if (c != W.prev) {
                    if (lane == 0) fin_row(R, W.idx, base + rel, W.pp, W.prev);
                    W.idx++;
                    W.pp = base + rel;
                }
                W.prev = c;
            }
            const uint32_t* st = staging + t * (int64_t)stage_cap;
            for (int k = 0; k < ncand; k += 32) {
                const uint32_t w = (k == 0) ? w0[u] : ((k + lane < ncand) ? __ldg(st + k + lane) : 0u);
                fin_chunk(W, w, min(32, ncand - k), lane, base, R);
            }
            if (t == ntiles - 1 && lane == 0) {
                int64_t idx = W.idx;
                const int64_t fired = idx;
                if (emit_tail && (is_ask || row_base + fired < n_total)) {
                    if (idx < cap_rows) *((longlong2*)out + idx) = make_longlong2(W.prev, (W.pp >= 0) ? (n_total - 1 - W.pp) : (n_total - tol));
                    idx++;
                }
                d_out[0] = idx;
                d_out[1] = fired;
            }
        }
    }
}

struct ScanMergeRows {
    const int64_t* raw;
    int64_t rows;
    int64_t n_total;
    int has_tail;
    int64_t* out;
    int64_t* d_k;
    const int64_t* prev_last;
    int64_t row_base;
    __device__ __forceinline__ int64_t load(int64_t r) const {
        if (r == 0) return (prev_last && raw[0] == *prev_last) ? 0 : 1;
        return raw[2 * r] != raw[2 * r - 2] ? 1 : 0;
    }
    __device__ __forceinline__ void post(int64_t r, const int64_t& excl, const int64_t& head) const {
        const bool is_tail = has_tail && r == rows - 1;
        if (is_tail && row_base + excl >= n_total) {
            *d_k = excl;
            return;
        }
        const int64_t o = excl + head - 1;
        if (head) out[2 * o] = raw[2 * r];
        atomicAdd((unsigned long long*)&out[2 * o + 1], (unsigned long long)raw[2 * r + 1]);
        if (r == rows - 1) *d_k = o + 1;
    }
};
struct AddI64 {
    __device__ __forceinline__ int64_t operator()(int64_t a, int64_t b) const { return a + b; }
};

__global__ void k_pack_stage1(const int16_t* __restrict__ d_init, const RunCarry* __restrict__ total, int64_t* __restrict__ msg) {
    memcpy(msg, total, sizeof(RunCarry));
    msg[2] = *d_init;
    msg[3] = 0;
}
__global__ void k_fold_carry(const int64_t* __restrict__ all, int rank, RunCarry* __restrict__ xcarry) {
    RunCarry acc;
    acc.len = 0; acc.cls = 0; acc.flags = 2 | 1;
    for (int q = 0; q < rank; q++) {
        RunCarry c;
        memcpy(&c, all + 4 * q, sizeof(c));
        acc = RunCarryOp()(acc, c);
    }
    if (rank == 0) acc.flags = 2;
    else acc.flags &= ~1;
    *xcarry = acc;
}
__global__ void k_fold_prev_cls(const int64_t* __restrict__ all, int rank, const int64_t* __restrict__ stage1, int16_t* __restrict__ prev0) {
    int v = (int)stage1[2];
    for (int q = 0; q < rank; q++) {
        CandAgg c;
        memcpy(&c, all + 2 * q, sizeof(c));
        if (c.last_cls != CLS_NONE) v = c.last_cls;
    }
    *prev0 = (int16_t)v;
}
__global__ void k_fold_prev_fired(const int64_t* __restrict__ all, int rank, int64_t* __restrict__ xprev) {
    int64_t v = -1;
    for (int q = 0; q < rank; q++) {
        FireAgg c;
        memcpy(&c, all + 2 * q, sizeof(c));
        if (c.last_pos >= 0) v = c.last_pos;
    }
    *xprev = v;
}

__global__ void k_chain_start(const int16_t* __restrict__ d_init, UrhChain* __restrict__ chain) {
    chain->run.len = 0; chain->run.cls = 0; chain->run.flags = 2 | 1;
    chain->prev_fired = -1;
    chain->last_state = INT64_MIN;
    chain->prev_cls = *d_init;
}
__global__ void k_chain_advance(UrhChain* __restrict__ chain, const RunCarry* __restrict__ tot_run, const CandAgg* __restrict__ tot_cand,
                                const FireAgg* __restrict__ tot_fire) {
    chain->run = RunCarryOp()(chain->run, *tot_run);
    if (tot_cand->last_cls != CLS_NONE) chain->prev_cls = (int16_t)tot_cand->last_cls;
    if (tot_fire->last_pos >= 0) chain->prev_fired = tot_fire->last_pos;
}
__global__ void k_chain_last_row(UrhChain* __restrict__ chain, const int64_t* __restrict__ table, int64_t rows) {
    if (rows > 0) chain->last_state = table[2 * (rows - 1)];
}

struct FinishShard {
    int rank, world;
    int64_t global_offset;
    int64_t n_total;
    int emit_tail;
    UrhChain* chain;
    int64_t row_base, rows_cap;
};

static int finish_tiles(urh_ctx* ctx, int64_t n, int tol, bool is_ask, uint32_t sps, const UrhTileSummary* tiles, const uint32_t* staging,
                        int stage_cap, const int16_t* d_init, const FinishShard& sh, int64_t* k) {
    const int64_t ntiles = urh_div_up(n, URH_TILE);
    const bool sharded = sh.world > 1;
    UrhChain* chain = sh.chain;
    RunCarry* carry;
    int32_t *head_rel, *prev_cls;
    int64_t *row_off, *prev_fired, *d_small;
    URH_CHECK(urh_arena(ctx, (size_t)ntiles, &carry));
    URH_CHECK(urh_arena(ctx, (size_t)ntiles, &head_rel));
    URH_CHECK(urh_arena(ctx, (size_t)ntiles, &prev_cls));
    URH_CHECK(urh_arena(ctx, (size_t)ntiles, &row_off));
    URH_CHECK(urh_arena(ctx, (size_t)ntiles, &prev_fired));
    TileFire* fire;
    URH_CHECK(urh_arena(ctx, (size_t)ntiles, &fire));
    URH_CHECK(urh_arena(ctx, (size_t)(32 + 8 * (sharded ? sh.world : 0)), &d_small));
    URH_CUDA(ctx, cudaMemsetAsync(d_small, 0xff, 4 * sizeof(int64_t), ctx->stream));
    RunCarry* d_tot_run = (RunCarry*)(d_small + 4);
    CandAgg* d_tot_cand = (CandAgg*)(d_small + 6);
    FireAgg* d_tot_fire = (FireAgg*)(d_small + 8);
    RunCarry* d_xcarry = (RunCarry*)(d_small + 10);
    int16_t* d_prev0 = (int16_t*)(d_small + 12);
    int64_t* d_xprev = d_small + 13;
    int64_t* d_msg1 = d_small + 16;
    int64_t* d_all1 = d_small + 32;
    int64_t* d_all2 = d_all1 + 4 * (sharded ? sh.world : 0);
    int64_t* d_all3 = d_all2 + 2 * (sharded ? sh.world : 0);

    if (chain && sh.global_offset == 0) URH_LAUNCH(ctx, k_chain_start, 1, 1, 0, d_init, chain);
    RunCarry rc_ident;
    rc_ident.len = 0; rc_ident.cls = 0; rc_ident.flags = 2 | 1;
    ScanRunCarry fa;
    fa.tiles = tiles; fa.n = n; fa.carry = carry;
    URH_CHECK((urhts::scan<RunCarry, RunCarryOp, ScanRunCarry>(ctx, ntiles, rc_ident, RunCarryOp(), fa, d_tot_run)));
    if (sharded) {
        URH_LAUNCH(ctx, k_pack_stage1, 1, 1, 0, d_init, (const RunCarry*)d_tot_run, d_msg1);
        URH_TL_MARK(ctx, "x4 run carry: enter");
        URH_CHECK(urh_nccl_allgather(ctx, d_msg1, d_all1, 4 * sizeof(int64_t)));
        URH_TL_MARK(ctx, "x4 run carry: done");
        URH_LAUNCH(ctx, k_fold_carry, 1, 1, 0, (const int64_t*)d_all1, sh.rank, d_xcarry);
    }
    ScanCandidates fb;
    fb.tiles = tiles; fb.staging = staging; fb.stage_cap = stage_cap; fb.carry = carry;
    fb.xcarry = sharded ? d_xcarry : (chain ? &chain->run : nullptr);
    fb.tol = tol; fb.head_rel = head_rel; fb.prev_cls = prev_cls; fb.fire = fire;
    CandAgg ca_ident;
    ca_ident.cnt = 0; ca_ident.last_cls = CLS_NONE; ca_ident.pad = 0;
    URH_CHECK((urhts::scan<CandAgg, CandOp, ScanCandidates, 4>(ctx, ntiles, ca_ident, CandOp(), fb, d_tot_cand)));
    const int16_t* prev0 = chain ? &chain->prev_cls : d_init;
    if (sharded) {
        URH_TL_MARK(ctx, "x5 candidates: enter");
        URH_CHECK(urh_nccl_allgather(ctx, d_tot_cand, d_all2, sizeof(CandAgg)));
        URH_TL_MARK(ctx, "x5 candidates: done");
        URH_LAUNCH(ctx, k_fold_prev_cls, 1, 1, 0, (const int64_t*)d_all2, sh.rank, (const int64_t*)d_all1, d_prev0);
        prev0 = d_prev0;
    }
    ScanFirings fc;
    fc.fire = fire; fc.prev_cls = prev_cls; fc.d_prev0 = prev0; fc.global_offset = sh.global_offset; fc.row_off = row_off;
    fc.prev_fired = prev_fired;
    FireAgg fi_ident;
    fi_ident.fired = 0; fi_ident.last_pos = -1;
    URH_CHECK((urhts::scan<FireAgg, FireOp, ScanFirings>(ctx, ntiles, fi_ident, FireOp(), fc, d_tot_fire)));
    const int64_t* xprev = chain ? &chain->prev_fired : d_small + 2;
    if (sharded) {
        URH_TL_MARK(ctx, "x6 firings: enter");
        URH_CHECK(urh_nccl_allgather(ctx, d_tot_fire, d_all3, sizeof(FireAgg)));
        URH_TL_MARK(ctx, "x6 firings: done");
        URH_LAUNCH(ctx, k_fold_prev_fired, 1, 1, 0, (const int64_t*)d_all3, sh.rank, d_xprev);
        xprev = d_xprev;
    }

    int64_t cap_rows = (int64_t)ctx->pulses_cap_rows;
    const int64_t guess = n / 64 + 1024;
    if (!chain && cap_rows < guess) {
        URH_CHECK(urh_ensure_pulses(ctx, (size_t)guess));
        cap_rows = (int64_t)ctx->pulses_cap_rows;
    }
    const int64_t row_base = chain ? sh.row_base : 0;
    int64_t* raw = ctx->pulses + 2 * row_base;
    int64_t raw_cap = chain ? sh.rows_cap : cap_rows;
    if (is_ask) URH_CHECK(urh_arena(ctx, (size_t)raw_cap * 2, &raw));
    int64_t got[2] = {0, 0};
    for (int attempt = 0; attempt < 2; attempt++) {
        URH_LAUNCH(ctx, k_finish_rows, (unsigned)urh_div_up(ntiles, 8 * FIN_TILES), 256, 0, tiles, staging, stage_cap, (const int32_t*)head_rel,
                   (const int32_t*)prev_cls, prev0, (const int64_t*)row_off, (const int64_t*)prev_fired, xprev, ntiles, sh.global_offset,
                   sh.n_total, tol, is_ask ? 1 : 0, (int64_t)sps, sh.emit_tail, row_base, raw, raw_cap, d_small);
        if (sharded && attempt == 0) URH_TL_MARK(ctx, "rows written");
        URH_CHECK(urh_read_i64(ctx, d_small, 2, got));
        if (got[0] <= raw_cap) break;
        if (attempt == 1 || chain) URH_FAIL(ctx, URH_ERR_CUDA, "finish_tiles: row buffer overflow after regrowth");
        if (is_ask) {
            URH_CHECK(urh_arena(ctx, (size_t)got[0] * 2, &raw));
            raw_cap = got[0];
        } else {
            URH_CHECK(urh_ensure_pulses(ctx, (size_t)got[0]));
            raw = ctx->pulses;
            raw_cap = (int64_t)ctx->pulses_cap_rows;
        }
    }
    if (chain) URH_LAUNCH(ctx, k_chain_advance, 1, 1, 0, chain, (const RunCarry*)d_tot_run, (const CandAgg*)d_tot_cand, (const FireAgg*)d_tot_fire);
    int64_t K = got[0];
    if (is_ask && K > 0) {
        if (!chain) URH_CHECK(urh_ensure_pulses(ctx, (size_t)K));
        int64_t* out = ctx->pulses + 2 * row_base;
        URH_CUDA(ctx, cudaMemsetAsync(out, 0, (size_t)K * 2 * sizeof(int64_t), ctx->stream));
        ScanMergeRows fm;
        fm.raw = raw; fm.rows = K; fm.n_total = sh.n_total; fm.has_tail = (sh.emit_tail && K > got[1]) ? 1 : 0; fm.out = out;
        fm.d_k = d_small;
        fm.prev_last = (chain && row_base > 0) ? &chain->last_state : nullptr;
        fm.row_base = row_base;
        URH_CHECK((urhts::scan<int64_t, AddI64, ScanMergeRows>(ctx, K, (int64_t)0, AddI64(), fm, (int64_t*)nullptr)));
        URH_CHECK(urh_read_i64(ctx, d_small, 1, &K));
        if (chain) URH_LAUNCH(ctx, k_chain_last_row, 1, 1, 0, chain, (const int64_t*)ctx->pulses, row_base + K);
    }
    ctx->pulses_k = row_base + K;
    *k = K;
    return URH_OK;
}

int urh_finish_chunk(urh_ctx* ctx, int64_t n, int tol, bool is_ask, uint32_t sps, const UrhTileSummary* tiles, const uint32_t* staging,
                     int stage_cap, const int16_t* d_init, UrhChain* chain, int64_t global_offset, int64_t n_total, int64_t row_base,
                     int64_t rows_cap, int64_t* k) {
    FinishShard sh;
    sh.rank = 0; sh.world = 1; sh.global_offset = global_offset; sh.n_total = n_total;
    sh.emit_tail = (global_offset + n == n_total) ? 1 : 0;
    sh.chain = chain; sh.row_base = row_base; sh.rows_cap = rows_cap;
    return finish_tiles(ctx, n, tol, is_ask, sps, tiles, staging, stage_cap, d_init, sh, k);
}

int urh_finish_local(urh_ctx* ctx, int64_t n, int tol, bool is_ask, uint32_t sps, const UrhTileSummary* tiles, const uint32_t* staging,
                     int stage_cap, const int16_t* d_init, int64_t* k) {
    FinishShard sh;
    sh.rank = 0; sh.world = 1; sh.global_offset = 0; sh.n_total = n; sh.emit_tail = 1;
    sh.chain = nullptr; sh.row_base = 0; sh.rows_cap = 0;
    return finish_tiles(ctx, n, tol, is_ask, sps, tiles, staging, stage_cap, d_init, sh, k);
}

int urh_finish_shard(urh_ctx* ctx, int64_t n, int tol, bool is_ask, uint32_t sps, const UrhTileSummary* tiles, const uint32_t* staging,
                     int stage_cap, const int16_t* d_init, int64_t global_offset, int64_t n_total, int64_t* k) {
    FinishShard sh;
    sh.rank = ctx->nccl_rank; sh.world = ctx->nccl_world; sh.global_offset = global_offset; sh.n_total = n_total;
    sh.emit_tail = (ctx->nccl_rank == ctx->nccl_world - 1) ? 1 : 0;
    sh.chain = nullptr; sh.row_base = 0; sh.rows_cap = 0;
    return finish_tiles(ctx, n, tol, is_ask, sps, tiles, staging, stage_cap, d_init, sh, k);
}
```

Measured before the change: 217,800.

## Fuse center-plan kernels, cut launches and host copies, retune finish scan sizes

Several changes land together. The center-rank computation is folded into the kept-count scan's post step, and the plan computation is folded into the last block of the window kernel. The pick step is fused into the histogram kernel through a last-block ticket, and the FAST template split becomes a runtime branch. Host readback is merged into a single plan-span memcpy, the occupancy query result is cached, and a memset is replaced by a write inside a scan. The certify loop is vectorized, and the finish tile and scan sizes are retuned. The aim is fewer kernel launches and host API calls per call, at the cost of more complex last-block synchronization and a possible register-pressure change from runtime branching.

```diff
diff --git a/urh_b200/csrc/center.cu b/urh_b200/csrc/center.cu
--- a/urh_b200/csrc/center.cu
+++ b/urh_b200/csrc/center.cu
@@ -2,6 +2,8 @@
 #include "scan.cuh"
 
 #include <math.h>
+#include <stddef.h>
+#include <string.h>
 #include <stdlib.h>
 
 int urh_window_var_bitwise(urh_ctx* ctx, const float* d_x, int64_t n, const int64_t* d_prefix, int64_t t0, int64_t t1, int64_t r0,
@@ -520,23 +522,7 @@
     long long pad;
 };
 
-struct ScanKept {
-    const UrhTileStats* ts;
-    int64_t* prefix;
-    __device__ __forceinline__ int64_t load(int64_t t) const { return ts[t].cnt; }
-    __device__ __forceinline__ void post(int64_t t, const int64_t& excl, const int64_t&) const { prefix[t] = excl; }
-};
-struct CenAddI64 {
-    __device__ __forceinline__ int64_t operator()(int64_t a, int64_t b) const { return a + b; }
-};
-
-__global__ void k_center_ranks(const int64_t* __restrict__ counts, int rank, int world, int64_t max_size, CenterPlan* __restrict__ plan) {
-    long long total = 0, offset = 0;
-    for (int q = 0; q < world; q++) {
-        if (q < rank) offset += counts[q];
-        total += counts[q];
-    }
-    const long long kept = counts[rank];
+__device__ __forceinline__ void cen_set_ranks(long long total, long long offset, long long kept, int64_t max_size, CenterPlan* plan) {
     long long r0 = (long long)(0.05 * (double)total), r1 = (long long)(0.95 * (double)total);
     if (max_size >= 0 && r1 - r0 > max_size) r1 = r0 + max_size;
     plan->total = total; plan->offset = offset; plan->r0 = r0; plan->r1 = r1;
@@ -550,6 +536,31 @@
     plan->straddle = 0;
 }
 
+struct ScanKept {
+    const UrhTileStats* ts;
+    int64_t* prefix;
+    int64_t ntiles;
+    int64_t max_size;
+    CenterPlan* plan;
+    __device__ __forceinline__ int64_t load(int64_t t) const { return ts[t].cnt; }
+    __device__ __forceinline__ void post(int64_t t, const int64_t& excl, const int64_t& elem) const {
+        prefix[t] = excl;
+        if (plan && t == ntiles - 1) cen_set_ranks(excl + elem, 0, excl + elem, max_size, plan);
+    }
+};
+struct CenAddI64 {
+    __device__ __forceinline__ int64_t operator()(int64_t a, int64_t b) const { return a + b; }
+};
+
+__global__ void k_center_ranks(const int64_t* __restrict__ counts, int rank, int world, int64_t max_size, CenterPlan* __restrict__ plan) {
+    long long total = 0, offset = 0;
+    for (int q = 0; q < world; q++) {
+        if (q < rank) offset += counts[q];
+        total += counts[q];
+    }
+    cen_set_ranks(total, offset, counts[rank], max_size, plan);
+}
+
 __device__ __forceinline__ int64_t cen_tile_of_rank(const int64_t* __restrict__ prefix, int64_t ntiles, int64_t r) {
     int64_t lo = 0, hi = ntiles;
     while (hi - lo > 1) {
@@ -559,85 +570,8 @@
     return lo;
 }
 
-__global__ void __launch_bounds__(256) k_center_window(const float* __restrict__ x, int64_t n, const UrhTileStats* __restrict__ ts,
-                                                      const int64_t* __restrict__ prefix, int64_t ntiles, CenterPlan* __restrict__ plan,
-                                                      CenStats* __restrict__ partial) {
-    __shared__ long long s_win[4];
-    __shared__ int s_pre[256];
-    __shared__ bool s_last;
-    const long long r0 = plan->lr0, r1 = plan->lr1;
-    if (threadIdx.x == 0) {
-        long long w0 = -1, w1 = -1, w2 = -1, w3 = -1;
-        if (r1 > r0) {
-            w0 = cen_tile_of_rank(prefix, ntiles, r0);
-            w1 = cen_tile_of_rank(prefix, ntiles, r1 - 1);
-            const bool cov0 = prefix[w0] >= r0 && prefix[w0 + 1] <= r1;
-            const bool cov1 = prefix[w1] >= r0 && prefix[w1 + 1] <= r1;
-            w2 = cov0 ? -1 : w0;
-            w3 = (cov1 || w1 == w0) ? -1 : w1;
-        }
-        s_win[0] = w0; s_win[1] = w1; s_win[2] = w2; s_win[3] = w3;
-        if (blockIdx.x == 0) { plan->win[0] = w0; plan->win[1] = w1; plan->win[2] = w2; plan->win[3] = w3; }
-    }
-    __syncthreads();
-    double sum = 0.0, sq = 0.0;
-    float mn = INFINITY, mx = -INFINITY;
-    long long cnt = 0;
-    if (s_win[0] >= 0) {
-        for (int64_t t = s_win[0] + (int64_t)blockIdx.x * 256 + threadIdx.x; t <= s_win[1]; t += (int64_t)gridDim.x * 256) {
-            const int64_t a = prefix[t], b = prefix[t + 1];
-            if (b > a && a >= r0 && b <= r1) {
-                const UrhTileStats v = ts[t];
-                sum += v.sum; sq += v.sumsq; mn = fminf(mn, v.mn); mx = fmaxf(mx, v.mx); cnt += v.cnt;
-            }
-        }
-    }
-    cen_block_fold(sum, sq, mn, mx, cnt, partial + blockIdx.x);
-    if (blockIdx.x < 2) {
-        const int64_t t = s_win[2 + blockIdx.x];
-        sum = 0.0; sq = 0.0; mn = INFINITY; mx = -INFINITY; cnt = 0;
-        if (t >= 0) {
-            float v[CEN_PER];
-            int64_t rank = cen_tile_ranks(x, n, t, prefix[t], v, s_pre);
-#pragma unroll
-            for (int j = 0; j < CEN_PER; j++) {
-                if (v[j] > -4.0f) {
-                    if (rank >= r0 && rank < r1) {
-                        sum += (double)v[j];
-                        sq += (double)v[j] * (double)v[j];
-                        mn = fminf(mn, v[j]);
-                        mx = fmaxf(mx, v[j]);
-                        cnt++;
-                    }
-                    rank++;
-                }
-            }
-        }
-        cen_block_fold(sum, sq, mn, mx, cnt, partial + gridDim.x + blockIdx.x);
-    }
-    __threadfence();
-    __syncthreads();
-    if (threadIdx.x == 0) s_last = atomicAdd(&plan->ticket, 1u) == gridDim.x - 1;
-    __syncthreads();
-    if (!s_last) return;
-    __threadfence();
-    sum = 0.0; sq = 0.0; mn = INFINITY; mx = -INFINITY; cnt = 0;
-    for (int64_t t = threadIdx.x; t < (int64_t)gridDim.x + 2; t += 256) {
-        CenStats p;
-        {
-            const int4* src = (const int4*)(partial + t);
-            int4 w0 = __ldcg(src), w1 = __ldcg(src + 1);
-            memcpy(&p, &w0, 16);
-            memcpy((char*)&p + 16, &w1, 16);
-        }
-        sum += p.sum; sq += p.sumsq; mn = fminf(mn, p.mn); mx = fmaxf(mx, p.mx); cnt += p.cnt;
-    }
-    cen_block_fold(sum, sq, mn, mx, cnt, &plan->local);
-}
-
-__global__ void __launch_bounds__(256) k_center_plan(const CenStats* __restrict__ parts, int world, CenterPlan* __restrict__ plan,
-                                                    float* __restrict__ fe, unsigned long long* __restrict__ hist,
-                                                    unsigned long long* __restrict__ xhist) {
+__device__ __forceinline__ void cen_plan_body(const CenStats* parts, int world, CenterPlan* plan, float* __restrict__ fe,
+                                              unsigned long long* __restrict__ hist, unsigned long long* __restrict__ xhist) {
     __shared__ int s_state;
     __shared__ long long s_nbins;
     __shared__ double s_hmin, s_edge1, s_delta;
@@ -678,6 +612,7 @@
         }
         plan->hmin = hmin; plan->edge1 = edge1; plan->delta = delta; plan->nbins = nbins;
         plan->state = state;
+        plan->ticket = 0u;
         plan->center = 0.0; plan->centerf = 0.0f;
         if (state == 1) {
             plan->scale = (float)(1.0 / delta);
@@ -703,13 +638,88 @@
     }
 }
 
-template <bool FAST>
-__global__ void __launch_bounds__(256, 3) k_hist_interior_dev(const float* __restrict__ x, int64_t n, const CenterPlan* __restrict__ plan,
-                                                          const float* __restrict__ g_fe, unsigned long long* __restrict__ hist,
-                                                          const int64_t* __restrict__ prefix) {
-    if (plan->state != 1 || plan->certified || (plan->fast != 0) != FAST) return;
-    hist_interior_body<true, FAST>(x, n, plan->win[0] + 1, plan->win[1], blockIdx.x, gridDim.x, g_fe, plan->scale, (int)plan->nbins, hist, 1,
-                                   prefix);
+__global__ void __launch_bounds__(256) k_center_plan(const CenStats* __restrict__ parts, int world, CenterPlan* __restrict__ plan,
+                                                    float* __restrict__ fe, unsigned long long* __restrict__ hist,
+                                                    unsigned long long* __restrict__ xhist) {
+    cen_plan_body(parts, world, plan, fe, hist, xhist);
+}
+
+__global__ void __launch_bounds__(256) k_center_window(const float* __restrict__ x, int64_t n, const UrhTileStats* __restrict__ ts,
+                                                      const int64_t* __restrict__ prefix, int64_t ntiles, CenterPlan* __restrict__ plan,
+                                                      CenStats* __restrict__ partial, int plan_here, float* __restrict__ fe,
+                                                      unsigned long long* __restrict__ hist, unsigned long long* __restrict__ xhist) {
+    __shared__ long long s_win[4];
+    __shared__ int s_pre[256];
+    __shared__ bool s_last;
+    const long long r0 = plan->lr0, r1 = plan->lr1;
+    if (threadIdx.x == 0) {
+        long long w0 = -1, w1 = -1, w2 = -1, w3 = -1;
+        if (r1 > r0) {
+            w0 = cen_tile_of_rank(prefix, ntiles, r0);
+            w1 = cen_tile_of_rank(prefix, ntiles, r1 - 1);
+            const bool cov0 = prefix[w0] >= r0 && prefix[w0 + 1] <= r1;
+            const bool cov1 = prefix[w1] >= r0 && prefix[w1 + 1] <= r1;
+            w2 = cov0 ? -1 : w0;
+            w3 = (cov1 || w1 == w0) ? -1 : w1;
+        }
+        s_win[0] = w0; s_win[1] = w1; s_win[2] = w2; s_win[3] = w3;
+        if (blockIdx.x == 0) { plan->win[0] = w0; plan->win[1] = w1; plan->win[2] = w2; plan->win[3] = w3; }
+    }
+    __syncthreads();
+    double sum = 0.0, sq = 0.0;
+    float mn = INFINITY, mx = -INFINITY;
+    long long cnt = 0;
+    if (s_win[0] >= 0) {
+        for (int64_t t = s_win[0] + (int64_t)blockIdx.x * 256 + threadIdx.x; t <= s_win[1]; t += (int64_t)gridDim.x * 256) {
+            const int64_t a = prefix[t], b = prefix[t + 1];
+            if (b > a && a >= r0 && b <= r1) {
+                const UrhTileStats v = ts[t];
+                sum += v.sum; sq += v.sumsq; mn = fminf(mn, v.mn); mx = fmaxf(mx, v.mx); cnt += v.cnt;
+            }
+        }
+    }
+    cen_block_fold(sum, sq, mn, mx, cnt, partial + blockIdx.x);
+    if (blockIdx.x < 2) {
+        const int64_t t = s_win[2 + blockIdx.x];
+        sum = 0.0; sq = 0.0; mn = INFINITY; mx = -INFINITY; cnt = 0;
+        if (t >= 0) {
+            float v[CEN_PER];
+            int64_t rank = cen_tile_ranks(x, n, t, prefix[t], v, s_pre);
+#pragma unroll
+            for (int j = 0; j < CEN_PER; j++) {
+                if (v[j] > -4.0f) {
+                    if (rank >= r0 && rank < r1) {
+                        sum += (double)v[j];
+                        sq += (double)v[j] * (double)v[j];
+                        mn = fminf(mn, v[j]);
+                        mx = fmaxf(mx, v[j]);
+                        cnt++;
+                    }
+                    rank++;
+                }
+            }
+        }
+        cen_block_fold(sum, sq, mn, mx, cnt, partial + gridDim.x + blockIdx.x);
+    }
+    __threadfence();
+    __syncthreads();
+    if (threadIdx.x == 0) s_last = atomicAdd(&plan->ticket, 1u) == gridDim.x - 1;
+    __syncthreads();
+    if (!s_last) return;
+    __threadfence();
+    sum = 0.0; sq = 0.0; mn = INFINITY; mx = -INFINITY; cnt = 0;
+    for (int64_t t = threadIdx.x; t < (int64_t)gridDim.x + 2; t += 256) {
+        CenStats p;
+        {
+            const int4* src = (const int4*)(partial + t);
+            int4 w0 = __ldcg(src), w1 = __ldcg(src + 1);
+            memcpy(&p, &w0, 16);
+            memcpy((char*)&p + 16, &w1, 16);
+        }
+        sum += p.sum; sq += p.sumsq; mn = fminf(mn, p.mn); mx = fmaxf(mx, p.mx); cnt += p.cnt;
+    }
+    cen_block_fold(sum, sq, mn, mx, cnt, &plan->local);
+    if (plan_here) cen_plan_body(&plan->local, 1, plan, fe, hist, xhist);
 }
 
 __device__ __forceinline__ void cen_full_slabs(int64_t win0, int64_t win1, int64_t slab_tiles, int64_t* sf, int64_t* se) {
@@ -760,14 +770,19 @@
     constexpr int PER = URH_FINE_NB / CERT_THREADS;
     int64_t sf, se;
     cen_full_slabs(plan->win[0], plan->win[1], fine.slab_tiles, &sf, &se);
+    static_assert(PER == 8, "k_center_certify: one thread sums 8 buckets, two 16-byte loads per slab");
     unsigned long long b[PER], tot = 0;
 #pragma unroll
-    for (int j = 0; j < PER; j++) {
-        unsigned long long v = 0;
-        for (int64_t sl = sf; sl < se; sl++) v += fine.gh[sl * URH_FINE_NB + tid * PER + j];
-        b[j] = v;
-        tot += v;
-    }
+    for (int j = 0; j < PER; j++) b[j] = 0ull;
+    const uint4* g = (const uint4*)(fine.gh + tid * PER);
+#pragma unroll 4
+    for (int64_t sl = sf; sl < se; sl++) {
+        const uint4 u = g[sl * (URH_FINE_NB / 4)], w = g[sl * (URH_FINE_NB / 4) + 1];
+        b[0] += u.x; b[1] += u.y; b[2] += u.z; b[3] += u.w;
+        b[4] += w.x; b[5] += w.y; b[6] += w.z; b[7] += w.w;
+    }
+#pragma unroll
+    for (int j = 0; j < PER; j++) tot += b[j];
     s_part[tid] = tot;
     if (tid < 3) s_key[tid] = 0ull;
     if (tid == 0) s_certain = 0u;
@@ -842,11 +857,7 @@
     plan->certified = 1;
 }
 
-__global__ void __launch_bounds__(256) k_center_pick(const unsigned long long* __restrict__ y, CenterPlan* __restrict__ plan) {
-    __shared__ unsigned long long s_best[256];
-    __shared__ int s_idx[256];
-    __shared__ int s_cnt[256];
-    if (plan->state != 1 || plan->certified) return;
+__device__ __forceinline__ void cen_pick_body(const unsigned long long* y, CenterPlan* plan, unsigned long long* s_best, int* s_idx, int* s_cnt) {
     const int nbins = (int)plan->nbins;
     int window = (int)(0.05 * (double)nbins) + 1;
     if (window < 2) window = 2;
@@ -859,12 +870,12 @@
         int bi = -1, ties = 0;
         for (int i = threadIdx.x; i < nbins; i += 256) {
             if (pass == 1 && i == top_idx[0]) continue;
-            const unsigned long long v = y[i];
+            const unsigned long long v = __ldcg(y + i);
             if (v == 0ull || v < best) continue;
             bool peak = true;
             for (int d = 1; d < window && peak; d++) {
-                const unsigned long long a = (i + d < nbins) ? y[i + d] : 0ull;
-                const unsigned long long b = (i - d >= 0) ? y[i - d] : 0ull;
+                const unsigned long long a = (i + d < nbins) ? __ldcg(y + i + d) : 0ull;
+                const unsigned long long b = (i - d >= 0) ? __ldcg(y + i - d) : 0ull;
                 peak = v > a && v > b;
             }
             if (!peak) continue;
@@ -893,11 +904,11 @@
             if (t == 2) {
                 int other = -1;
                 for (int i = threadIdx.x; i < nbins; i += 256) {
-                    if (i == idx || y[i] != b) continue;
+                    if (i == idx || __ldcg(y + i) != b) continue;
                     bool peak = true;
                     for (int d = 1; d < window && peak; d++) {
-                        const unsigned long long a = (i + d < nbins) ? y[i + d] : 0ull;
-                        const unsigned long long c = (i - d >= 0) ? y[i - d] : 0ull;
+                        const unsigned long long a = (i + d < nbins) ? __ldcg(y + i + d) : 0ull;
+                        const unsigned long long c = (i - d >= 0) ? __ldcg(y + i - d) : 0ull;
                         peak = b > a && b > c;
                     }
                     if (peak) other = i;
@@ -930,6 +941,36 @@
     plan->centerf = __double2float_rn(c);
     plan->state = 1;
     (void)top_val;
+}
+
+__global__ void __launch_bounds__(256) k_center_pick(const unsigned long long* __restrict__ y, CenterPlan* __restrict__ plan) {
+    __shared__ unsigned long long s_best[256];
+    __shared__ int s_idx[256];
+    __shared__ int s_cnt[256];
+    if (plan->state != 1 || plan->certified) return;
+    cen_pick_body(y, plan, s_best, s_idx, s_cnt);
+}
+
+__global__ void __launch_bounds__(256, 3) k_hist_interior_dev(const float* __restrict__ x, int64_t n, CenterPlan* plan,
+                                                          const float* __restrict__ g_fe, unsigned long long* hist,
+                                                          const int64_t* __restrict__ prefix, int pick) {
+    extern __shared__ unsigned long long s_pick[];
+    __shared__ bool s_last;
+    if (plan->state != 1 || plan->certified) return;
+    if (plan->fast)
+        hist_interior_body<true, true>(x, n, plan->win[0] + 1, plan->win[1], blockIdx.x, gridDim.x, g_fe, plan->scale, (int)plan->nbins, hist, 1,
+                                       prefix);
+    else
+        hist_interior_body<true, false>(x, n, plan->win[0] + 1, plan->win[1], blockIdx.x, gridDim.x, g_fe, plan->scale, (int)plan->nbins, hist, 1,
+                                        prefix);
+    if (!pick) return;
+    __threadfence();
+    __syncthreads();
+    if (threadIdx.x == 0) s_last = atomicAdd(&plan->ticket, 1u) == gridDim.x - 1;
+    __syncthreads();
+    if (!s_last) return;
+    __threadfence();
+    cen_pick_body(hist, plan, s_pick, (int*)(s_pick + 256), (int*)(s_pick + 256) + 256);
 }
 
 int urh_center_chain(urh_ctx* ctx, const float* d_qad, int64_t n, const UrhTileStats* ts, int64_t max_size, int rank, int world,
@@ -957,38 +998,34 @@
         URH_CHECK(urh_arena(ctx, (size_t)CEN_MAX_BINS, &cert_hi));
     }
     ScanKept fk;
-    fk.ts = ts; fk.prefix = prefix;
+    fk.ts = ts; fk.prefix = prefix; fk.ntiles = ntiles; fk.max_size = max_size; fk.plan = world == 1 ? plan : nullptr;
     URH_CHECK((urhts::scan<int64_t, CenAddI64, ScanKept>(ctx, ntiles, (int64_t)0, CenAddI64(), fk, prefix + ntiles)));
-    const int64_t* counts = prefix + ntiles;
     if (world > 1) {
         URH_TL_MARK(ctx, "x1 kept counts: enter");
         URH_CHECK(urh_nccl_allgather(ctx, prefix + ntiles, d_counts, sizeof(int64_t)));
         URH_TL_MARK(ctx, "x1 kept counts: done");
-        counts = d_counts;
-    }
-    URH_LAUNCH(ctx, k_center_ranks, 1, 1, 0, counts, rank, world, max_size, plan);
-    URH_LAUNCH(ctx, k_center_window, nb, 256, 0, d_qad, n, ts, (const int64_t*)prefix, ntiles, plan, partial);
-    const CenStats* parts = &plan->local;
+        URH_LAUNCH(ctx, k_center_ranks, 1, 1, 0, (const int64_t*)d_counts, rank, world, max_size, plan);
+    }
+    URH_LAUNCH(ctx, k_center_window, nb, 256, 0, d_qad, n, ts, (const int64_t*)prefix, ntiles, plan, partial, world == 1 ? 1 : 0, fe, hist,
+               xhist);
     if (world > 1) {
         URH_TL_MARK(ctx, "x2 window partials: enter");
         URH_CHECK(urh_nccl_allgather(ctx, &plan->local, d_parts, sizeof(CenStats)));
         URH_TL_MARK(ctx, "x2 window partials: done");
-        parts = d_parts;
-    }
-    URH_LAUNCH(ctx, k_center_plan, 1, 256, 0, parts, world, plan, fe, hist, xhist);
+        URH_LAUNCH(ctx, k_center_plan, 1, 256, 0, (const CenStats*)d_parts, world, plan, fe, hist, xhist);
+    }
     const size_t dyn = (size_t)CEN_MAX_BINS * 4 + (size_t)(CEN_MAX_BINS + 3) * 4;
     const unsigned gs = (unsigned)min(urh_div_up(ntiles, 8), (int64_t)ctx->sm_count * 8);
     URH_LAUNCH(ctx, k_hist_window_ends_dev, fine ? 2 + ctx->sm_count * 4 : 2, 256, fine ? dyn : 0, d_qad, n, (const int64_t*)prefix,
                (const CenterPlan*)plan, (const float*)fe, hist, xhist, fine ? fine->slab_tiles : (int64_t)1);
     if (fine) URH_LAUNCH(ctx, k_center_certify, 1, CERT_THREADS, 0, *fine, plan, (const float*)fe, (const unsigned long long*)xhist, cert_lo, cert_hi);
-    URH_LAUNCH(ctx, (k_hist_interior_dev<true>), gs, 256, dyn, d_qad, n, (const CenterPlan*)plan, (const float*)fe, hist, (const int64_t*)prefix);
-    URH_LAUNCH(ctx, (k_hist_interior_dev<false>), gs, 256, dyn, d_qad, n, (const CenterPlan*)plan, (const float*)fe, hist, (const int64_t*)prefix);
+    URH_LAUNCH(ctx, k_hist_interior_dev, gs, 256, dyn, d_qad, n, plan, (const float*)fe, hist, (const int64_t*)prefix, world == 1 ? 1 : 0);
     if (world > 1) {
         URH_TL_MARK(ctx, "x3 histogram sum: enter");
         URH_CHECK(urh_nccl_allreduce_i64(ctx, (int64_t*)hist, CEN_MAX_BINS, 0));
         URH_TL_MARK(ctx, "x3 histogram sum: done");
-    }
-    URH_LAUNCH(ctx, k_center_pick, 1, 256, 0, (const unsigned long long*)hist, plan);
+        URH_LAUNCH(ctx, k_center_pick, 1, 256, 0, (const unsigned long long*)hist, plan);
+    }
     ctx->center_prefix = prefix;
     ctx->center_ts = ts;
     ctx->center_n = n;
@@ -997,11 +1034,20 @@
     return URH_OK;
 }
 
-int urh_center_plan_certify_stats(urh_ctx* ctx, const CenterPlan* plan, int64_t* h_dst3) {
-    h_dst3[0] = h_dst3[1] = h_dst3[2] = 0;
-    URH_CUDA(ctx, cudaMemcpyAsync(h_dst3, &plan->certified, sizeof(int), cudaMemcpyDeviceToHost, ctx->stream));
-    URH_CUDA(ctx, cudaMemcpyAsync(h_dst3 + 2, &plan->straddle, sizeof(long long), cudaMemcpyDeviceToHost, ctx->stream));
+#define CEN_RESULT_SPAN (offsetof(CenterPlan, straddle) + sizeof(long long) - offsetof(CenterPlan, center))
+static_assert(CEN_RESULT_SPAN == 5 * sizeof(int64_t), "CenterPlan: center .. straddle must be contiguous");
+int urh_center_plan_fetch(urh_ctx* ctx, const CenterPlan* plan, int64_t* h_dst5) {
+    URH_CUDA(ctx, cudaMemcpyAsync(h_dst5, &plan->center, CEN_RESULT_SPAN, cudaMemcpyDeviceToHost, ctx->stream));
     return URH_OK;
+}
+void urh_center_plan_read(const int64_t* h_src5, double* center, int* state, int64_t* cert3) {
+    CenterPlan p;
+    memcpy((char*)&p + offsetof(CenterPlan, center), h_src5, CEN_RESULT_SPAN);
+    *center = p.center;
+    *state = p.state;
+    cert3[0] = p.certified;
+    cert3[1] = 0;
+    cert3[2] = p.straddle;
 }
 
 extern "C" int urh_center_certify_stats(urh_ctx* ctx, int64_t* h_out3) {
diff --git a/urh_b200/csrc/common.cuh b/urh_b200/csrc/common.cuh
--- a/urh_b200/csrc/common.cuh
+++ b/urh_b200/csrc/common.cuh
@@ -66,6 +66,7 @@
     void* center_prefix;
     int64_t center_cert[3];
     int64_t spec_stats[3];
+    int redo_blocks_per_sm;
     void* nccl_comm;
     void* nccl_stage;
     void* nccl_hstage;
diff --git a/urh_b200/csrc/digitize.cu b/urh_b200/csrc/digitize.cu
--- a/urh_b200/csrc/digitize.cu
+++ b/urh_b200/csrc/digitize.cu
@@ -676,7 +676,8 @@
 int urh_center_chain(urh_ctx* ctx, const float* d_qad, int64_t n, const UrhTileStats* ts, int64_t max_size, int rank, int world,
                      const UrhFine* fine, CenterPlan** d_plan_out);
 int urh_center_plan_result(urh_ctx* ctx, const CenterPlan* plan, const float** d_centerf, const double** d_center, const int** d_state);
-int urh_center_plan_certify_stats(urh_ctx* ctx, const CenterPlan* plan, int64_t* h_dst3);
+int urh_center_plan_fetch(urh_ctx* ctx, const CenterPlan* plan, int64_t* h_dst5);
+void urh_center_plan_read(const int64_t* h_src5, double* center, int* state, int64_t* cert3);
 
 extern "C" int urh_shard_digitize(urh_ctx* ctx, const void* d_iq, int dtype, const float* d_qad_in, int64_t n, int has_halo,
                                   float noise_mag, int mod_type, float center, uint16_t tolerance, uint32_t samples_per_symbol,
@@ -820,19 +821,17 @@
     URH_CHECK(urh_center_chain(ctx, d_qad_out, n, ts, max_size, sharded ? ctx->nccl_rank : 0, sharded ? ctx->nccl_world : 1,
                                fine.gh ? &fine : nullptr, &plan));
     const float* d_centerf;
-    const double* d_center;
-    const int* d_state;
-    urh_center_plan_result(ctx, plan, &d_centerf, &d_center, &d_state);
+    urh_center_plan_result(ctx, plan, &d_centerf, nullptr, nullptr);
     int64_t rows = 0;
     if (sc) {
-        URH_CUDA(ctx, cudaMemcpyAsync(ctx->h_mail + 40, d_center, sizeof(double), cudaMemcpyDeviceToHost, ctx->stream));
-        URH_CUDA(ctx, cudaMemcpyAsync(ctx->h_mail + 41, d_state, sizeof(int), cudaMemcpyDeviceToHost, ctx->stream));
-        URH_CHECK(urh_center_plan_certify_stats(ctx, plan, ctx->h_mail + 42));
+        URH_CHECK(urh_center_plan_fetch(ctx, plan, ctx->h_mail + 48));
         URH_CUDA(ctx, cudaMemcpyAsync(ctx->h_mail + 45, (const int64_t*)ctx->center_prefix + ntiles, sizeof(int64_t), cudaMemcpyDeviceToHost,
                                       ctx->stream));
         URH_CUDA(ctx, cudaStreamSynchronize(ctx->stream));
+        double c0;
         int st0 = 0;
-        memcpy(&st0, ctx->h_mail + 41, sizeof(int));
+        int64_t cert0[3];
+        urh_center_plan_read(ctx->h_mail + 48, &c0, &st0, cert0);
         if (st0 == 1) {
             StreamDigitizer dz;
             URH_CHECK(dz.init(ctx, n, scs, tol, mod_type == URH_MOD_ASK, samples_per_symbol));
@@ -849,16 +848,17 @@
         const int vec_in = (((uintptr_t)d_qad_out % 8) == 0) ? 1 : 0;
         int64_t grid = urh_div_up(ntiles, URH_WARPS_PER_BLOCK);
         if (speculate) {
-            int per_sm = 0;
-            URH_CUDA(ctx, cudaOccupancyMaxActiveBlocksPerMultiprocessor(&per_sm, k_dense_f32<SrcQad2, float>, URH_WARPS_PER_BLOCK * 32, 0));
-            const int64_t resident = (int64_t)ctx->sm_count * (per_sm > 0 ? per_sm : 1);
+            if (ctx->redo_blocks_per_sm == 0) {
+                int per_sm = 0;
+                URH_CUDA(ctx, cudaOccupancyMaxActiveBlocksPerMultiprocessor(&per_sm, k_dense_f32<SrcQad2, float>, URH_WARPS_PER_BLOCK * 32, 0));
+                ctx->redo_blocks_per_sm = per_sm > 0 ? per_sm : 1;
+            }
+            const int64_t resident = (int64_t)ctx->sm_count * ctx->redo_blocks_per_sm;
             if (grid > resident) grid = resident;
         }
         URH_LAUNCH(ctx, (k_dense_f32<SrcQad2, float>), (unsigned)grid, URH_WARPS_PER_BLOCK * 32, 0,
                    (const float*)d_qad_out, n, vec_in, cls, tol, tiles, staging, cap, d_init, 0, d_centerf, (const UrhTileStats*)ts, spec);
-        URH_CUDA(ctx, cudaMemcpyAsync(ctx->h_mail + 40, d_center, sizeof(double), cudaMemcpyDeviceToHost, ctx->stream));
-        URH_CUDA(ctx, cudaMemcpyAsync(ctx->h_mail + 41, d_state, sizeof(int), cudaMemcpyDeviceToHost, ctx->stream));
-        URH_CHECK(urh_center_plan_certify_stats(ctx, plan, ctx->h_mail + 42));
+        URH_CHECK(urh_center_plan_fetch(ctx, plan, ctx->h_mail + 48));
         ctx->h_mail[46] = 0;
         if (speculate) URH_CUDA(ctx, cudaMemcpyAsync(ctx->h_mail + 46, spec.redone, sizeof(unsigned int), cudaMemcpyDeviceToHost, ctx->stream));
         if (sharded)
@@ -866,13 +866,10 @@
         else
             URH_CHECK(urh_finish_local(ctx, n, tol, mod_type == URH_MOD_ASK, samples_per_symbol, tiles, staging, cap, d_init, &rows));
     }
-    memcpy(center, ctx->h_mail + 40, sizeof(double));
     int st = 0;
-    memcpy(&st, ctx->h_mail + 41, sizeof(int));
+    urh_center_plan_read(ctx->h_mail + 48, center, &st, ctx->center_cert);
     *center_state = st;
-    ctx->center_cert[0] = ctx->h_mail[42];
     ctx->center_cert[1] = fine.gh ? URH_FINE_NB : 0;
-    ctx->center_cert[2] = ctx->h_mail[44];
     const int64_t redone = (spec.hi > spec.lo) ? ctx->h_mail[46] : 0;
     ctx->spec_stats[0] = spec.hi - spec.lo;
     ctx->spec_stats[1] = spec.hi - spec.lo - redone;
diff --git a/urh_b200/csrc/finish.cu b/urh_b200/csrc/finish.cu
--- a/urh_b200/csrc/finish.cu
+++ b/urh_b200/csrc/finish.cu
@@ -36,6 +36,7 @@
     const UrhTileSummary* tiles;
     int64_t n;
     RunCarry* carry;
+    int64_t* no_prev;
     __device__ __forceinline__ RunCarry load(int64_t t) const {
         const int64_t rem = n - t * URH_TILE;
         const int tile_len = rem < URH_TILE ? (int)rem : URH_TILE;
@@ -46,7 +47,10 @@
         r.flags = (s.head_len == tile_len) ? 1 : 0;
         return r;
     }
-    __device__ __forceinline__ void post(int64_t t, const RunCarry& excl, const RunCarry&) const { carry[t] = excl; }
+    __device__ __forceinline__ void post(int64_t t, const RunCarry& excl, const RunCarry&) const {
+        carry[t] = excl;
+        if (t == 0) *no_prev = -1;
+    }
 };
 
 struct __align__(16) TileFire {
@@ -140,7 +144,7 @@
     }
 };
 
-constexpr int FIN_TILES = 32;
+constexpr int FIN_TILES = 8;
 constexpr int FIN_BATCH = 8;
 
 struct FinRows {
@@ -194,7 +198,7 @@
     const int64_t tl = t0 + lane;
     int l_first = 0, l_ncand = 0, l_rel = -1, l_prev = 0;
     int64_t l_idx = 0, l_pp = -1;
-    if (tl < ntiles) {
+    if (lane < FIN_TILES && tl < ntiles) {
         const UrhTileSummary s = tiles[tl];
         l_first = s.first_cls;
         l_ncand = s.ncand;
@@ -358,7 +362,6 @@
     TileFire* fire;
     URH_CHECK(urh_arena(ctx, (size_t)ntiles, &fire));
     URH_CHECK(urh_arena(ctx, (size_t)(32 + 8 * (sharded ? sh.world : 0)), &d_small));
-    URH_CUDA(ctx, cudaMemsetAsync(d_small, 0xff, 4 * sizeof(int64_t), ctx->stream));
     RunCarry* d_tot_run = (RunCarry*)(d_small + 4);
     CandAgg* d_tot_cand = (CandAgg*)(d_small + 6);
     FireAgg* d_tot_fire = (FireAgg*)(d_small + 8);
@@ -374,7 +377,7 @@
     RunCarry rc_ident;
     rc_ident.len = 0; rc_ident.cls = 0; rc_ident.flags = 2 | 1;
     ScanRunCarry fa;
-    fa.tiles = tiles; fa.n = n; fa.carry = carry;
+    fa.tiles = tiles; fa.n = n; fa.carry = carry; fa.no_prev = d_small + 2;
     URH_CHECK((urhts::scan<RunCarry, RunCarryOp, ScanRunCarry>(ctx, ntiles, rc_ident, RunCarryOp(), fa, d_tot_run)));
     if (sharded) {
         URH_LAUNCH(ctx, k_pack_stage1, 1, 1, 0, d_init, (const RunCarry*)d_tot_run, d_msg1);
@@ -389,7 +392,7 @@
     fb.tol = tol; fb.head_rel = head_rel; fb.prev_cls = prev_cls; fb.fire = fire;
     CandAgg ca_ident;
     ca_ident.cnt = 0; ca_ident.last_cls = CLS_NONE; ca_ident.pad = 0;
-    URH_CHECK((urhts::scan<CandAgg, CandOp, ScanCandidates, 4>(ctx, ntiles, ca_ident, CandOp(), fb, d_tot_cand)));
+    URH_CHECK((urhts::scan<CandAgg, CandOp, ScanCandidates, 2>(ctx, ntiles, ca_ident, CandOp(), fb, d_tot_cand)));
     const int16_t* prev0 = chain ? &chain->prev_cls : d_init;
     if (sharded) {
         URH_TL_MARK(ctx, "x5 candidates: enter");
```

After: 220,300 (median of 6 runs). 1.2% higher.
